# tanhuajie/Pytorch-RT1-for-Distributed-Training

Hardware: AMD Instinct MI355X
Metric: train samples/sec (whole node), RT-1 Language-Table, 1/2/4/8 MI355X (higher is better)
Workload: dtype bf16; 1 GPU; model=RT-1 (FiLM-EfficientNet-B3 + TokenLearner-8 + 8-layer transformer, 35.3M params), global_batch=128, batch_per_gpu=128, seq_len=6, parallelism=dp1, backend=hip, hipgraph=True, step=graph, graph_segments=1, tuned_library_gemms=True, full=False

## Files before the change

### pytorch_rt1_for_distributed_training_amd/csrc/bindings.cpp

```cpp
#include <algorithm>
#include <cmath>
#include <cstdlib>

#include <torch/extension.h>
#include <c10/hip/HIPStream.h>
#include <hip/hip_runtime.h>

#include "rt1_kernels.h"

namespace {

hipStream_t cur_stream() { return c10::hip::getCurrentHIPStream().stream(); }

bool sync_check() {
    static const bool on = [] {
        const char* e = std::getenv("RT1_SYNC_CHECK");
        return e != nullptr && *e != '\0' && *e != '0';
    }();
    return on;
}

void check_launch(int err, const char* what) {
    TORCH_CHECK(err == 0, what, ": HIP launch failed: ", hipGetErrorString((hipError_t)err));
    if (sync_check()) {
// ... 1207 lines not shown
    auto red = fs > 1 ? at::empty({5, N, Ce}, f32(y2)) : R[0];
    auto dW = at::empty({Cout, Ce}, f32(y2));
    check_launch(rt1_proj_bwd_finalize(G.data_ptr<float>(), R.data_ptr<float>(), gate.data_ptr<float>(), N, Cout, Ce, fs,
                                       red.data_ptr<float>(), dW.data_ptr<float>(), cur_stream()), "proj_bwd_finalize");
    return {red, dW};
}
bool proj_bwd_supported(int64_t Cout, int64_t Ce) { return rt1_proj_bwd_supported((int)Cout, (int)Ce) != 0; }

}

bool pw_gemm_supported(int64_t K, int64_t N) {
    return rt1_pw_gemm_supported((int)K, (int)N) != 0 || rt1_pw_wide_supported((int)K, (int)N) != 0;
}
bool pw_stats_supported(int64_t K, int64_t N) { return rt1_pw_gemm_supported((int)K, (int)N) != 0; }

std::vector<at::Tensor> pw_gemm(at::Tensor A, at::Tensor B, int64_t max_blocks, bool stats, OptT scale, OptT shift,
                                OptT gate, int64_t hw, bool store_operand) {
    check_bf(A, "A"); check_bf(B, "B");
    TORCH_CHECK(A.dim() == 2 && B.dim() == 2 && A.size(1) == B.size(1), "pw_gemm: A [M,K], B [N,K]");
    const int64_t M = A.size(0), K = A.size(1), N = B.size(0);
    TORCH_CHECK(M > 0 && M < (int64_t)1 << 31, "pw_gemm: bad M");
    const bool skinny = rt1_pw_gemm_supported((int)K, (int)N) != 0;
    TORCH_CHECK(skinny || (!stats && rt1_pw_wide_supported((int)K, (int)N)), "pw_gemm: no specialisation for K=", K,
                " N=", N, stats ? " with BN statistics" : "");
    TORCH_CHECK(reinterpret_cast<uintptr_t>(A.data_ptr()) % 16 == 0 && reinterpret_cast<uintptr_t>(B.data_ptr()) % 16 == 0,
                "pw_gemm: operands must be 16-byte aligned");
    const bool pro = scale.has_value() && scale->defined();
    if (pro) {
        TORCH_CHECK(skinny, "pw_gemm: the operand prologue needs a skinny specialisation (K=", K, " N=", N, ")");
        check_f(*scale, "scale", K);
        TORCH_CHECK(shift.has_value() && shift->defined() && gate.has_value() && gate->defined(),
                    "pw_gemm: prologue needs scale, shift and gate");
        check_f(*shift, "shift", K);
        TORCH_CHECK(hw > 0 && M % hw == 0, "pw_gemm: hw must divide M");
        check_f(*gate, "gate", (M / hw) * K);
    }
    TORCH_CHECK(!store_operand || pro, "pw_gemm: store_operand needs the prologue");
    auto C = at::empty({M, N}, A.options());
    at::Tensor aout;
    if (store_operand) aout = at::empty({M, K}, A.options());
    if (!skinny) {
        check_launch(rt1_pw_wide(bp(A), bp(B), (int)M, (int)K, (int)N, bp(C), (int)max_blocks, cur_stream()), "pw_wide");
        return {C};
    }
    at::Tensor ps, pq;
    if (stats) {
        const int g = rt1_pw_gemm_grid((int)M, (int)K, (int)N, (int)max_blocks);
        ps = at::empty({g, N}, f32(A));
        pq = at::empty({g, N}, f32(A));
    }
    check_launch(rt1_pw_gemm(bp(A), bp(B), (int)M, (int)K, (int)N, bp(C), stats ? ps.data_ptr<float>() : nullptr,
                             stats ? pq.data_ptr<float>() : nullptr, (int)max_blocks, fpo(scale), fpo(shift),
                             fpo(gate), (int)hw, store_operand ? bp(aout) : nullptr, cur_stream()), "pw_gemm");
    std::vector<at::Tensor> res{C};
    if (stats) { res.push_back(ps); res.push_back(pq); }
    if (store_operand) res.push_back(aout);
    return res;
}


bool pw_gemm_bnbwd_supported(int64_t K, int64_t N) { return rt1_pw_gemm_bnbwd_supported((int)K, (int)N) != 0; }
std::vector<at::Tensor> pw_gemm_bnbwd(at::Tensor dout, at::Tensor y, at::Tensor W, at::Tensor fmul, OptT keep,
                                      int64_t hw, OptT gamma, at::Tensor mean, at::Tensor rstd, at::Tensor mdz,
                                      at::Tensor mdzx, int64_t max_blocks) {
    check_bf(dout, "dout"); check_bf(y, "y"); check_bf(W, "W");
    TORCH_CHECK(dout.dim() == 2 && dout.sizes() == y.sizes() && W.dim() == 2 && W.size(1) == dout.size(1),
                "pw_gemm_bnbwd: dout, y [M, K], W [N, K]");
    const int64_t M = dout.size(0), K = dout.size(1), N = W.size(0);
    TORCH_CHECK(rt1_pw_gemm_bnbwd_supported((int)K, (int)N), "pw_gemm_bnbwd: no specialisation for K=", K, " N=", N);
    TORCH_CHECK(hw > 0 && M % hw == 0, "pw_gemm_bnbwd: hw must divide M");
    TORCH_CHECK(reinterpret_cast<uintptr_t>(dout.data_ptr()) % 16 == 0 && reinterpret_cast<uintptr_t>(y.data_ptr()) % 16 == 0 &&
                reinterpret_cast<uintptr_t>(W.data_ptr()) % 16 == 0, "pw_gemm_bnbwd: operands must be 16-byte aligned");
    check_f(fmul, "fmul", (M / hw) * K);
    check_opt_f(keep, "keep", M / hw); check_opt_f(gamma, "gamma", K);
    check_f(mean, "mean", K); check_f(rstd, "rstd", K); check_f(mdz, "mdz", K); check_f(mdzx, "mdzx", K);
    auto C = at::empty({M, N}, dout.options());
    auto dy = at::empty({M, K}, dout.options());
    check_launch(rt1_pw_gemm_bnbwd(bp(dout), bp(W), (int)M, (int)K, (int)N, bp(C), (int)max_blocks, bp(y),
                                   fmul.data_ptr<float>(), fpo(keep), (int)hw, fpo(gamma), mean.data_ptr<float>(),
                                   rstd.data_ptr<float>(), mdz.data_ptr<float>(), mdzx.data_ptr<float>(), bp(dy),
                                   cur_stream()), "pw_gemm_bnbwd");
    return {C, dy};
}

bool pw_bwd_supported(int64_t CE, int64_t CIN) { return rt1_pw_bwd_supported((int)CE, (int)CIN) != 0; }

std::vector<at::Tensor> pw_bwd(at::Tensor dA, at::Tensor y, at::Tensor x, at::Tensor We, at::Tensor consts, OptT dout,
                               OptT fmul, int64_t HW, int64_t max_blocks) {
    check_bf(dA, "dA"); check_bf(y, "y"); check_bf(x, "x"); check_bf(We, "We");
    TORCH_CHECK(dA.dim() == 2 && y.sizes() == dA.sizes() && x.dim() == 2 && x.size(0) == dA.size(0),
                "pw_bwd: dA/y [M, CE], x [M, CIN]");
    const int64_t M = dA.size(0), CE = dA.size(1), CIN = x.size(1);
    TORCH_CHECK(M > 0 && M < (int64_t)1 << 31, "pw_bwd: bad M");
    TORCH_CHECK(rt1_pw_bwd_supported((int)CE, (int)CIN), "pw_bwd: no specialisation for CE=", CE, " CIN=", CIN);
    TORCH_CHECK(We.dim() == 2 && We.size(0) == CE && We.size(1) == CIN, "pw_bwd: We must be [CE, CIN]");
    check_f(consts, "consts", 5 * CE);
    const bool skip = dout.has_value() && dout->defined();
    if (skip) {
        check_opt_bf(dout, "dout", M * CIN);
        TORCH_CHECK(fmul.has_value() && fmul->defined() && HW > 0 && M % HW == 0, "pw_bwd: residual needs fmul, HW");
        check_f(*fmul, "fmul", (M / HW) * CIN);
    }
    const int g = rt1_pw_bwd_grid((int)M, (int)max_blocks);
    auto dx = at::empty({M, CIN}, x.options());
    auto dwp = at::empty({g, CE, CIN}, f32(x));
    check_launch(rt1_pw_bwd(bp(dA), bp(y), bp(x), bp(We), consts.data_ptr<float>(), (int)M, (int)CE, (int)CIN, bp(dx),
                            skip ? bp(*dout) : nullptr, skip ? fmul->data_ptr<float>() : nullptr, (int)HW,
                            dwp.data_ptr<float>(), g, cur_stream()), "pw_bwd");
    return {dx, sum0(dwp)};
}

std::vector<at::Tensor> pw_bwd_z(at::Tensor dz, at::Tensor x, at::Tensor We, at::Tensor consts, OptT dout, OptT fmul,
                                 int64_t HW, int64_t max_blocks) {
    check_bf(dz, "dz"); check_bf(x, "x"); check_bf(We, "We");
    TORCH_CHECK(dz.dim() == 2 && x.dim() == 2 && x.size(0) == dz.size(0), "pw_bwd_z: dz [M, CE], x [M, CIN]");
    const int64_t M = dz.size(0), CE = dz.size(1), CIN = x.size(1);
    TORCH_CHECK(M > 0 && M < (int64_t)1 << 31, "pw_bwd_z: bad M");
    TORCH_CHECK(rt1_pw_bwd_supported((int)CE, (int)CIN), "pw_bwd_z: no specialisation for CE=", CE, " CIN=", CIN);
    TORCH_CHECK(We.dim() == 2 && We.size(0) == CE && We.size(1) == CIN, "pw_bwd_z: We must be [CE, CIN]");
    check_f(consts, "consts", 5 * CE);
    const bool skip = dout.has_value() && dout->defined();
    if (skip) {
        check_opt_bf(dout, "dout", M * CIN);
        TORCH_CHECK(fmul.has_value() && fmul->defined() && HW > 0 && M % HW == 0, "pw_bwd_z: residual needs fmul, HW");
        check_f(*fmul, "fmul", (M / HW) * CIN);
    }
    const int g = rt1_pw_bwd_grid((int)M, (int)max_blocks);
    auto dx = at::empty({M, CIN}, x.options());
    auto mk = at::empty({(int64_t)rt1_pw_bwd_z_mk_elems((int)CIN)}, x.options());
    auto r0 = at::empty({CIN}, f32(x));
    auto part = at::empty({g, (int64_t)rt1_pw_bwd_z_width((int)CE, (int)CIN)}, f32(x));
    check_launch(rt1_pw_bwd_z(bp(dz), bp(x), bp(We), consts.data_ptr<float>(), (int)M, (int)CE, (int)CIN, bp(mk),
                              r0.data_ptr<float>(), bp(dx), skip ? bp(*dout) : nullptr,
                              skip ? fmul->data_ptr<float>() : nullptr, (int)HW, part.data_ptr<float>(), g,
                              cur_stream()), "pw_bwd_z");
    auto S = sum0(part);
    auto dWe = at::empty({CE, CIN}, f32(x));
    check_launch(rt1_pw_bwd_z_finish(S.data_ptr<float>(), bp(We), consts.data_ptr<float>(), (int)CE, (int)CIN,
                                     dWe.data_ptr<float>(), cur_stream()), "pw_bwd_z_finish");
    return {dx, dWe};
}

std::vector<at::Tensor> pw_z_prep(at::Tensor We, at::Tensor consts) {
    check_bf(We, "We");
    TORCH_CHECK(We.dim() == 2, "pw_z_prep: We must be [CE, CIN]");
    const int64_t CE = We.size(0), CIN = We.size(1);
    check_f(consts, "consts", 5 * CE);
    auto wt = at::empty({CIN, CE}, We.options());
    auto mk = at::empty({CIN, CIN}, We.options());
    auto r0 = at::empty({CIN}, We.options().dtype(at::kFloat));
    check_launch(rt1_pw_z_prep(bp(We), consts.data_ptr<float>(), (int)CE, (int)CIN, bp(wt), bp(mk),
                               r0.data_ptr<float>(), cur_stream()), "pw_z_prep");
    return {wt, mk, r0};
}

at::Tensor pw_tall_tail(at::Tensor A, at::Tensor W, at::Tensor A2, at::Tensor W2, at::Tensor bias, OptT res,
                        OptT rmul, int64_t rhw) {
    check_bf(A, "A"); check_bf(W, "W"); check_bf(A2, "A2"); check_bf(W2, "W2");
    TORCH_CHECK(A.dim() == 2 && W.dim() == 2 && A.size(1) == W.size(1), "pw_tall_tail: A [M, K], W [N, K]");
    const int64_t M = A.size(0), K = A.size(1), N = W.size(0), K2 = A2.size(1);
    TORCH_CHECK(A2.dim() == 2 && A2.size(0) == M, "pw_tall_tail: A2 must be [M, K2]");
    TORCH_CHECK(W2.numel() == N * K2, "pw_tall_tail: W2 must be [N, K2]"); check_f(bias, "bias", N);
    TORCH_CHECK(rt1_pw_tall_preferred((int)K, (int)N) && K2 % 8 == 0, "pw_tall_tail: unsupported K=", K, " N=", N,
                " K2=", K2);
    const bool has_res = res.has_value() && res->defined();
    if (has_res) {
        check_opt_bf(res, "res", M * N);
        TORCH_CHECK(rmul.has_value() && rmul->defined() && rhw > 0 && M % rhw == 0, "pw_tall_tail: residual needs rmul");
        check_f(*rmul, "rmul", (M / rhw) * N);
    }
    auto C = at::empty({M, N}, A.options());
    check_launch(rt1_pw_tall_tail(bp(A), bp(W), (int)M, (int)K, (int)N, bp(A2), bp(W2), (int)K2,
                                  bias.data_ptr<float>(), has_res ? bp(*res) : nullptr,
                                  has_res ? rmul->data_ptr<float>() : nullptr, (int)rhw, bp(C), cur_stream()),
                 "pw_tall_tail");
    return C;
}

at::Tensor pw_z_finish(at::Tensor S, at::Tensor G, at::Tensor sx, at::Tensor We, at::Tensor consts) {
    check_bf(We, "We");
    const int64_t CE = We.size(0), CIN = We.size(1);
    const int64_t splits = S.dim() == 3 ? S.size(0) : 1;
    check_f(S, "S", splits * CE * CIN); check_f(G, "G", CIN * CIN); check_f(sx, "sx", CIN);
    check_f(consts, "consts", 5 * CE);
    auto dWe = at::empty({CE, CIN}, f32(S));
    check_launch(rt1_pw_z_finish(S.data_ptr<float>(), (int)splits, G.data_ptr<float>(), sx.data_ptr<float>(), bp(We),
                                 consts.data_ptr<float>(), (int)CE, (int)CIN, dWe.data_ptr<float>(), cur_stream()),
                 "pw_z_finish");
    return dWe;
}

void check_rows512(const at::Tensor& t, const char* name, at::ScalarType dt) {
    check_dev(t, name, dt);
    TORCH_CHECK(t.dim() == 2 && t.size(1) == 512, name, " must be [T, 512]");
}

std::vector<at::Tensor> tf_ln_fwd(at::Tensor x, at::Tensor g, at::Tensor b, double eps) {
    check_rows512(x, "x", at::kFloat);
    check_f(g, "g", 512); check_f(b, "b", 512);
    const int T = (int)x.size(0);
    auto y = at::empty({T, 512}, x.options().dtype(at::kBFloat16));
    auto mu = at::empty({T}, x.options()), rs = at::empty({T}, x.options());
    check_launch(rt1_ln_fwd(x.data_ptr<float>(), g.data_ptr<float>(), b.data_ptr<float>(), T, (float)eps, bp(y),
                            mu.data_ptr<float>(), rs.data_ptr<float>(), cur_stream()), "ln_fwd");
    return {y, mu, rs};
}

std::vector<at::Tensor> tf_ln_bwd(at::Tensor dy, at::Tensor x, at::Tensor mu, at::Tensor rs, at::Tensor g, OptT dres,
                                  bool want_bf) {
    check_rows512(dy, "dy", at::kBFloat16); check_rows512(x, "x", at::kFloat);
    const int T = (int)x.size(0);
    TORCH_CHECK(dy.size(0) == T, "dy/x rows");
    check_f(mu, "mu", T); check_f(rs, "rs", T); check_f(g, "g", 512);
    if (dres.has_value() && dres->defined()) { check_rows512(*dres, "dres", at::kFloat); TORCH_CHECK(dres->size(0) == T, "dres rows"); }
    const int grid = rt1_tf_grid(T);
    auto dx = at::empty({T, 512}, x.options());
    auto part = at::empty({want_bf ? 3 : 2, grid, 512}, x.options());
    at::Tensor dxb;
    if (want_bf) dxb = at::empty({T, 512}, x.options().dtype(at::kBFloat16));
    check_launch(rt1_ln_bwd(bp(dy), x.data_ptr<float>(), mu.data_ptr<float>(), rs.data_ptr<float>(), g.data_ptr<float>(),
                            fpo(dres), T, dx.data_ptr<float>(), part[0].data_ptr<float>(), part[1].data_ptr<float>(),
                            want_bf ? bp(dxb) : nullptr, want_bf ? part[2].data_ptr<float>() : nullptr, grid,
                            cur_stream()), "ln_bwd");
    auto s = colsum3(part, want_bf ? 3 : 2, grid, 512);
    if (want_bf) return {dx, s[0], s[1], dxb, s[2]};
    return {dx, s[0], s[1]};
}

std::vector<at::Tensor> tf_resid(at::Tensor x, at::Tensor a, at::Tensor bias, double p, int64_t seed, OptT seed_dev,
                                 OptT lg, OptT lb, double eps) {
    check_rows512(x, "x", at::kFloat); check_rows512(a, "a", at::kBFloat16);
    TORCH_CHECK(a.size(0) == x.size(0), "x/a rows");
    check_f(bias, "bias", 512);
    const int T = (int)x.size(0);
    const bool ln = lg.has_value() && lg->defined();
    if (ln) { check_f(*lg, "lg", 512); check_f(*lb, "lb", 512); }
    auto out = at::empty_like(x);
    at::Tensor xn, mu, rs;
    if (ln) {
        xn = at::empty({T, 512}, x.options().dtype(at::kBFloat16));
        mu = at::empty({T}, x.options());
        rs = at::empty({T}, x.options());
    }
    check_launch(rt1_resid(x.data_ptr<float>(), bp(a), bias.data_ptr<float>(), T, (float)p, (uint32_t)seed,
                           seed_ptr(seed_dev), out.data_ptr<float>(), fpo(lg), fpo(lb), (float)eps,
                           ln ? bp(xn) : nullptr, ln ? mu.data_ptr<float>() : nullptr,
                           ln ? rs.data_ptr<float>() : nullptr, cur_stream()), "resid");
    if (ln) return {out, xn, mu, rs};
    return {out};
}

std::vector<at::Tensor> tf_drop_bwd(at::Tensor dout, double p, int64_t seed, OptT seed_dev) {
    check_rows512(dout, "dout", at::kFloat);
    const int T = (int)dout.size(0);
    const int grid = rt1_tf_grid(T);
    auto dh = at::empty({T, 512}, dout.options().dtype(at::kBFloat16));
    auto part = at::empty({grid, 512}, dout.options());
    check_launch(rt1_drop_bwd(dout.data_ptr<float>(), T, (float)p, (uint32_t)seed, seed_ptr(seed_dev), bp(dh),
                              part.data_ptr<float>(), grid,
                              cur_stream()), "drop_bwd");
    return {dh, sum0(part)};
}


namespace rt1comm {
void register_comm(py::module_& m);
}
namespace rt1head {
void register_head(py::module_& m);
}

PYBIND11_MODULE(_rt1_hip, m) {
    m.doc() = "RT-1 HIP/CDNA4 kernels (gfx950)";
    m.def("flat_adam", &flat_adam, "fused Adam/AdamW over flat fp32 buffers");
    m.def("flat_adam_dev", &flat_adam_dev, "fused Adam/AdamW, step/lr read from a device tensor (graph-replayable)");
    m.def("flat_adam_clip_dev", &flat_adam_clip_dev, "flat_adam_dev obeying clip_state (clip coefficient, skipped step)");
    m.def("flat_adam_ema_dev", &flat_adam_ema_dev, "flat_adam_dev / flat_adam_clip_dev that also updates the EMA of the weights");
    m.def("flat_adam_groups_dev", &flat_adam_groups_dev,
          "the device-state Adam forms (plain, clip, EMA, both) with lr / weight_decay per parameter group");
    m.def("gradnorm_partials", &gradnorm_partials, "fp64 partial sums grad_sumsq writes for n floats");
    m.def("grad_sumsq", &grad_sumsq, "deterministic sum of squares of a flat fp32 gradient -> fp64 partials");
    m.def("grad_clip_finalize", &grad_clip_finalize, "partials -> clip_state {norm, coef, ok, counters}");
    m.def("buffer_guard_", &buffer_guard_, "ok ? shadow = buf : buf = shadow");
    m.def("bn_stats", &bn_stats);
    m.def("bn_finalize", &bn_finalize);
    m.def("xgram", &xgram);
    m.def("gemm_tail", &gemm_tail, py::arg("A"), py::arg("B"), py::arg("A2"), py::arg("B2"), py::arg("bias") = py::none(),
          py::arg("res") = py::none(), py::arg("rmul") = py::none(), py::arg("rhw") = 1, py::arg("cfg") = -1);
    m.def("gemm256", &gemm256, py::arg("A"), py::arg("B"), py::arg("nn") = false, py::arg("bias") = py::none(),
          py::arg("scale") = py::none(), py::arg("shift") = py::none(), py::arg("gate") = py::none(),
          py::arg("hw") = 0, py::arg("stats") = false, py::arg("store_a") = false, py::arg("bn") = 256);
    m.def("film_fwd", &film_fwd, py::arg("xe"), py::arg("K"), py::arg("w"), py::arg("bias"), py::arg("cmap"),
          py::arg("total"), py::arg("cfg") = -1);
    m.def("film_wgrad", &film_wgrad, py::arg("dflat"), py::arg("cmap"), py::arg("xe"), py::arg("K"),
          py::arg("splits") = 1, py::arg("tile") = 0);
    m.def("gemm", &gemm, py::arg("A"), py::arg("B"), py::arg("nn") = false, py::arg("bias") = py::none(),
          py::arg("scale") = py::none(), py::arg("shift") = py::none(), py::arg("gate") = py::none(),
          py::arg("hw") = 0, py::arg("out_f32") = false, py::arg("stats") = false, py::arg("cfg") = -1,
          py::arg("store_a") = false);
    m.def("x_bn_stats", &x_bn_stats);
    m.def("bn_from_gram", &bn_from_gram);
    m.def("dw_x_supported", &dw_x_supported);
    m.def("dw_tile_info", &dw_tile_info);
    m.def("dw_fwd_x", &dw_fwd_x);
    m.def("dw_bwd_fused_x", &dw_bwd_fused_x, py::arg("dA"), py::arg("y2"), py::arg("gate"), py::arg("rb"),
          py::arg("sc2"), py::arg("sh2"), py::arg("mu2"), py::arg("rs2"), py::arg("g2"), py::arg("mdz2"),
          py::arg("mdzx2"), py::arg("w"), py::arg("k"), py::arg("x"), py::arg("we"), py::arg("sc1"), py::arg("sh1"),
          py::arg("mu1"), py::arg("rs1"), py::arg("max_blocks"), py::arg("zout") = true);
    m.def("bn_apply", &bn_apply);
    m.def("bn_bwd_reduce", &bn_bwd_reduce);
    m.def("bn_bwd_finalize", &bn_bwd_finalize);
    m.def("bn_bwd_finalize_new", &bn_bwd_finalize_new);
    m.def("bn_bwd_finalize_pw", &bn_bwd_finalize_pw);
    m.def("bn_bwd_apply", &bn_bwd_apply, py::arg("G"), py::arg("rs"), py::arg("rb"), py::arg("HW"), py::arg("y"),
          py::arg("scale"), py::arg("shift"), py::arg("mean"), py::arg("rstd"), py::arg("gamma"), py::arg("act"),
          py::arg("mdz"), py::arg("mdzx"), py::arg("keep") = py::none());
    m.def("dw_fwd", &dw_fwd);
    m.def("dw_bwd_data", &dw_bwd_data);
    m.def("dw_bwd_weight", &dw_bwd_weight);
    m.def("dw_bwd_fused", &dw_bwd_fused, py::arg("dA"), py::arg("y2"), py::arg("gate"), py::arg("rb"), py::arg("sc2"),
          py::arg("sh2"), py::arg("mu2"), py::arg("rs2"), py::arg("g2"), py::arg("mdz2"), py::arg("mdzx2"), py::arg("w"),
          py::arg("k"), py::arg("x1"), py::arg("sc1"), py::arg("sh1"), py::arg("act1"), py::arg("mu1"), py::arg("rs1"),
          py::arg("max_blocks"), py::arg("variant") = -1, py::arg("zout") = false, py::arg("res") = py::none(),
          py::arg("rmul") = py::none());
    m.def("gram", &gram, "{x^T x, sum_m x} fp32 of x [M, C] bf16 in one MFMA pass", py::arg("x"),
          py::arg("variant") = -1, py::arg("splits") = 0);
    m.def("wgrad", &wgrad, "1x1-conv weight gradient dy^T a on MFMA (optional BN/act/gate prologue on a)",
          py::arg("dy"), py::arg("a"), py::arg("scale") = py::none(), py::arg("shift") = py::none(),
          py::arg("gate") = py::none(), py::arg("act") = 0, py::arg("hw") = 0, py::arg("variant") = -1,
          py::arg("splits") = -1, py::arg("partials") = false, py::arg("sums") = false);
    m.def("crop_resize_u8", &crop_resize_u8, "Pillow-exact random-resized-crop of raw uint8 frames (GPU)");
    m.def("crop_resize_gather_u8", &crop_resize_gather_u8,
          "crop_resize_u8 over frames gathered by index from an HBM-resident [F, h, w, 3] table");
    m.def("multi_reduce_copy_", &multi_reduce_copy_, "dst[i] = fixed-order sum of splits[i] partials of src[i]",
          py::arg("dst"), py::arg("src"), py::arg("splits"), py::arg("sstride"));
    m.def("multi_copy_", &multi_copy_, "dst[i].copy_(src[i]) for many same-dtype tensors, 128 per launch");
    m.def("multi_reduce_add_", &multi_reduce_add_, "dst[i] += fixed-order sum of splits[i] partials of src[i]",
          py::arg("dst"), py::arg("src"), py::arg("splits"), py::arg("sstride"));
    m.def("multi_add_", &multi_add_, "dst[i] += src[i] for many fp32 tensors, 128 per launch");
    m.def("colsum", &colsum_py, "deterministic fixed-order sum over dim 0 (fp32/bf16 in, fp32 out)");
    m.def("frame_pool", &frame_pool);
    m.def("block_tail", &block_tail);
    m.def("tail_bwd_reduce", &tail_bwd_reduce);
    m.def("stem_fwd", &stem_fwd);
    m.def("stem_bwd_weight", &stem_bwd_weight, py::arg("img"), py::arg("shift"), py::arg("dy"), py::arg("max_blocks"),
          py::arg("bn_x") = py::none(), py::arg("scale") = py::none(), py::arg("shift_bn") = py::none(),
          py::arg("mean") = py::none(), py::arg("rstd") = py::none(), py::arg("gamma") = py::none(),
          py::arg("mdz") = py::none(), py::arg("mdzx") = py::none());
    m.def("attn_fwd", &attn_fwd, py::arg("qkv"), py::arg("L"), py::arg("Kimg"), py::arg("scale"), py::arg("drop_p"),
          py::arg("seed"), py::arg("seed_dev") = py::none());
    m.def("se_bn_bwd_reduce", &se_bn_bwd_reduce);
    m.def("proj_bwd", &proj_bwd, "project-conv backward sums + dWp from (dy3, y2) per frame (skinny blocks)");
    m.def("proj_bwd_supported", &proj_bwd_supported);
    m.def("attn_keepmask", &attn_keepmask, py::arg("BH"), py::arg("S"), py::arg("drop_p"), py::arg("seed"),
          py::arg("like"), py::arg("seed_dev") = py::none());
    m.def("attn_bwd", &attn_bwd, py::arg("qkv"), py::arg("out"), py::arg("dout"), py::arg("lse"), py::arg("L"),
          py::arg("Kimg"), py::arg("scale"), py::arg("drop_p"), py::arg("seed"), py::arg("seed_dev") = py::none());
    m.def("tf_ln_fwd", &tf_ln_fwd);
    m.def("tf_ln_bwd", &tf_ln_bwd, py::arg("dy"), py::arg("x"), py::arg("mu"), py::arg("rs"), py::arg("g"),
          py::arg("dres") = py::none(), py::arg("want_bf") = false);
    m.def("tf_resid", &tf_resid, py::arg("x"), py::arg("a"), py::arg("bias"), py::arg("p"), py::arg("seed"),
          py::arg("seed_dev") = py::none(), py::arg("lg") = py::none(), py::arg("lb") = py::none(), py::arg("eps") = 1e-6);
    m.def("tf_drop_bwd", &tf_drop_bwd, py::arg("dout"), py::arg("p"), py::arg("seed"), py::arg("seed_dev") = py::none());
    m.def("pw_gemm_supported", &pw_gemm_supported);
    m.def("pw_stats_supported", &pw_stats_supported);
    m.def("add_scaled_", &add_scaled_);
    m.def("pw_bwd_supported", &pw_bwd_supported);
    m.def("pw_bwd", &pw_bwd);
    m.def("pw_bwd_z", &pw_bwd_z);
    m.def("pw_z_prep", &pw_z_prep);
    m.def("pw_gemm_bnbwd_supported", &pw_gemm_bnbwd_supported);
    m.def("pw_gemm_bnbwd", &pw_gemm_bnbwd);
    m.def("pw_tall_tail", &pw_tall_tail, py::arg("A"), py::arg("W"), py::arg("A2"), py::arg("W2"), py::arg("bias"),
          py::arg("res") = py::none(), py::arg("rmul") = py::none(), py::arg("rhw") = 1);
    m.def("pw_z_finish", &pw_z_finish);
    rt1comm::register_comm(m);
    rt1head::register_head(m);
    m.def("pw_gemm", &pw_gemm, py::arg("A"), py::arg("B"), py::arg("max_blocks"), py::arg("stats") = false,
          py::arg("scale") = py::none(), py::arg("shift") = py::none(), py::arg("gate") = py::none(),
          py::arg("hw") = 0, py::arg("store_operand") = false);
}
```

### pytorch_rt1_for_distributed_training_amd/csrc/kernels/dw/dw_plan.h

```cpp
#pragma once

namespace rt1 {
namespace dw {

enum Op : int { OP_FWD = 0, OP_FWD_X, OP_BWD_DATA, OP_BWD_WEIGHT, OP_BWD_FUSED_S1, OP_BWD_FUSED_S2 };

enum TileKind : int {
    TK_FWD = 0, TK_BWD_W = 1, TK_BWD_S2 = 2, TK_BWD_F = 3, TK_BWD_U4 = 4, TK_BWD_U8 = 5, TK_BWD_V4 = 6, TK_BWD_V8 = 7,
    TK_BWD_U2 = 8
};
inline bool is_uni(int kind) { return kind == TK_BWD_U4 || kind == TK_BWD_U8 || kind == TK_BWD_U2; }

constexpr int DW_R1 = 4;
constexpr int DWU_CPT3 = 8;
constexpr int DWU_R3 = 2;
constexpr int DWU_CPT5 = 4;
constexpr int DWU_R5 = 4;
constexpr int DWV_CPT3 = 8;
constexpr int DWV_R3 = 2;
constexpr int DWV_CPT5 = 4;
constexpr int DWV_R5 = 4;

#define DW_XMODE_S1(X) X(3, 0x14) X(5, 0x26)
#define DW_XMODE_S2(X) X(3, 0x19) X(3, 0x13) X(3, 0x11) X(3, 0x26) X(5, 0x14)

struct DwPlan {
    int err;
    int N, H, W, C, Ho, Wo, k, s, pad, nv, cv, chunks;
    int kind;
    int xk;
    int R;
    int cpt;
    int ring;
    int TH, TW;
    int sb;
    int lds;
    int red_taps;
    int grid_x;
};

DwPlan dw_plan(int op, int N, int H, int W, int C, int k, int s, int pro, int epi, int variant, int cin,
               int max_blocks_x);

}
}
```

### pytorch_rt1_for_distributed_training_amd/csrc/kernels/dw/dw_stage.h

```cpp
#pragma once
#include "dw_common.h"

namespace rt1 {
namespace dw {

typedef float f2 __attribute__((ext_vector_type(2)));

__device__ __forceinline__ void unpack4x2(const uint4 u, f2 (&f)[4]) {
#if RT1_DW_TIMING & 1
    f[0] = f2{__uint_as_float(u.x), __uint_as_float(u.y)};
    f[1] = f2{__uint_as_float(u.y), __uint_as_float(u.z)};
    f[2] = f2{__uint_as_float(u.z), __uint_as_float(u.w)};
    f[3] = f2{__uint_as_float(u.w), __uint_as_float(u.x)};
    return;
#endif
    f[0] = f2{__uint_as_float(u.x << 16), __uint_as_float(u.x & 0xffff0000u)};
    f[1] = f2{__uint_as_float(u.y << 16), __uint_as_float(u.y & 0xffff0000u)};
    f[2] = f2{__uint_as_float(u.z << 16), __uint_as_float(u.z & 0xffff0000u)};
    f[3] = f2{__uint_as_float(u.w << 16), __uint_as_float(u.w & 0xffff0000u)};
}

__device__ __forceinline__ void load4x2(const float* __restrict__ p, f2 (&o)[4]) {
    const float4 a = *reinterpret_cast<const float4*>(p);
    const float4 b = *reinterpret_cast<const float4*>(p + 4);
    o[0] = f2{a.x, a.y}; o[1] = f2{a.z, a.w}; o[2] = f2{b.x, b.y}; o[3] = f2{b.z, b.w};
}

struct StripWalk {
    int ty, gx, o1, o2;
    int dty, dgx, gw, d1, d2, w1, w2;
    __device__ __forceinline__ StripWalk(int start, int step, int gw_, int r1, int c1, int r2, int c2) {
        gw = gw_;
        ty = start / gw;
        gx = start - ty * gw;
        dty = step / gw;
        dgx = step - dty * gw;
        o1 = ty * r1 + gx * c1;
        o2 = ty * r2 + gx * c2;
        d1 = dty * r1 + dgx * c1;
        d2 = dty * r2 + dgx * c2;
        w1 = r1 - gw * c1;
        w2 = r2 - gw * c2;
    }
    __device__ __forceinline__ void next() {
        ty += dty;
        gx += dgx;
        o1 += d1;
        o2 += d2;
        if (gx >= gw) {
            gx -= gw;
            ++ty;
            o1 += w1;
            o2 += w2;
        }
    }
};

struct WinRect {
    int r0, r1, c0, c1;
    __device__ __forceinline__ WinRect(int ih0, int iw0, int IH, int IW, int Hs, int Ws)
        : r0(max(0, -ih0)), r1(max(max(0, -ih0), min(IH, Hs - ih0))), c0(max(0, -iw0)),
          c1(max(max(0, -iw0), min(IW, Ws - iw0))) {}
    __device__ __forceinline__ WinRect(int IH, int IW) : r0(0), r1(IH), c0(0), c1(IW) {}
    __device__ __forceinline__ int w() const { return c1 - c0; }
    __device__ __forceinline__ int npix() const { return (r1 - r0) * (c1 - c0); }
};

template <typename T>
__device__ __forceinline__ void zero_ring(T* tile, const WinRect& q, int IH, int IW, int lanes, int vv, int pb,
                                          int PLs, const T zero) {
    const int top = q.r0 * IW, bot = (IH - q.r1) * IW, wl = q.c0, sw = q.c0 + (IW - q.c1);
    const int n = top + bot + (q.r1 - q.r0) * sw;
    for (int i = pb; i < n; i += PLs) {
        int px;
        if (i < top) {
            px = i;
        } else if (i < top + bot) {
            px = q.r1 * IW + (i - top);
        } else {
            const int j = i - top - bot, r = j / sw, c = j - r * sw;
            px = (q.r0 + r) * IW + (c < wl ? c : q.c1 + (c - wl));
        }
        tile[px * lanes + vv] = zero;
    }
}

typedef short bf16x8 __attribute__((ext_vector_type(8)));
typedef float f32x4 __attribute__((ext_vector_type(4)));

constexpr int xk_kc(int xk) { return xk >> 4; }
constexpr int xk_ng(int xk) { return xk & 15; }

template <int KC>
constexpr int xw_ld() { return KC * 32 + 8; }
template <int KC>
__device__ __forceinline__ void stage_xweights(bf16_t* __restrict__ wel, const XExp& xe, int C8, int c0, int nch) {
    constexpr int LDW = xw_ld<KC>();
    for (int i = threadIdx.x; i < C8 * KC * 4; i += BLOCK) {
        const int row = i / (KC * 4), col = (i - row * (KC * 4)) * 8;
        uint4 u = make_uint4(0, 0, 0, 0);
        if (row < nch && col < xe.cin) u = *reinterpret_cast<const uint4*>(xe.we + (int64_t)(c0 + row) * xe.cin + col);
        *reinterpret_cast<uint4*>(wel + row * LDW + col) = u;
    }
}

template <int KC, int NG, bool ACT, bool WLDS = false>
__device__ __forceinline__ void stage_xmfma(bf16_t* __restrict__ tl, int ldt, const XExp& xe, int H, int W, int n,
                                            int ih0, int iw0, int IH, int IW, int c0, int nch,
                                            const float* __restrict__ bnl, const bf16_t* __restrict__ wel = nullptr,
                                            int ps = 1, int p0 = 0, int np = -1) {
    const int lane = threadIdx.x & 63, wave = threadIdx.x >> 6;
    const int lr = lane & 15, lh = lane >> 4;
    const int npix = np >= 0 ? np : IH * IW, ngrp = (npix + 15) >> 4;
    const int cin = xe.cin;
    bf16x8 wf[WLDS ? 1 : NG][KC];
    if constexpr (!WLDS) {
#pragma unroll
        for (int g = 0; g < NG; ++g)
#pragma unroll
            for (int kc = 0; kc < KC; ++kc) {
                const int c = g * 16 + lr, col = kc * 32 + lh * 8;
                wf[g][kc] = (c < nch && col < cin)
                                ? *reinterpret_cast<const bf16x8*>(xe.we + (int64_t)(c0 + c) * cin + col)
                                : bf16x8{0, 0, 0, 0, 0, 0, 0, 0};
            }
    }
    const bf16_t* xb = xe.x + (int64_t)n * H * W * cin;
    auto load_x = [&](int grp, bf16x8 (&xf)[KC]) -> bool {
        const int p = grp * 16 + lr, pw = p0 + p;
        const int r = pw / IW, c = pw - r * IW;
        const int ih = ih0 + ps * r, iw = iw0 + ps * c;
        const bool ok = p < npix && (unsigned)ih < (unsigned)H && (unsigned)iw < (unsigned)W;
#pragma unroll
        for (int kc = 0; kc < KC; ++kc) {
            const int col = kc * 32 + lh * 8;
            xf[kc] = (ok && col < cin)
                         ? *reinterpret_cast<const bf16x8*>(xb + (uint32_t)(ih * W + iw) * (uint32_t)cin + col)
                         : bf16x8{0, 0, 0, 0, 0, 0, 0, 0};
        }
        return ok;
    };
    int grp = wave;
    bf16x8 xc[KC], xn[KC];
    bool okc = false, okn = false;
    if (grp < ngrp) okc = load_x(grp, xc);
    for (; grp < ngrp; grp += 4) {
        if (grp + 4 < ngrp) okn = load_x(grp + 4, xn);
        const int p = grp * 16 + lr;
#pragma unroll
        for (int g = 0; g < NG; ++g) {
            f32x4 acc = f32x4{0.f, 0.f, 0.f, 0.f};
#pragma unroll
            for (int kc = 0; kc < KC; ++kc) {
                const bf16x8 wv = WLDS ? *reinterpret_cast<const bf16x8*>(wel + (g * 16 + lr) * xw_ld<KC>() + kc * 32 +
                                                                          lh * 8)
                                       : wf[WLDS ? 0 : g][kc];
                acc = __builtin_amdgcn_mfma_f32_16x16x32_bf16(wv, xc[kc], acc, 0, 0, 0);
            }
            const int ch = g * 16 + lh * 4;
            if (p < npix) {
                uint2 u = make_uint2(pack2(acc[0], acc[1]), pack2(acc[2], acc[3]));
                if constexpr (ACT) {
                    const float4 sc4 = *reinterpret_cast<const float4*>(bnl + ch);
                    const float4 sh4 = *reinterpret_cast<const float4*>(bnl + ldt + ch);
                    f2 z[2] = {f2{__uint_as_float(u.x << 16), __uint_as_float(u.x & 0xffff0000u)},
                               f2{__uint_as_float(u.y << 16), __uint_as_float(u.y & 0xffff0000u)}};
                    z[0] = z[0] * f2{sc4.x, sc4.y} + f2{sh4.x, sh4.y};
                    z[1] = z[1] * f2{sc4.z, sc4.w} + f2{sh4.z, sh4.w};
                    f2 t[2];
#pragma unroll
                    for (int j = 0; j < 2; ++j) t[j] = z[j] * f2{-1.4426950408889634f, -1.4426950408889634f};
#pragma unroll
                    for (int j = 0; j < 2; ++j)
                        t[j] = f2{__builtin_amdgcn_exp2f(t[j].x), __builtin_amdgcn_exp2f(t[j].y)} + f2{1.f, 1.f};
#pragma unroll
                    for (int j = 0; j < 2; ++j) t[j] = f2{__builtin_amdgcn_rcpf(t[j].x), __builtin_amdgcn_rcpf(t[j].y)};
#pragma unroll
                    for (int j = 0; j < 2; ++j) z[j] = z[j] * t[j];
                    u = make_uint2(pack2(z[0].x, z[0].y), pack2(z[1].x, z[1].y));
                }
                if (!okc) u = make_uint2(0u, 0u);
                *reinterpret_cast<uint2*>(tl + p * ldt + ch) = u;
            }
        }
        if (grp + 4 < ngrp) {
#pragma unroll
            for (int kc = 0; kc < KC; ++kc) xc[kc] = xn[kc];
            okc = okn;
        }
    }
}

template <int EPI>
__device__ __forceinline__ void stage_epi_consts(float* ecl, const BnBwdEpi& e, int v0, int ncv, int cv) {
    if constexpr (EPI == EPI_BNBWD) {
        const int C8 = cv * 8;
        for (int i = threadIdx.x; i < C8; i += BLOCK) {
            const bool ok = i < ncv * 8;
            const int c = v0 * 8 + i;
            const float rr = ok ? e.rstd[c] : 0.f;
            ecl[i] = ok ? e.scale[c] : 0.f;
            ecl[C8 + i] = ok ? e.shift[c] : 0.f;
            ecl[2 * C8 + i] = rr;
            ecl[3 * C8 + i] = ok ? -e.mean[c] * rr : 0.f;
        }
    }
}

constexpr uint32_t OOB = 0x7ffffff0u;
__device__ __forceinline__ __amdgpu_buffer_rsrc_t wave_rsrc(const void* p, uint32_t bytes) {
    const uint64_t a = reinterpret_cast<uint64_t>(p);
    const uint32_t lo = __builtin_amdgcn_readfirstlane((uint32_t)a);
    const uint32_t hi = __builtin_amdgcn_readfirstlane((uint32_t)(a >> 32));
    void* q = reinterpret_cast<void*>(((uint64_t)hi << 32) | lo);
    return __builtin_amdgcn_make_buffer_rsrc(q, (short)0, (int)__builtin_amdgcn_readfirstlane(bytes), 0x00020000);
}
__device__ __forceinline__ uint4 buf_load16(__amdgpu_buffer_rsrc_t r, uint32_t off) {
    typedef unsigned int u32x4 __attribute__((ext_vector_type(4)));
    const u32x4 v = __builtin_amdgcn_raw_buffer_load_b128(r, (int)off, 0, 0);
    return make_uint4(v.x, v.y, v.z, v.w);
}

template <int SU, bool RING>
__device__ __forceinline__ void stage_dy(uint4* tile, const DyBnBwd& d, const DwGeo& g, int n, int ih0, int iw0,
                                         int IH, int IW, int v0, int ncv) {
    const int cv = g.cv;
    const int t = threadIdx.x;
    const int vv = t % cv, PLs = BLOCK / cv;
    int pb = t / cv;
    if (pb >= PLs) return;
    const bool cvalid = vv < ncv;
    const int c0 = (v0 + (cvalid ? vv : 0)) * 8;
    f2 A[4], B[4], K2[4], K0[4], SC[4], SH[4];
    {
        float gm[8], rr[8], mu[8], mz[8], mx[8], a[8], b[8], sc[8], sh[8];
        load8f(d.gamma + c0, gm); load8f(d.rstd + c0, rr); load8f(d.mean + c0, mu);
        load8f(d.mdz + c0, mz); load8f(d.mdzx + c0, mx);
        load8f(d.gate + (int64_t)n * g.C + c0, a); load8f(d.rb + (int64_t)n * g.C + c0, b);
        load8f(d.scale + c0, sc); load8f(d.shift + c0, sh);
#pragma unroll
        for (int j = 0; j < 4; ++j) {
            float k1x = gm[2 * j] * rr[2 * j], k1y = gm[2 * j + 1] * rr[2 * j + 1];
            A[j] = f2{a[2 * j] * k1x, a[2 * j + 1] * k1y};
            B[j] = f2{b[2 * j] * k1x, b[2 * j + 1] * k1y};
            K2[j] = f2{-k1x * rr[2 * j] * mx[2 * j], -k1y * rr[2 * j + 1] * mx[2 * j + 1]};
            K0[j] = f2{-k1x * (mz[2 * j] - mu[2 * j] * rr[2 * j] * mx[2 * j]),
                       -k1y * (mz[2 * j + 1] - mu[2 * j + 1] * rr[2 * j + 1] * mx[2 * j + 1])};
            SC[j] = f2{sc[2 * j], sc[2 * j + 1]};
            SH[j] = f2{sh[2 * j], sh[2 * j + 1]};
        }
    }
#if RT1_DW_TIMING & 32
    const uint32_t fbytes = 0u;
#else
    const uint32_t fbytes = (uint32_t)g.H * g.W * g.C * 2u;
#endif
    const __amdgpu_buffer_rsrc_t rg = wave_rsrc(d.dA + (int64_t)n * g.H * g.W * g.C, fbytes);
    const __amdgpu_buffer_rsrc_t ry = wave_rsrc(d.y + (int64_t)n * g.H * g.W * g.C, fbytes);
    const uint32_t cb = (uint32_t)c0 * 2u;
    const WinRect q = RING ? WinRect(ih0, iw0, IH, IW, g.H, g.W) : WinRect(IH, IW);
    if constexpr (RING) zero_ring(tile, q, IH, IW, cv, vv, pb, PLs, make_uint4(0, 0, 0, 0));
    const int npix = q.npix(), qw = q.w();
    if (npix == 0) return;
    int row = pb / qw, col = pb - row * qw;
    const int dr = PLs / qw, dc = PLs - dr * qw;
    for (; pb < npix; pb += PLs * SU) {
        uint4 ug[SU], uy[SU];
        bool ok[SU];
        int px[SU];
#pragma unroll
        for (int k = 0; k < SU; ++k) {
            const int ih = ih0 + q.r0 + row, iw = iw0 + q.c0 + col;
            if constexpr (RING) px[k] = (q.r0 + row) * IW + q.c0 + col;
            ok[k] = cvalid && pb + k * PLs < npix &&
                    (RING || ((unsigned)ih < (unsigned)g.H && (unsigned)iw < (unsigned)g.W));
            const uint32_t off = ok[k] ? (uint32_t)(ih * g.W + iw) * (uint32_t)g.C * 2u + cb : OOB;
            ug[k] = buf_load16(rg, off);
            uy[k] = buf_load16(ry, off);
            row += dr;
            col += dc;
            if (col >= qw) { col -= qw; ++row; }
        }
#pragma unroll
        for (int k = 0; k < SU; ++k) {
            const int p = RING ? px[k] : pb + k * PLs;
            if (pb + k * PLs >= npix) break;
            f2 gv[4], yv[4];
            unpack4x2(ug[k], gv);
            unpack4x2(uy[k], yv);
            f2 o[4];
            const f2 one = f2{1.f, 1.f};
            f2 z[4], t[4], lin[4];
#pragma unroll
            for (int j = 0; j < 4; ++j) z[j] = yv[j] * SC[j] + SH[j];
#pragma unroll
            for (int j = 0; j < 4; ++j) t[j] = z[j] * f2{-1.4426950408889634f, -1.4426950408889634f};
#pragma unroll
            for (int j = 0; j < 4; ++j) lin[j] = K2[j] * yv[j] + K0[j];
#pragma unroll
            for (int j = 0; j < 4; ++j) t[j] = f2{__builtin_amdgcn_exp2f(t[j].x), __builtin_amdgcn_exp2f(t[j].y)};
#pragma unroll
            for (int j = 0; j < 4; ++j) gv[j] = A[j] * gv[j] + B[j];
#pragma unroll
            for (int j = 0; j < 4; ++j) t[j] = t[j] + one;
#pragma unroll
            for (int j = 0; j < 4; ++j) t[j] = f2{__builtin_amdgcn_rcpf(t[j].x), __builtin_amdgcn_rcpf(t[j].y)};
#pragma unroll
            for (int j = 0; j < 4; ++j) yv[j] = one - t[j];
#pragma unroll
            for (int j = 0; j < 4; ++j) z[j] = z[j] * yv[j] + one;
#pragma unroll
            for (int j = 0; j < 4; ++j) z[j] = t[j] * z[j];
#pragma unroll
            for (int j = 0; j < 4; ++j) o[j] = z[j] * gv[j] + lin[j];
            uint4 v = make_uint4(pack2(o[0].x, o[0].y), pack2(o[1].x, o[1].y), pack2(o[2].x, o[2].y),
                                 pack2(o[3].x, o[3].y));
            if (!ok[k]) v = make_uint4(0, 0, 0, 0);
            tile[p * cv + vv] = v;
        }
    }
}

}
}
```

### pytorch_rt1_for_distributed_training_amd/csrc/kernels/dw_bwd_s1.hip

```cpp
#include "dw/dw_uni.h"

using namespace rt1;
using namespace rt1::dw;

namespace {


#ifndef DW_CENTRE_PREFETCH
#define DW_CENTRE_PREFETCH 1
#endif
typedef __attribute__((address_space(3))) void dw_lds_void;
constexpr int DWU2_SU = 4;

template <int SU, bool RING>
__device__ __forceinline__ void stage_dy_half(uint4* tile, const DyBnBwd& d, const DwGeo& g, int n, int ih0, int iw0,
                                              int IH, int IW, int v0, int ncv) {
    const int cv = g.cv, ch = 2 * cv;
    const int t = threadIdx.x;
    const int hv = t % ch, PLs = BLOCK / ch;
    int pb = t / ch;
    if (pb >= PLs) return;
    const bool cvalid = (hv >> 1) < ncv;
    const int c0 = v0 * 8 + (cvalid ? hv : 0) * 4;
    f2 A[2], B[2], K2[2], K0[2], SC[2], SH[2];
    {
        float gm[4], rr[4], mu[4], mz[4], mx[4], a[4], b[4], sc[4], sh[4];
        auto ld4 = [](const float* p, float (&o)[4]) {
            const float4 v = *reinterpret_cast<const float4*>(p);
            o[0] = v.x; o[1] = v.y; o[2] = v.z; o[3] = v.w;
        };
        ld4(d.gamma + c0, gm); ld4(d.rstd + c0, rr); ld4(d.mean + c0, mu);
        ld4(d.mdz + c0, mz); ld4(d.mdzx + c0, mx);
        ld4(d.gate + (int64_t)n * g.C + c0, a); ld4(d.rb + (int64_t)n * g.C + c0, b);
        ld4(d.scale + c0, sc); ld4(d.shift + c0, sh);
#pragma unroll
        for (int j = 0; j < 2; ++j) {
            float k1x = gm[2 * j] * rr[2 * j], k1y = gm[2 * j + 1] * rr[2 * j + 1];
            A[j] = f2{a[2 * j] * k1x, a[2 * j + 1] * k1y};
            B[j] = f2{b[2 * j] * k1x, b[2 * j + 1] * k1y};
            K2[j] = f2{-k1x * rr[2 * j] * mx[2 * j], -k1y * rr[2 * j + 1] * mx[2 * j + 1]};
            K0[j] = f2{-k1x * (mz[2 * j] - mu[2 * j] * rr[2 * j] * mx[2 * j]),
                       -k1y * (mz[2 * j + 1] - mu[2 * j + 1] * rr[2 * j + 1] * mx[2 * j + 1])};
            SC[j] = f2{sc[2 * j], sc[2 * j + 1]};
            SH[j] = f2{sh[2 * j], sh[2 * j + 1]};
        }
    }
    const uint32_t fbytes = (uint32_t)g.H * g.W * g.C * 2u;
    const __amdgpu_buffer_rsrc_t rg = wave_rsrc(d.dA + (int64_t)n * g.H * g.W * g.C, fbytes);
    const __amdgpu_buffer_rsrc_t ry = wave_rsrc(d.y + (int64_t)n * g.H * g.W * g.C, fbytes);
    const uint32_t cb = (uint32_t)c0 * 2u;
    uint2* tl = reinterpret_cast<uint2*>(tile);
    const WinRect q = RING ? WinRect(ih0, iw0, IH, IW, g.H, g.W) : WinRect(IH, IW);
    if constexpr (RING) zero_ring(tl, q, IH, IW, ch, hv, pb, PLs, make_uint2(0, 0));
    const int npix = q.npix(), qw = q.w();
    if (npix == 0) return;
    int row = pb / qw, col = pb - row * qw;
    const int dr = PLs / qw, dc = PLs - dr * qw;
    typedef unsigned int u32x2 __attribute__((ext_vector_type(2)));
    for (; pb < npix; pb += PLs * SU) {
        u32x2 ug[SU], uy[SU];
        bool ok[SU];
        int px[SU];
#pragma unroll
        for (int k = 0; k < SU; ++k) {
            const int ih = ih0 + q.r0 + row, iw = iw0 + q.c0 + col;
            if constexpr (RING) px[k] = (q.r0 + row) * IW + q.c0 + col;
            ok[k] = cvalid && pb + k * PLs < npix &&
                    (RING || ((unsigned)ih < (unsigned)g.H && (unsigned)iw < (unsigned)g.W));
            const uint32_t off = ok[k] ? (uint32_t)(ih * g.W + iw) * (uint32_t)g.C * 2u + cb : OOB;
            ug[k] = __builtin_amdgcn_raw_buffer_load_b64(rg, (int)off, 0, 0);
            uy[k] = __builtin_amdgcn_raw_buffer_load_b64(ry, (int)off, 0, 0);
            row += dr;
            col += dc;
            if (col >= qw) { col -= qw; ++row; }
        }
        f2 o[SU][2];
        {
            const f2 one = f2{1.f, 1.f};
            f2 gv[SU][2], yv[SU][2], z[SU][2], t[SU][2];
#pragma unroll
            for (int k = 0; k < SU; ++k) {
                gv[k][0] = f2{__uint_as_float(ug[k].x << 16), __uint_as_float(ug[k].x & 0xffff0000u)};
                gv[k][1] = f2{__uint_as_float(ug[k].y << 16), __uint_as_float(ug[k].y & 0xffff0000u)};
                yv[k][0] = f2{__uint_as_float(uy[k].x << 16), __uint_as_float(uy[k].x & 0xffff0000u)};
                yv[k][1] = f2{__uint_as_float(uy[k].y << 16), __uint_as_float(uy[k].y & 0xffff0000u)};
            }
#pragma unroll
            for (int k = 0; k < SU; ++k)
#pragma unroll
                for (int j = 0; j < 2; ++j) z[k][j] = yv[k][j] * SC[j] + SH[j];
#pragma unroll
            for (int k = 0; k < SU; ++k)
#pragma unroll
                for (int j = 0; j < 2; ++j) t[k][j] = z[k][j] * f2{-1.4426950408889634f, -1.4426950408889634f};
#pragma unroll
            for (int k = 0; k < SU; ++k)
#pragma unroll
                for (int j = 0; j < 2; ++j) {
                    t[k][j] = f2{__builtin_amdgcn_exp2f(t[k][j].x), __builtin_amdgcn_exp2f(t[k][j].y)};
                    o[k][j] = K2[j] * yv[k][j] + K0[j];
                }
#pragma unroll
            for (int k = 0; k < SU; ++k)
#pragma unroll
                for (int j = 0; j < 2; ++j) {
                    t[k][j] = t[k][j] + one;
                    gv[k][j] = A[j] * gv[k][j] + B[j];
                }
#pragma unroll
            for (int k = 0; k < SU; ++k)
#pragma unroll
                for (int j = 0; j < 2; ++j) t[k][j] = f2{__builtin_amdgcn_rcpf(t[k][j].x), __builtin_amdgcn_rcpf(t[k][j].y)};
#pragma unroll
            for (int k = 0; k < SU; ++k)
#pragma unroll
                for (int j = 0; j < 2; ++j) yv[k][j] = one - t[k][j];
#pragma unroll
            for (int k = 0; k < SU; ++k)
#pragma unroll
                for (int j = 0; j < 2; ++j) z[k][j] = z[k][j] * yv[k][j] + one;
#pragma unroll
            for (int k = 0; k < SU; ++k)
#pragma unroll
                for (int j = 0; j < 2; ++j) z[k][j] = t[k][j] * z[k][j];
#pragma unroll
            for (int k = 0; k < SU; ++k)
#pragma unroll
                for (int j = 0; j < 2; ++j) o[k][j] = z[k][j] * gv[k][j] + o[k][j];
        }
#pragma unroll
        for (int k = 0; k < SU; ++k) {
            const int p = RING ? px[k] : pb + k * PLs;
            if (pb + k * PLs >= npix) break;
            uint2 v = make_uint2(pack2(o[k][0].x, o[k][0].y), pack2(o[k][1].x, o[k][1].y));
            if (!ok[k]) v = make_uint2(0, 0);
            tl[p * ch + hv] = v;
        }
    }
}

template <int K, int R, int EPI, int CPT, int XK = 0, bool RG = false>
__global__ __launch_bounds__(BLOCK, CPT == 2 ? DWU2_OCC : DWU_OCC) void dw_bwd_uni_kernel(DyBnBwd d, const bf16_t* __restrict__ x1,
                                                                        const float* __restrict__ w, DwGeo g,
                                                                        int TH, int TW, BnBwdEpi e,
                                                                        bf16_t* __restrict__ dx, float* __restrict__ pdz,
                                                                        float* __restrict__ pdzx,
                                                                        float* __restrict__ dwp, int red_taps, XExp xe,
                                                                        int sb) {
    using CV = ChanVec<CPT>;
    using V = typename CV::T;
    constexpr int P = (K - 1) / 2, KK = K * K, NV = CPT / 2, HPV = 8 / CPT;
    static_assert(XK == 0 || EPI == EPI_BNBWD, "x-mode is for expand blocks (BN1 epilogue)");
    extern __shared__ __attribute__((aligned(16))) char smem[];
    const int IH = TH + K - 1, IW = TW + K - 1;
    const int cv = g.cv, C8 = cv * 8, nlc = cv * HPV;
    uint4* dt = reinterpret_cast<uint4*>(smem);
    float* wl = reinterpret_cast<float*>(dt + IH * IW * cv);
    float* ecl = wl + KK * C8;
    bf16_t* yl = reinterpret_cast<bf16_t*>(ecl + (EPI == EPI_BNBWD ? 4 * C8 : 0));
    bf16_t* wel = yl + (sb > 0 ? sb * R : TH * TW) * C8;
    float* red = reinterpret_cast<float*>(smem);

    const int v0 = blockIdx.y * cv;
    const int ncv = min(cv, g.nv - v0);
    const int t = threadIdx.x;
    if constexpr (XK != 0) stage_xweights<xk_kc(XK)>(wel, xe, C8, v0 * 8, ncv * 8);
    const int lane_c = t % nlc, pl = t / nlc, PL = BLOCK / nlc;
    const int cofs = lane_c * CPT;
    const bool active = lane_c / HPV < ncv && pl < PL;
    const int groups_w = TW / R;
    const StripWalk walk0(pl, PL, groups_w, IW * nlc, R * nlc, g.W * g.C, R * g.C);

    for (int i = t; i < KK * C8; i += BLOCK) {
        const int tap = i / C8, cc = i % C8;
        wl[i] = (cc < ncv * 8) ? w[(int64_t)(v0 * 8 + cc) * KK + (KK - 1 - tap)] : 0.f;
    }
    stage_epi_consts<EPI>(ecl, e, v0, ncv, cv);
    const int tiles_h = (g.H + TH - 1) / TH, tiles_w = (g.W + TW - 1) / TW;
    const int64_t ntiles = (int64_t)g.N * tiles_h * tiles_w;
    f2 wacc[KK][NV], s_acc[NV], q_acc[NV];
#pragma unroll
    for (int j = 0; j < NV; ++j) {
        s_acc[j] = q_acc[j] = f2{0.f, 0.f};
#pragma unroll
        for (int a = 0; a < KK; ++a) wacc[a][j] = f2{0.f, 0.f};
    }

    constexpr bool CS = XK == 0 && centre_stage_on(CPT, R);
    for (int64_t tile_id = blockIdx.x; tile_id < ntiles; tile_id += gridDim.x) {
        const int n = (int)(tile_id / (tiles_h * tiles_w));
        const int rem = (int)(tile_id - (int64_t)n * tiles_h * tiles_w);
        const int oh0 = (rem / tiles_w) * TH, ow0 = (rem % tiles_w) * TW;
        __syncthreads();
        if constexpr (CS) {
            const int nvec = TH * TW * cv, lane = t & 63;
            const bf16_t* fb = x1 + (int64_t)n * g.H * g.W * g.C;
            for (int i0 = (t >> 6) * 64; i0 < nvec; i0 += BLOCK) {
                const int i = i0 + lane;
                if (i < nvec) {
                    const int px = i / cv, v = i - px * cv;
                    const int py = px / TW, pxx = px - py * TW;
                    const bool ok = v < ncv && oh0 + py < g.H && ow0 + pxx < g.W;
                    const bf16_t* src = ok ? fb + ((int64_t)(oh0 + py) * g.W + ow0 + pxx) * g.C + (v0 + v) * 8 : fb;
                    __builtin_amdgcn_global_load_lds(src, (dw_lds_void*)(yl + (size_t)i0 * 8), 16, 0, 0);
                }
            }
        }
#if !(RT1_DW_TIMING & 2)
        if constexpr (CPT == 2) stage_dy_half<DWU2_SU, RG>(dt, d, g, n, oh0 - P, ow0 - P, IH, IW, v0, ncv);
        else stage_dy<DWU_SU, RG>(dt, d, g, n, oh0 - P, ow0 - P, IH, IW, v0, ncv);
#endif
        if constexpr (CS) asm volatile("s_waitcnt vmcnt(0)" ::: "memory");
        const int nstrips = TH * groups_w, sbw = (XK != 0 && sb > 0) ? sb : nstrips;
        for (int s0 = 0; s0 < nstrips; s0 += sbw) {
        const int s1 = XK != 0 ? min(nstrips, s0 + sbw) : nstrips;
        if constexpr (XK != 0) {
            if (s0 > 0) __syncthreads();
            stage_xmfma<xk_kc(XK), xk_ng(XK), false, true>(yl, C8, xe, g.H, g.W, n, oh0, ow0, TH, TW, v0 * 8, ncv * 8,
                                                           nullptr, wel, 1, s0 * R, (s1 - s0) * R);
        }
        __syncthreads();
        if (!active) {
            if constexpr (XK != 0) continue;
            else break;
        }
        const int64_t tbase = (((int64_t)n * g.H + oh0) * g.W + ow0) * g.C + v0 * 8 + cofs;
        auto centre_load = [&](const StripWalk& w, V (&dst)[R]) {
            const bool rowok = w.ty < TH && oh0 + w.ty < g.H;
#pragma unroll
            for (int r = 0; r < R; ++r)
                dst[r] = (rowok && ow0 + w.gx * R + r < g.W)
                             ? *reinterpret_cast<const V*>(x1 + tbase + w.o2 + (int64_t)r * g.C)
                             : CV::zero();
        };
        constexpr bool CPREF = XK == 0 && !CS && DW_CENTRE_PREFETCH && CPT == 2 && R == 4;
        V ynext[R];
        if constexpr (CPREF) centre_load(walk0, ynext);
        int si = s0 + pl;
        for (StripWalk it = (XK != 0 && s0) ? StripWalk(s0 + pl, PL, groups_w, IW * nlc, R * nlc, g.W * g.C, R * g.C)
                                            : walk0;
             (XK == 0 || si < s1) && it.ty < TH; it.next(), si += (XK != 0 ? PL : 0)) {
            const int tx = it.gx * R;
            if (oh0 + it.ty >= g.H) break;
            const int64_t obase = tbase + it.o2;
            const int co = opaque(cofs);
            V yr[R];
            if constexpr (CPREF) {
#pragma unroll
                for (int r = 0; r < R; ++r) yr[r] = ynext[r];
                StripWalk nx = it;
                nx.next();
                centre_load(nx, ynext);
            } else {
#pragma unroll
            for (int r = 0; r < R; ++r) {
#if RT1_DW_TIMING & 16
                yr[r] = CV::zero();
#else
                if constexpr (XK != 0)
                    yr[r] = *reinterpret_cast<const V*>(yl + ((si - s0) * R + r) * C8 + co);
                else if constexpr (CS)
                    yr[r] = (ow0 + tx + r < g.W) ? *reinterpret_cast<const V*>(yl + (it.ty * TW + tx + r) * C8 + co)
                                                 : CV::zero();
                else
                    yr[r] = (ow0 + tx + r < g.W) ? *reinterpret_cast<const V*>(x1 + obase + (int64_t)r * g.C)
                                                 : CV::zero();
#endif
            }
            }
            f2 a[R][NV], gp[R][NV];
#if RT1_DW_TIMING & 16
            if constexpr (false) {
#else
            if constexpr (EPI == EPI_BNBWD) {
#endif
                f2 sc[NV], sh[NV];
                CV::loadf(ecl + co, sc);
                CV::loadf(ecl + C8 + co, sh);
                f2 y[R][NV];
                bool ok[R];
#pragma unroll
                for (int r = 0; r < R; ++r) {
                    CV::unpack(yr[r], y[r]);
                    ok[r] = ow0 + tx + r < g.W;
                }
                centre_silu<R, NV>(y, sc, sh, ok, a, gp);
            } else {
#pragma unroll
                for (int r = 0; r < R; ++r) CV::unpack(yr[r], a[r]);
            }
            f2 acc[R][NV];
#pragma unroll
            for (int r = 0; r < R; ++r)
#pragma unroll
                for (int j = 0; j < NV; ++j) acc[r][j] = f2{0.f, 0.f};
            const V* trow = reinterpret_cast<const V*>(dt) + it.o1 + lane_c;
#if RT1_DW_TIMING & 4
#pragma unroll
            for (int kr = 0; kr < 0; ++kr) {
#else
#pragma unroll
            for (int kr = 0; kr < K; ++kr) {
#endif
                f2 wrow[K][NV];
#pragma unroll
                for (int kw = 0; kw < K; ++kw) CV::loadf(wl + (kr * K + kw) * C8 + co, wrow[kw]);
                constexpr int NIN = R - 1 + K;
#pragma unroll
                for (int qq = 0; qq < NIN; ++qq) {
                    f2 in[NV];
                    CV::unpack(trow[(kr * IW + qq) * nlc], in);
#pragma unroll
                    for (int r = 0; r < R; ++r) {
                        const int kw = qq - r;
                        if (kw >= 0 && kw < K) {
#pragma unroll
                            for (int j = 0; j < NV; ++j) {
                                acc[r][j] = in[j] * wrow[kw][j] + acc[r][j];
                                wacc[kr * K + kw][j] = in[j] * a[r][j] + wacc[kr * K + kw][j];
                            }
                        }
                    }
                }
#pragma unroll
                for (int r = 0; r < R; ++r)
#pragma unroll
                    for (int j = 0; j < NV; ++j) pin(acc[r][j]);
#pragma unroll
                for (int kw = 0; kw < K; ++kw)
#pragma unroll
                    for (int j = 0; j < NV; ++j) pin(wacc[kr * K + kw][j]);
            }
            f2 rr[NV], mr[NV];
            if constexpr (EPI == EPI_BNBWD) {
                CV::loadf(ecl + 2 * C8 + co, rr);
                CV::loadf(ecl + 3 * C8 + co, mr);
            }
#if RT1_DW_TIMING & 8
#pragma unroll
            for (int r = 0; r < R; ++r)
                if (acc[r][0].x == 1234.5f) dx[obase + (int64_t)r * g.C] = (bf16_t)1;
            if constexpr (false)
#endif
#pragma unroll
            for (int r = 0; r < R; ++r) {
                if (ow0 + tx + r >= g.W) continue;
                if constexpr (EPI == EPI_BNBWD) {
                    if (e.zout) {
#pragma unroll
                        for (int j = 0; j < NV; ++j) acc[r][j] = acc[r][j] * gp[r][j];
                    }
                }
                if constexpr (EPI == EPI_NONE) {
                    if (e.res) {
                        f2 rv[NV], fm[NV];
                        CV::unpack(*reinterpret_cast<const V*>(e.res + obase + (int64_t)r * g.C), rv);
                        CV::loadf(e.rmul + (int64_t)n * g.C + v0 * 8 + co, fm);
#pragma unroll
                        for (int j = 0; j < NV; ++j) acc[r][j] = rv[j] * fm[j] + acc[r][j];
                    }
                }
                const V o = CV::pack(acc[r]);
                *reinterpret_cast<V*>(dx + obase + (int64_t)r * g.C) = o;
                if constexpr (EPI == EPI_BNBWD) {
                    f2 of[NV], y[NV];
                    CV::unpack(o, of);
                    CV::unpack(yr[r], y);
#pragma unroll
                    for (int j = 0; j < NV; ++j) {
                        f2 dz = of[j];
                        if (!e.zout) dz = dz * gp[r][j];
                        s_acc[j] = s_acc[j] + dz;
                        q_acc[j] = dz * (y[j] * rr[j] + mr[j]) + q_acc[j];
                    }
                }
            }
        }
        if constexpr (XK == 0) break;
        }
    }
    const int nc = ncv * 8;
    if constexpr (EPI != EPI_NONE) {
        __syncthreads();
        if (active) {
#pragma unroll
            for (int j = 0; j < NV; ++j) {
                red[pl * C8 + cofs + 2 * j] = s_acc[j].x;
                red[pl * C8 + cofs + 2 * j + 1] = s_acc[j].y;
                red[(PL + pl) * C8 + cofs + 2 * j] = q_acc[j].x;
                red[(PL + pl) * C8 + cofs + 2 * j + 1] = q_acc[j].y;
            }
        }
        __syncthreads();
        for (int cc = t; cc < nc; cc += BLOCK) {
            float sa = 0.f, sb = 0.f;
            for (int p = 0; p < PL; ++p) {
                sa += red[p * C8 + cc];
                sb += red[(PL + p) * C8 + cc];
            }
            pdz[(int64_t)blockIdx.x * g.C + v0 * 8 + cc] = sa;
            pdzx[(int64_t)blockIdx.x * g.C + v0 * 8 + cc] = sb;
        }
    }
    for (int t0 = 0; t0 < KK; t0 += red_taps) {
        const int tn = min(red_taps, KK - t0);
        __syncthreads();
        if (active) {
#pragma unroll
            for (int tap = 0; tap < KK; ++tap) {
                if (tap < t0 || tap >= t0 + tn) continue;
                float* rp = red + ((tap - t0) * PL + pl) * C8 + cofs;
#pragma unroll
                for (int j = 0; j < NV; ++j) {
                    rp[2 * j] = wacc[tap][j].x;
                    rp[2 * j + 1] = wacc[tap][j].y;
                }
            }
        }
        __syncthreads();
        for (int i = t; i < tn * nc; i += BLOCK) {
            const int tt = i / nc, cc = i - tt * nc;
            float s = 0.f;
            for (int p = 0; p < PL; ++p) s += red[(tt * PL + p) * C8 + cc];
            dwp[(int64_t)blockIdx.x * g.C * KK + (int64_t)(v0 * 8 + cc) * KK + (KK - 1 - (t0 + tt))] = s;
        }
    }
}

}

extern "C" {

int rt1_dw_bwd_fused(const bf16_t* dA, const bf16_t* y2, const float* gate, const float* rb, const float* scale2,
                     const float* shift2, const float* mean2, const float* rstd2, const float* gamma2,
                     const float* mdz2, const float* mdzx2, const float* w, const float* wflip, const bf16_t* x1,
                     const float* scale1, const float* shift1, int act1, const float* mean1, const float* rstd1, int N,
                     int H, int W, int C, int k, int grid_x, bf16_t* dx, float* pdz, float* pdzx, float* dwp,
                     hipStream_t st, int variant, int zout, const bf16_t* xin, const bf16_t* we, int cin,
                     const bf16_t* res, const float* rmul) {
    const bool pro = scale1 != nullptr, epi = mean1 != nullptr;
    if (xin && (cin <= 0 || !we)) return (int)hipErrorInvalidValue;
    const DwPlan p = dw_plan(OP_BWD_FUSED_S1, N, H, W, C, k, 1, pro, epi, variant, xin ? cin : 0, grid_x);
    if (p.err) return p.err;
    const bool uni = is_uni(p.kind);
    if (res && (epi || !rmul || !uni)) return (int)hipErrorInvalidValue;
    if (zout && !(epi && uni)) return (int)hipErrorInvalidValue;
    const DwGeo g = geo_of(p);
    DyBnBwd d{dA, y2, gate, rb, scale2, shift2, mean2, rstd2, gamma2, mdz2, mdzx2};
    BnBwdEpi e{epi ? x1 : nullptr, scale1, shift1, mean1, rstd1, zout ? 1 : 0, res, rmul};
    dim3 grid(grid_x, p.chunks);
    if (uni) {
        if (epi && act1 != ACT_SILU) return (int)hipErrorInvalidValue;
        const XExp xe{xin, we, cin};
#define LU1(KK, RR, EE, CC, XX, RGV)                                                                                \
    hipLaunchKernelGGL((dw_bwd_uni_kernel<KK, RR, EE, CC, XX, RGV>), grid, dim3(BLOCK), p.lds, st, d, x1, w, g,      \
                       p.TH, p.TW, e, dx, pdz, pdzx, dwp, p.red_taps, xe, p.sb)
#define LU(KK, RR, EE, CC, XX)                                                                                      \
    if (p.k == KK && p.R == RR && epi == (EE == EPI_BNBWD) && p.cpt == CC && p.xk == XX) {                          \
        if (p.ring) LU1(KK, RR, EE, CC, XX, true); else LU1(KK, RR, EE, CC, XX, false);                             \
        return (int)hipGetLastError();                                                                              \
    }
#define XU(KK, XX) LU(KK, (KK == 3 ? DWU_R3 : DWU_R5), EPI_BNBWD, (KK == 3 ? DWU_CPT3 : DWU_CPT5), XX)
        DW_XMODE_S1(XU)
        LU(3, DWU_R3, EPI_BNBWD, DWU_CPT3, 0) LU(3, DWU_R3, EPI_NONE, DWU_CPT3, 0)
        LU(5, 5, EPI_BNBWD, 2, 0) LU(5, 5, EPI_NONE, 2, 0)
        LU(5, 4, EPI_BNBWD, 2, 0) LU(5, 4, EPI_NONE, 2, 0)
        LU(5, 5, EPI_BNBWD, DWU_CPT5, 0) LU(5, 5, EPI_NONE, DWU_CPT5, 0)
        LU(5, DWU_R5, EPI_BNBWD, DWU_CPT5, 0) LU(5, DWU_R5, EPI_NONE, DWU_CPT5, 0)
#undef XU
#undef LU
#undef LU1
        return (int)hipErrorInvalidValue;
    }
    if (y2 == nullptr) return (int)hipErrorInvalidValue;
    return launch_bwd_twopass(p, d, x1, scale1, shift1, act1, wflip, grid_x, dx, pdz, pdzx, e, epi, dwp, st);
}

}
```

### pytorch_rt1_for_distributed_training_amd/csrc/kernels/dw_bwd_s2.hip

```cpp
#include "dw/dw_uni.h"

using namespace rt1;
using namespace rt1::dw;

namespace {

template <int K, int R, int EPI, int CPT, int PR, int PC, bool XM>
__device__ __forceinline__ void uni_s2_class(const uint4* __restrict__ dt, const float* __restrict__ wl,
                                             const float* __restrict__ ecl, const bf16_t* __restrict__ x1,
                                             bf16_t* __restrict__ dx, const DwGeo& g, int C8, int nlc, int lane_c,
                                             int cofs, int pl, int PL, int TH, int TW, int DW, int ih0, int iw0,
                                             int oh_lo, int ow_lo, int64_t tbase, f2 (&wacc)[K * K][CPT / 2],
                                             f2 (&s_acc)[CPT / 2], f2 (&q_acc)[CPT / 2], int zout,
                                             const bf16_t* __restrict__ yl) {
    using CV = ChanVec<CPT>;
    using V = typename CV::T;
    constexpr int P = (K - 1) / 2, NV = CPT / 2;
    constexpr int KH0 = (PR + P) & 1, KW0 = (PC + P) & 1;
    constexpr int NKH = (K - KH0 + 1) / 2, NKW = (K - KW0 + 1) / 2;
    constexpr int KWMAX = KW0 + 2 * (NKW - 1);
    constexpr int NIN = R + NKW - 1;
    const int groups_w = TW / (2 * R);
    StripWalk it(pl, PL, groups_w, DW * nlc, R * nlc, 2 * g.W * g.C, 2 * R * g.C);
    const int64_t cbase = tbase + ((int64_t)PR * g.W + PC) * g.C;
    for (; 2 * it.ty + PR < TH; it.next()) {
        const int ih = ih0 + PR + 2 * it.ty;
        if (ih >= g.H) break;
        const int iwb = iw0 + PC + 2 * R * it.gx;
        const int64_t obase = cbase + it.o2;
        const int co = opaque(cofs);
        V yr[R];
#pragma unroll
        for (int r = 0; r < R; ++r) {
            if constexpr (XM)
                yr[r] = *reinterpret_cast<const V*>(yl + (it.ty * (TW / 2) + R * it.gx + r) * C8 + co);
            else
                yr[r] = (iwb + 2 * r < g.W) ? *reinterpret_cast<const V*>(x1 + obase + (int64_t)2 * r * g.C)
                                            : CV::zero();
        }
        f2 a[R][NV], gp[R][NV];
        if constexpr (EPI == EPI_BNBWD) {
            f2 sc[NV], sh[NV];
            CV::loadf(ecl + co, sc);
            CV::loadf(ecl + C8 + co, sh);
            f2 y[R][NV];
            bool ok[R];
#pragma unroll
            for (int r = 0; r < R; ++r) {
                CV::unpack(yr[r], y[r]);
                ok[r] = iwb + 2 * r < g.W;
            }
            centre_silu<R, NV>(y, sc, sh, ok, a, gp);
        } else {
#pragma unroll
            for (int r = 0; r < R; ++r) CV::unpack(yr[r], a[r]);
        }
        f2 acc[R][NV];
#pragma unroll
        for (int r = 0; r < R; ++r)
#pragma unroll
            for (int j = 0; j < NV; ++j) acc[r][j] = f2{0.f, 0.f};
        const int row0 = ((ih + P - KH0) >> 1) - oh_lo, col0 = ((iwb + P - KWMAX) >> 1) - ow_lo;
        const V* tw = reinterpret_cast<const V*>(dt) + (row0 * DW + col0) * nlc + lane_c;
#pragma unroll
        for (int ih_ = 0; ih_ < NKH; ++ih_) {
            const int kh = KH0 + 2 * ih_;
            f2 wrow[NKW][NV];
#pragma unroll
            for (int jw = 0; jw < NKW; ++jw) CV::loadf(wl + (kh * K + KWMAX - 2 * jw) * C8 + co, wrow[jw]);
            const V* trow = tw - ih_ * DW * nlc;
#pragma unroll
            for (int q = 0; q < NIN; ++q) {
                f2 in[NV];
                CV::unpack(trow[q * nlc], in);
#pragma unroll
                for (int r = 0; r < R; ++r) {
                    const int jw = q - r;
                    if (jw >= 0 && jw < NKW) {
#pragma unroll
                        for (int j = 0; j < NV; ++j) {
                            acc[r][j] = in[j] * wrow[jw][j] + acc[r][j];
                            wacc[kh * K + KWMAX - 2 * jw][j] = in[j] * a[r][j] + wacc[kh * K + KWMAX - 2 * jw][j];
                        }
                    }
                }
            }
#pragma unroll
            for (int r = 0; r < R; ++r)
#pragma unroll
                for (int j = 0; j < NV; ++j) pin(acc[r][j]);
#pragma unroll
            for (int jw = 0; jw < NKW; ++jw)
#pragma unroll
                for (int j = 0; j < NV; ++j) pin(wacc[kh * K + KWMAX - 2 * jw][j]);
        }
        f2 rr[NV], mr[NV];
        if constexpr (EPI == EPI_BNBWD) {
            CV::loadf(ecl + 2 * C8 + co, rr);
            CV::loadf(ecl + 3 * C8 + co, mr);
        }
#pragma unroll
        for (int r = 0; r < R; ++r) {
            if (iwb + 2 * r >= g.W) continue;
            if constexpr (EPI == EPI_BNBWD) {
                if (zout) {
#pragma unroll
                    for (int j = 0; j < NV; ++j) acc[r][j] = acc[r][j] * gp[r][j];
                }
            }
            const V o = CV::pack(acc[r]);
            *reinterpret_cast<V*>(dx + obase + (int64_t)2 * r * g.C) = o;
            if constexpr (EPI == EPI_BNBWD) {
                f2 of[NV], y[NV];
                CV::unpack(o, of);
                CV::unpack(yr[r], y);
#pragma unroll
                for (int j = 0; j < NV; ++j) {
                    f2 dz = of[j];
                        if (!zout) dz = dz * gp[r][j];
                    s_acc[j] = s_acc[j] + dz;
                    q_acc[j] = dz * (y[j] * rr[j] + mr[j]) + q_acc[j];
                }
            }
        }
    }
}

template <int K, int R, int EPI, int CPT, int XK = 0, bool RG = false>
__global__ __launch_bounds__(BLOCK, DWU_OCC) void dw_bwd_uni_s2_kernel(DyBnBwd d, const bf16_t* __restrict__ x1,
                                                                           const float* __restrict__ w, DwGeo g,
                                                                           int TH, int TW, BnBwdEpi e,
                                                                           bf16_t* __restrict__ dx,
                                                                           float* __restrict__ pdz,
                                                                           float* __restrict__ pdzx,
                                                                           float* __restrict__ dwp, int red_taps,
                                                                           XExp xe) {
    constexpr int P = (K - 1) / 2, KK = K * K, NV = CPT / 2, HPV = 8 / CPT;
    static_assert(XK == 0 || EPI == EPI_BNBWD, "x-mode is for expand blocks (BN1 epilogue)");
    extern __shared__ __attribute__((aligned(16))) char smem[];
    const int DH = (TH + K) / 2 + 1, DW = (TW + K) / 2 + 1;
    const int cv = g.cv, C8 = cv * 8, nlc = cv * HPV;
    uint4* dt = reinterpret_cast<uint4*>(smem);
    float* wl = reinterpret_cast<float*>(dt + DH * DW * cv);
    float* ecl = wl + KK * C8;
    bf16_t* yl = reinterpret_cast<bf16_t*>(ecl + (EPI == EPI_BNBWD ? 4 * C8 : 0));
    bf16_t* wel = yl + (TH / 2) * (TW / 2) * C8;
    float* red = reinterpret_cast<float*>(smem);

    const int v0 = blockIdx.y * cv;
    const int ncv = min(cv, g.nv - v0);
    const int t = threadIdx.x;
    if constexpr (XK != 0) stage_xweights<xk_kc(XK)>(wel, xe, C8, v0 * 8, ncv * 8);
    const int lane_c = t % nlc, pl = t / nlc, PL = BLOCK / nlc;
    const int cofs = lane_c * CPT;
    const bool active = lane_c / HPV < ncv && pl < PL;
    DwGeo go = g;
    go.H = g.Ho;
    go.W = g.Wo;

    for (int i = t; i < KK * C8; i += BLOCK) {
        const int tap = i / C8, cc = i % C8;
        wl[i] = (cc < ncv * 8) ? w[(int64_t)(v0 * 8 + cc) * KK + tap] : 0.f;
    }
    stage_epi_consts<EPI>(ecl, e, v0, ncv, cv);
    const int tiles_h = (g.H + TH - 1) / TH, tiles_w = (g.W + TW - 1) / TW;
    const int64_t ntiles = (int64_t)g.N * tiles_h * tiles_w;
    f2 wacc[KK][NV], s_acc[NV], q_acc[NV];
#pragma unroll
    for (int j = 0; j < NV; ++j) {
        s_acc[j] = q_acc[j] = f2{0.f, 0.f};
#pragma unroll
        for (int a = 0; a < KK; ++a) wacc[a][j] = f2{0.f, 0.f};
    }
    for (int64_t tile_id = blockIdx.x; tile_id < ntiles; tile_id += gridDim.x) {
        const int n = (int)(tile_id / (tiles_h * tiles_w));
        const int rem = (int)(tile_id - (int64_t)n * tiles_h * tiles_w);
        const int ih0 = (rem / tiles_w) * TH, iw0 = (rem % tiles_w) * TW;
        const int oh_lo = (ih0 + P - (K - 1)) >> 1, ow_lo = (iw0 + P - (K - 1)) >> 1;
        __syncthreads();
        stage_dy<DWU_SU, RG>(dt, d, go, n, oh_lo, ow_lo, DH, DW, v0, ncv);
        const int64_t tbase = (((int64_t)n * g.H + ih0) * g.W + iw0) * g.C + v0 * 8 + cofs;
        if constexpr (XK != 0) {
#define CLS(PR_, PC_)                                                                                              \
    if (PR_ | PC_) __syncthreads();                                                                                \
    stage_xmfma<xk_kc(XK), xk_ng(XK), false, true>(yl, C8, xe, g.H, g.W, n, ih0 + PR_, iw0 + PC_, TH / 2, TW / 2,   \
                                                   v0 * 8, ncv * 8, nullptr, wel, 2);                              \
    __syncthreads();                                                                                               \
    if (active)                                                                                                    \
        uni_s2_class<K, R, EPI, CPT, PR_, PC_, true>(dt, wl, ecl, x1, dx, g, C8, nlc, lane_c, cofs, pl, PL, TH, TW, DW, \
                                                     ih0, iw0, oh_lo, ow_lo, tbase, wacc, s_acc, q_acc, e.zout, yl)
            CLS(0, 0);
            CLS(0, 1);
            CLS(1, 0);
            CLS(1, 1);
#undef CLS
            continue;
        }
        __syncthreads();
        if (!active) continue;
#define CLS(PR_, PC_)                                                                                              \
    uni_s2_class<K, R, EPI, CPT, PR_, PC_, false>(dt, wl, ecl, x1, dx, g, C8, nlc, lane_c, cofs, pl, PL, TH, TW, DW, \
                                                  ih0, iw0, oh_lo, ow_lo, tbase, wacc, s_acc, q_acc, e.zout, yl)
        CLS(0, 0);
        CLS(0, 1);
        CLS(1, 0);
        CLS(1, 1);
#undef CLS
    }
    const int nc = ncv * 8;
    if constexpr (EPI != EPI_NONE) {
        __syncthreads();
        if (active) {
#pragma unroll
            for (int j = 0; j < NV; ++j) {
                red[pl * C8 + cofs + 2 * j] = s_acc[j].x;
                red[pl * C8 + cofs + 2 * j + 1] = s_acc[j].y;
                red[(PL + pl) * C8 + cofs + 2 * j] = q_acc[j].x;
                red[(PL + pl) * C8 + cofs + 2 * j + 1] = q_acc[j].y;
            }
        }
        __syncthreads();
        for (int cc = t; cc < nc; cc += BLOCK) {
            float sa = 0.f, sb = 0.f;
            for (int p = 0; p < PL; ++p) {
                sa += red[p * C8 + cc];
                sb += red[(PL + p) * C8 + cc];
            }
            pdz[(int64_t)blockIdx.x * g.C + v0 * 8 + cc] = sa;
            pdzx[(int64_t)blockIdx.x * g.C + v0 * 8 + cc] = sb;
        }
    }
    for (int t0 = 0; t0 < KK; t0 += red_taps) {
        const int tn = min(red_taps, KK - t0);
        __syncthreads();
        if (active) {
#pragma unroll
            for (int tap = 0; tap < KK; ++tap) {
                if (tap < t0 || tap >= t0 + tn) continue;
                float* rp = red + ((tap - t0) * PL + pl) * C8 + cofs;
#pragma unroll
                for (int j = 0; j < NV; ++j) {
                    rp[2 * j] = wacc[tap][j].x;
                    rp[2 * j + 1] = wacc[tap][j].y;
                }
            }
        }
        __syncthreads();
        for (int i = t; i < tn * nc; i += BLOCK) {
            const int tt = i / nc, cc = i - tt * nc;
            float s = 0.f;
            for (int p = 0; p < PL; ++p) s += red[(tt * PL + p) * C8 + cc];
            dwp[(int64_t)blockIdx.x * g.C * KK + (int64_t)(v0 * 8 + cc) * KK + t0 + tt] = s;
        }
    }
}

}

extern "C" {

int rt1_dw_bwd_fused_s2(const bf16_t* dA, const bf16_t* y2, const float* gate, const float* rb, const float* scale2,
                        const float* shift2, const float* mean2, const float* rstd2, const float* gamma2,
                        const float* mdz2, const float* mdzx2, const float* w, const bf16_t* x1, const float* scale1,
                        const float* shift1, const float* mean1, const float* rstd1, int N, int H, int W, int C, int k,
                        int grid_x, bf16_t* dx, float* pdz, float* pdzx, float* dwp, hipStream_t st, int zout,
                        const bf16_t* xin, const bf16_t* we, int cin) {
    const bool epi = mean1 != nullptr;
    if (epi != (scale1 != nullptr) || (zout && !epi)) return (int)hipErrorInvalidValue;
    if (xin && (cin <= 0 || !we)) return (int)hipErrorInvalidValue;
    const DwPlan p = dw_plan(OP_BWD_FUSED_S2, N, H, W, C, k, 2, epi, epi, 1, xin ? cin : 0, grid_x);
    if (p.err) return p.err;
    const DwGeo g = geo_of(p);
    DyBnBwd d{dA, y2, gate, rb, scale2, shift2, mean2, rstd2, gamma2, mdz2, mdzx2};
    BnBwdEpi e{epi ? x1 : nullptr, scale1, shift1, mean1, rstd1, zout ? 1 : 0};
    dim3 grid(grid_x, p.chunks);
    const XExp xe{xin, we, cin};
#define LV1(KK, RR, EE, CC, XX, RGV)                                                                                \
    hipLaunchKernelGGL((dw_bwd_uni_s2_kernel<KK, RR, EE, CC, XX, RGV>), grid, dim3(BLOCK), p.lds, st, d, x1, w, g,   \
                       p.TH, p.TW, e, dx, pdz, pdzx, dwp, p.red_taps, xe)
#define LV(KK, RR, EE, CC, XX)                                                                                      \
    if (p.k == KK && p.R == RR && epi == (EE == EPI_BNBWD) && p.cpt == CC && p.xk == XX) {                          \
        if (p.ring) LV1(KK, RR, EE, CC, XX, true); else LV1(KK, RR, EE, CC, XX, false);                             \
        return (int)hipGetLastError();                                                                              \
    }
#define XV(KK, XX) LV(KK, (KK == 3 ? DWV_R3 : DWV_R5), EPI_BNBWD, (KK == 3 ? DWV_CPT3 : DWV_CPT5), XX)
    DW_XMODE_S2(XV)
    LV(3, DWV_R3, EPI_BNBWD, DWV_CPT3, 0) LV(3, DWV_R3, EPI_NONE, DWV_CPT3, 0)
    LV(5, DWV_R5, EPI_BNBWD, DWV_CPT5, 0) LV(5, DWV_R5, EPI_NONE, DWV_CPT5, 0)
#undef XV
#undef LV
#undef LV1
    return (int)hipErrorInvalidValue;
}

}
```

### pytorch_rt1_for_distributed_training_amd/csrc/kernels/dw_fwd.hip

```cpp
#include "dw/dw_stage.h"

using namespace rt1;
using namespace rt1::dw;

namespace {

constexpr int DW_SU = 4;
enum StagePro : int { PRO_COPY = 0, PRO_AFFINE = 1, PRO_SILU = 2 };
template <int SU, int PRO, bool RING>
__device__ __forceinline__ void stage_tile_t(uint4* tile, const bf16_t* __restrict__ x, const DwGeo& g, int n, int ih0,
                                             int iw0, int IH, int IW, int Hs, int Ws, int v0, int ncv,
                                             const float* __restrict__ scale, const float* __restrict__ shift) {
    const int cv = g.cv;
    const int t = threadIdx.x;
    const int vv = t % cv, PLs = BLOCK / cv;
    int pb = t / cv;
    if (pb >= PLs) return;
    const bool cvalid = vv < ncv;
    const int c0 = (v0 + (cvalid ? vv : 0)) * 8;
    f2 SC[4], SH[4];
    if constexpr (PRO != PRO_COPY) {
        load4x2(scale + c0, SC);
        load4x2(shift + c0, SH);
    }
    const bf16_t* xb = x + (int64_t)n * Hs * Ws * g.C + c0;
    const WinRect q = RING ? WinRect(ih0, iw0, IH, IW, Hs, Ws) : WinRect(IH, IW);
    if constexpr (RING) zero_ring(tile, q, IH, IW, cv, vv, pb, PLs, make_uint4(0, 0, 0, 0));
    const int npix = q.npix(), qw = q.w();
    if (npix == 0) return;
    int row = pb / qw, col = pb - row * qw;
    const int dr = PLs / qw, dc = PLs - dr * qw;
    for (; pb < npix; pb += PLs * SU) {
        uint4 u[SU];
        int px[SU];
        unsigned valid = 0;
#pragma unroll
        for (int k = 0; k < SU; ++k) {
            const int ih = ih0 + q.r0 + row, iw = iw0 + q.c0 + col;
            if constexpr (RING) px[k] = (q.r0 + row) * IW + q.c0 + col;
            u[k] = make_uint4(0, 0, 0, 0);
            if (cvalid && pb + k * PLs < npix && (RING || ((unsigned)ih < (unsigned)Hs && (unsigned)iw < (unsigned)Ws))) {
                u[k] = *reinterpret_cast<const uint4*>(xb + (uint32_t)(ih * Ws + iw) * (uint32_t)g.C);
                valid |= 1u << k;
            }
            row += dr;
            col += dc;
            if (col >= qw) { col -= qw; ++row; }
        }
#pragma unroll
        for (int k = 0; k < SU; ++k) {
            const int p = RING ? px[k] : pb + k * PLs;
            if (pb + k * PLs >= npix) break;
            uint4 v = u[k];
            if (PRO != PRO_COPY && (valid >> k & 1u)) {
                f2 z[4];
                unpack4x2(v, z);
#pragma unroll
                for (int j = 0; j < 4; ++j) z[j] = z[j] * SC[j] + SH[j];
                if constexpr (PRO == PRO_SILU) {
                    f2 t[4];
#pragma unroll
                    for (int j = 0; j < 4; ++j) t[j] = z[j] * f2{-1.4426950408889634f, -1.4426950408889634f};
#pragma unroll
                    for (int j = 0; j < 4; ++j)
                        t[j] = f2{__builtin_amdgcn_exp2f(t[j].x), __builtin_amdgcn_exp2f(t[j].y)} + f2{1.f, 1.f};
#pragma unroll
                    for (int j = 0; j < 4; ++j) t[j] = f2{__builtin_amdgcn_rcpf(t[j].x), __builtin_amdgcn_rcpf(t[j].y)};
#pragma unroll
                    for (int j = 0; j < 4; ++j) z[j] = z[j] * t[j];
                }
                v.x = pack2(z[0].x, z[0].y); v.y = pack2(z[1].x, z[1].y); v.z = pack2(z[2].x, z[2].y);
                v.w = pack2(z[3].x, z[3].y);
            }
            tile[p * cv + vv] = v;
        }
    }
}

template <int SU = DW_SU, bool RING = false>
__device__ __forceinline__ void stage_tile(uint4* tile, const bf16_t* __restrict__ x, const DwGeo& g, int n, int ih0,
                                           int iw0, int IH, int IW, int Hs, int Ws, int v0, int ncv,
                                           const float* __restrict__ scale, const float* __restrict__ shift, int act) {
    if (!scale)
        stage_tile_t<SU, PRO_COPY, RING>(tile, x, g, n, ih0, iw0, IH, IW, Hs, Ws, v0, ncv, scale, shift);
    else if (act == ACT_SILU)
        stage_tile_t<SU, PRO_SILU, RING>(tile, x, g, n, ih0, iw0, IH, IW, Hs, Ws, v0, ncv, scale, shift);
    else
        stage_tile_t<SU, PRO_AFFINE, RING>(tile, x, g, n, ih0, iw0, IH, IW, Hs, Ws, v0, ncv, scale, shift);
}

__device__ __forceinline__ void write_partials(float* red, const float (&s)[8], const float (&q)[8], int PL, int pl,
                                               int cv, int lane_cv, int ncv, int v0, int C, float* __restrict__ ps,
                                               float* __restrict__ pq) {
    __syncthreads();
    const int C8 = cv * 8;
    for (int i = threadIdx.x; i < PL * C8 * 2; i += BLOCK) red[i] = 0.f;
    __syncthreads();
    if (pl < PL) {
#pragma unroll
        for (int j = 0; j < 8; ++j) {
            red[pl * C8 + lane_cv * 8 + j] = s[j];
            red[PL * C8 + pl * C8 + lane_cv * 8 + j] = q[j];
        }
    }
    __syncthreads();
    for (int cc = threadIdx.x; cc < ncv * 8; cc += BLOCK) {
        float a = 0.f, b = 0.f;
        for (int p = 0; p < PL; ++p) {
            a += red[p * C8 + cc];
            b += red[PL * C8 + p * C8 + cc];
        }
        ps[(int64_t)blockIdx.x * C + v0 * 8 + cc] = a;
        pq[(int64_t)blockIdx.x * C + v0 * 8 + cc] = b;
    }
}

template <int EPI>
__device__ __forceinline__ void epilogue(float (&o)[8], bf16_t* __restrict__ out, int64_t off, const uint4 ypre,
                                         const float* ecl, int C8, float (&s)[8], float (&q)[8]) {
#pragma unroll
    for (int j = 0; j < 8; ++j) o[j] = bf2f(f2bf(o[j]));
    store8(out + off, o);
    if constexpr (EPI == EPI_STATS) {
#pragma unroll
        for (int j = 0; j < 8; ++j) {
            s[j] += o[j];
            q[j] = fmaf(o[j], o[j], q[j]);
        }
    } else if constexpr (EPI == EPI_BNBWD) {
        float yv[8], sc[8], sh[8], rr[8], mr[8];
        unpack8(ypre, yv);
        load8f(ecl, sc);
        load8f(ecl + C8, sh);
        load8f(ecl + 2 * C8, rr);
        load8f(ecl + 3 * C8, mr);
#pragma unroll
        for (int j = 0; j < 8; ++j) {
            const float dz = o[j] * silu_grad(fmaf(yv[j], sc[j], sh[j]));
            s[j] += dz;
            q[j] = fmaf(dz, fmaf(yv[j], rr[j], mr[j]), q[j]);
        }
    }
}

template <int K, int S, int R, int EPI, int XK = 0, bool RG = false>
__global__ __launch_bounds__(BLOCK, 3) void dw_fwd_kernel(const bf16_t* __restrict__ x, const float* __restrict__ w,
                                                       const float* __restrict__ scale,
                                                       const float* __restrict__ shift, int act, DwGeo g, int TH,
                                                       int TW, bf16_t* __restrict__ out, float* __restrict__ psum,
                                                       float* __restrict__ psq, BnBwdEpi e, XExp xe) {
    extern __shared__ __attribute__((aligned(16))) char smem[];
    const int IH = (TH - 1) * S + K, IW = (TW - 1) * S + K;
    const int cv = g.cv;
    uint4* tile = reinterpret_cast<uint4*>(smem);
    float* wl = reinterpret_cast<float*>(smem + (size_t)IH * IW * cv * 16);
    float* ecl = wl + K * K * cv * 8;
    float* red = reinterpret_cast<float*>(smem);

    const int v0 = blockIdx.y * cv;
    const int ncv = min(cv, g.nv - v0);
    const int t = threadIdx.x;
    const int lane_cv = t % cv, pl = t / cv, PL = BLOCK / cv;
    const int groups_w = TW / R;
    const StripWalk walk0(pl, PL, groups_w, S * IW * cv, R * S * cv, g.Wo * g.C, R * g.C);

    for (int i = t; i < K * K * cv * 8; i += BLOCK) {
        const int tap = i / (cv * 8), cc = i % (cv * 8);
        wl[i] = (cc < ncv * 8) ? w[(int64_t)(v0 * 8 + cc) * K * K + tap] : 0.f;
    }
    const int tiles_h = (g.Ho + TH - 1) / TH, tiles_w = (g.Wo + TW - 1) / TW;
    const int64_t ntiles = (int64_t)g.N * tiles_h * tiles_w;
    float s_acc[8], q_acc[8];
    f2 s2[4], q2[4];
#pragma unroll
    for (int j = 0; j < 4; ++j) s2[j] = q2[j] = f2{0.f, 0.f};
    stage_epi_consts<EPI>(ecl, e, v0, ncv, cv);
    if constexpr (XK != 0) {
        for (int i = t; i < cv * 8; i += BLOCK) {
            const bool ok = i < ncv * 8;
            ecl[i] = ok ? scale[v0 * 8 + i] : 0.f;
            ecl[cv * 8 + i] = ok ? shift[v0 * 8 + i] : 0.f;
        }
    }
#pragma unroll
    for (int j = 0; j < 8; ++j) s_acc[j] = q_acc[j] = 0.f;

    for (int64_t tile_id = blockIdx.x; tile_id < ntiles; tile_id += gridDim.x) {
        const int n = (int)(tile_id / (tiles_h * tiles_w));
        const int rem = (int)(tile_id - (int64_t)n * tiles_h * tiles_w);
        const int oh0 = (rem / tiles_w) * TH, ow0 = (rem % tiles_w) * TW;
        __syncthreads();
        if constexpr (XK != 0)
            stage_xmfma<xk_kc(XK), xk_ng(XK), true>(reinterpret_cast<bf16_t*>(tile), cv * 8, xe, g.H, g.W, n,
                                                    oh0 * S - g.pad, ow0 * S - g.pad, IH, IW, v0 * 8, ncv * 8, ecl);
        else
#if !(RT1_DW_TIMING & 2)
            stage_tile<DW_SU, RG>(tile, x, g, n, oh0 * S - g.pad, ow0 * S - g.pad, IH, IW, g.H, g.W, v0, ncv, scale,
                                      shift, act);
#else
            ;
#endif
        __syncthreads();
        if (lane_cv >= ncv || pl >= PL) continue;
        const int c0 = (v0 + lane_cv) * 8;
        const int64_t tbase = (((int64_t)n * g.Ho + oh0) * g.Wo + ow0) * g.C + c0;
        for (StripWalk it = walk0; it.ty < TH; it.next()) {
            const int tx = it.gx * R;
            if (oh0 + it.ty >= g.Ho) break;
            const int64_t obase = tbase + it.o2;
            constexpr bool PREF = EPI == EPI_BNBWD && !(K == 5 && S == 1);
            uint4 ypre[R];
#pragma unroll
            for (int r = 0; r < R; ++r) {
                ypre[r] = make_uint4(0, 0, 0, 0);
                if (PREF && ow0 + tx + r < g.Wo)
                    ypre[r] = *reinterpret_cast<const uint4*>(e.y + obase + (int64_t)r * g.C);
            }
            f2 acc2[R][4];
#pragma unroll
            for (int r = 0; r < R; ++r)
#pragma unroll
                for (int j = 0; j < 4; ++j) acc2[r][j] = f2{0.f, 0.f};
            const uint4* trow = tile + it.o1 + lane_cv;
            const float* wrow_p = wl + lane_cv * 8;
#if RT1_DW_TIMING & 4
#pragma unroll 1
            for (int kh = 0; kh < 0; ++kh, trow += IW * cv, wrow_p += K * cv * 8) {
#else
#pragma unroll 1
            for (int kh = 0; kh < K; ++kh, trow += IW * cv, wrow_p += K * cv * 8) {
#endif
                f2 wrow[K][4];
#pragma unroll
                for (int kw = 0; kw < K; ++kw) load4x2(wrow_p + kw * cv * 8, wrow[kw]);
                constexpr int NIN = (R - 1) * S + K;
#pragma unroll
                for (int qq = 0; qq < NIN; ++qq) {
                    f2 in[4];
                    unpack4x2(trow[qq * cv], in);
#pragma unroll
                    for (int r = 0; r < R; ++r) {
                        const int kw = qq - r * S;
                        if (kw >= 0 && kw < K) {
#pragma unroll
                            for (int j = 0; j < 4; ++j) acc2[r][j] = in[j] * wrow[kw][j] + acc2[r][j];
                        }
                    }
                }
            }
            float acc[R][8];
#pragma unroll
            for (int r = 0; r < R; ++r)
#pragma unroll
                for (int j = 0; j < 4; ++j) { acc[r][2 * j] = acc2[r][j].x; acc[r][2 * j + 1] = acc2[r][j].y; }
            if constexpr (EPI == EPI_BNBWD && !PREF) {
#pragma unroll
                for (int r = 0; r < R; ++r)
                    if (ow0 + tx + r < g.Wo) ypre[r] = *reinterpret_cast<const uint4*>(e.y + obase + (int64_t)r * g.C);
            }
#if RT1_DW_TIMING & 8
#pragma unroll
            for (int r = 0; r < R; ++r)
                if (acc[r][0] == 1234.5f) out[obase + (int64_t)r * g.C] = (bf16_t)1;
            if constexpr (false)
#endif
#pragma unroll
            for (int r = 0; r < R; ++r) {
                const int ow = ow0 + tx + r;
                if (ow >= g.Wo) continue;
                if constexpr (EPI == EPI_BNBWD) {
                    epilogue<EPI>(acc[r], out, obase + (int64_t)r * g.C, ypre[r], ecl + lane_cv * 8, cv * 8, s_acc,
                                  q_acc);
                } else {
                    const uint4 u = make_uint4(pack2(acc2[r][0].x, acc2[r][0].y), pack2(acc2[r][1].x, acc2[r][1].y),
                                               pack2(acc2[r][2].x, acc2[r][2].y), pack2(acc2[r][3].x, acc2[r][3].y));
                    *reinterpret_cast<uint4*>(out + obase + (int64_t)r * g.C) = u;
                    if constexpr (EPI == EPI_STATS) {
                        f2 v[4];
                        unpack4x2(u, v);
#pragma unroll
                        for (int j = 0; j < 4; ++j) {
                            s2[j] = s2[j] + v[j];
                            q2[j].x = fmaf(v[j].x, v[j].x, q2[j].x);
                            q2[j].y = fmaf(v[j].y, v[j].y, q2[j].y);
                        }
                    }
                }
            }
        }
    }
    if constexpr (EPI == EPI_STATS) {
#pragma unroll
        for (int j = 0; j < 4; ++j) {
            s_acc[2 * j] = s2[j].x; s_acc[2 * j + 1] = s2[j].y;
            q_acc[2 * j] = q2[j].x; q_acc[2 * j + 1] = q2[j].y;
        }
    }
    if constexpr (EPI != EPI_NONE) write_partials(red, s_acc, q_acc, PL, pl, cv, lane_cv, ncv, v0, g.C, psum, psq);
}

template <int K, int EPI>
__global__ __launch_bounds__(BLOCK, EPI == EPI_NONE ? 4 : 3) void dw_bwd_data_s2_kernel(const bf16_t* __restrict__ dy,
                                                               const float* __restrict__ w, DwGeo g, int TH, int TW,
                                                               bf16_t* __restrict__ dx, float* __restrict__ pdz,
                                                               float* __restrict__ pdzx, BnBwdEpi e) {
    extern __shared__ __attribute__((aligned(16))) char smem[];
    constexpr int R = 4;
    const int DH = (TH + K) / 2 + 1, DW = (TW + K) / 2 + 1;
    const int cv = g.cv;
    uint4* tile = reinterpret_cast<uint4*>(smem);
    float* wl = reinterpret_cast<float*>(smem + (size_t)DH * DW * cv * 16);
    float* ecl = wl + K * K * cv * 8;
    float* red = reinterpret_cast<float*>(smem);

    const int v0 = blockIdx.y * cv;
    const int ncv = min(cv, g.nv - v0);
    const int t = threadIdx.x;
    const int lane_cv = t % cv, pl = t / cv, PL = BLOCK / cv;
    const int ngroups = TH * (TW / 8) * 2;

    for (int i = t; i < K * K * cv * 8; i += BLOCK) {
        const int tap = i / (cv * 8), cc = i % (cv * 8);
        wl[i] = (cc < ncv * 8) ? w[(int64_t)(v0 * 8 + cc) * K * K + tap] : 0.f;
    }
    const int tiles_h = (g.H + TH - 1) / TH, tiles_w = (g.W + TW - 1) / TW;
    const int64_t ntiles = (int64_t)g.N * tiles_h * tiles_w;
    float s_acc[8], q_acc[8];
    stage_epi_consts<EPI>(ecl, e, v0, ncv, cv);
#pragma unroll
    for (int j = 0; j < 8; ++j) s_acc[j] = q_acc[j] = 0.f;

    for (int64_t tile_id = blockIdx.x; tile_id < ntiles; tile_id += gridDim.x) {
        const int n = (int)(tile_id / (tiles_h * tiles_w));
        const int rem = (int)(tile_id - (int64_t)n * tiles_h * tiles_w);
        const int ih0 = (rem / tiles_w) * TH, iw0 = (rem % tiles_w) * TW;
        const int oh_lo = (ih0 + g.pad - (K - 1)) >> 1;
        const int ow_lo = (iw0 + g.pad - (K - 1)) >> 1;
        __syncthreads();
        stage_tile(tile, dy, g, n, oh_lo, ow_lo, DH, DW, g.Ho, g.Wo, v0, ncv, nullptr, nullptr, 0);
        __syncthreads();
        if (lane_cv >= ncv || pl >= PL) continue;
        for (int grp = pl; grp < ngroups; grp += PL) {
            const int ty = grp / ((TW / 8) * 2);
            const int rem2 = grp % ((TW / 8) * 2);
            const int par = rem2 & 1, xb = (rem2 >> 1) * 8;
            const int ih = ih0 + ty;
            if (ih >= g.H) continue;
            const int iwb = iw0 + xb + par;
            const int c0 = (v0 + lane_cv) * 8;
            const int64_t obase = (((int64_t)n * g.H + ih) * g.W + iwb) * g.C + c0;
            uint4 ypre[R];
#pragma unroll
            for (int r = 0; r < R; ++r) {
                ypre[r] = make_uint4(0, 0, 0, 0);
                if (EPI == EPI_BNBWD && iwb + 2 * r < g.W)
                    ypre[r] = *reinterpret_cast<const uint4*>(e.y + obase + (int64_t)2 * r * g.C);
            }
            f2 acc2[R][4];
#pragma unroll
            for (int r = 0; r < R; ++r)
#pragma unroll
                for (int j = 0; j < 4; ++j) acc2[r][j] = f2{0.f, 0.f};
#pragma unroll
            for (int kh = 0; kh < K; ++kh) {
                const int nh = ih + g.pad - kh;
                if (nh & 1) continue;
                const int oh = nh >> 1;
                const uint4* trow = tile + (oh - oh_lo) * DW * cv + lane_cv;
#pragma unroll
                for (int kw = 0; kw < K; ++kw) {
                    const int nw = iwb + g.pad - kw;
                    if (nw & 1) continue;
                    const int oc = (nw >> 1) - ow_lo;
                    f2 wv[4];
                    load4x2(wl + (kh * K + kw) * cv * 8 + lane_cv * 8, wv);
#pragma unroll
                    for (int r = 0; r < R; ++r) {
                        f2 in[4];
                        unpack4x2(trow[(oc + r) * cv], in);
#pragma unroll
                        for (int j = 0; j < 4; ++j) acc2[r][j] = in[j] * wv[j] + acc2[r][j];
                    }
                }
            }
            float acc[R][8];
#pragma unroll
            for (int r = 0; r < R; ++r)
#pragma unroll
                for (int j = 0; j < 4; ++j) { acc[r][2 * j] = acc2[r][j].x; acc[r][2 * j + 1] = acc2[r][j].y; }
#pragma unroll
            for (int r = 0; r < R; ++r) {
                const int iw = iwb + 2 * r;
                if (iw < g.W)
                    epilogue<EPI>(acc[r], dx, obase + (int64_t)2 * r * g.C, ypre[r], ecl + lane_cv * 8, cv * 8, s_acc,
                                  q_acc);
            }
        }
    }
    if constexpr (EPI != EPI_NONE) write_partials(red, s_acc, q_acc, PL, pl, cv, lane_cv, ncv, v0, g.C, pdz, pdzx);
}

template <int K, int S, int R>
__global__ __launch_bounds__(BLOCK, 3) void dw_bwd_weight_kernel(const bf16_t* __restrict__ dy,
                                                              const bf16_t* __restrict__ x,
                                                              const float* __restrict__ scale,
                                                              const float* __restrict__ shift, int act, DwGeo g,
                                                              int TH, int TW, float* __restrict__ dwp) {
    extern __shared__ __attribute__((aligned(16))) char smem[];
    const int IH = (TH - 1) * S + K, IW = (TW - 1) * S + K;
    const int cv = g.cv;
    uint4* xt = reinterpret_cast<uint4*>(smem);
    uint4* dt = xt + IH * IW * cv;
    float* red = reinterpret_cast<float*>(smem);

    const int v0 = blockIdx.y * cv;
    const int ncv = min(cv, g.nv - v0);
    const int t = threadIdx.x;
    const int per = cv * K;
    const int lane_cv = t % cv, kh = (t / cv) % K, pl = t / per, PL = BLOCK / per;
    const int groups_w = TW / R;
    const StripWalk walk0(pl, PL, groups_w, S * IW * cv, R * S * cv, TW * cv, R * cv);
    const int xoff = kh * IW * cv + lane_cv;

    const int tiles_h = (g.Ho + TH - 1) / TH, tiles_w = (g.Wo + TW - 1) / TW;
    const int64_t ntiles = (int64_t)g.N * tiles_h * tiles_w;
    f2 acc2[K][4];
#pragma unroll
    for (int a = 0; a < K; ++a)
#pragma unroll
        for (int j = 0; j < 4; ++j) acc2[a][j] = f2{0.f, 0.f};

    for (int64_t tile_id = blockIdx.x; tile_id < ntiles; tile_id += gridDim.x) {
        const int n = (int)(tile_id / (tiles_h * tiles_w));
        const int rem = (int)(tile_id - (int64_t)n * tiles_h * tiles_w);
        const int oh0 = (rem / tiles_w) * TH, ow0 = (rem % tiles_w) * TW;
        __syncthreads();
        stage_tile(xt, x, g, n, oh0 * S - g.pad, ow0 * S - g.pad, IH, IW, g.H, g.W, v0, ncv, scale, shift, act);
        stage_tile<2>(dt, dy, g, n, oh0, ow0, TH, TW, g.Ho, g.Wo, v0, ncv, nullptr, nullptr, 0);
        __syncthreads();
        if (pl >= PL || lane_cv >= ncv) continue;
        for (StripWalk it = walk0; it.ty < TH; it.next()) {
            f2 d[R][4];
            const uint4* drow = dt + it.o2 + lane_cv;
#pragma unroll
            for (int r = 0; r < R; ++r) unpack4x2(drow[r * cv], d[r]);
            const uint4* xrow = xt + it.o1 + xoff;
            constexpr int NIN = (R - 1) * S + K;
#pragma unroll
            for (int qq = 0; qq < NIN; ++qq) {
                f2 in[4];
                unpack4x2(xrow[qq * cv], in);
#pragma unroll
                for (int r = 0; r < R; ++r) {
                    const int kw = qq - r * S;
                    if (kw >= 0 && kw < K) {
#pragma unroll
                        for (int j = 0; j < 4; ++j) acc2[kw][j] = d[r][j] * in[j] + acc2[kw][j];
                    }
                }
            }
        }
    }
    __syncthreads();
    const int C8 = cv * 8, KK = K * K;
    for (int i = t; i < PL * C8 * KK; i += BLOCK) red[i] = 0.f;
    __syncthreads();
    if (pl < PL && lane_cv < ncv) {
#pragma unroll
        for (int kw = 0; kw < K; ++kw)
#pragma unroll
            for (int j = 0; j < 8; ++j)
                red[(pl * C8 + lane_cv * 8 + j) * KK + kh * K + kw] = (j & 1) ? acc2[kw][j >> 1].y : acc2[kw][j >> 1].x;
    }
    __syncthreads();
    for (int i = t; i < ncv * 8 * KK; i += BLOCK) {
        float a = 0.f;
        for (int p = 0; p < PL; ++p) a += red[p * C8 * KK + i];
        dwp[(int64_t)blockIdx.x * g.C * KK + (int64_t)v0 * 8 * KK + i] = a;
    }
}

constexpr int DWF_SU = 4;

template <int K, int R, int EPI>
__global__ __launch_bounds__(BLOCK, DWF_OCC) void dw_bwd_fused_kernel(DyBnBwd d, const bf16_t* __restrict__ x1,
                                                             const float* __restrict__ scale1,
                                                             const float* __restrict__ shift1, int act1,
                                                             const float* __restrict__ wflip, DwGeo g, int TH, int TW,
                                                             bf16_t* __restrict__ dx, float* __restrict__ pdz,
                                                             float* __restrict__ pdzx, BnBwdEpi e,
                                                             float* __restrict__ dwp) {
    extern __shared__ __attribute__((aligned(16))) char smem[];
    constexpr int P = (K - 1) / 2, KK = K * K;
    const int IH = TH + K - 1, IW = TW + K - 1;
    const int cv = g.cv;
    uint4* dt = reinterpret_cast<uint4*>(smem);
    uint4* at = dt + IH * IW * cv;
    float* wl = reinterpret_cast<float*>(at + IH * IW * cv);
    float* ecl = wl + KK * cv * 8;
    float* red = reinterpret_cast<float*>(smem);

    const int v0 = blockIdx.y * cv;
    const int ncv = min(cv, g.nv - v0);
    const int t = threadIdx.x;
    const int lane_cv = t % cv, pl = t / cv, PL = BLOCK / cv;
    const int kh = (t / cv) % K, plw = t / (cv * K), PLW = BLOCK / (cv * K);
    const int groups_w = TW / R;
    const StripWalk dwalk0(pl, PL, groups_w, IW * cv, R * cv, g.W * g.C, R * g.C);
    const StripWalk wwalk0(plw, PLW, groups_w, IW * cv, R * cv, IW * cv, R * cv);
    const int aoff = kh * IW * cv + lane_cv, doff = (P * IW + P) * cv + lane_cv;

    for (int i = t; i < KK * cv * 8; i += BLOCK) {
        const int tap = i / (cv * 8), cc = i % (cv * 8);
        wl[i] = (cc < ncv * 8) ? wflip[(int64_t)(v0 * 8 + cc) * KK + tap] : 0.f;
    }
    const int tiles_h = (g.H + TH - 1) / TH, tiles_w = (g.W + TW - 1) / TW;
    const int64_t ntiles = (int64_t)g.N * tiles_h * tiles_w;
    float s_acc[8], q_acc[8];
    stage_epi_consts<EPI>(ecl, e, v0, ncv, cv);
#pragma unroll
    for (int j = 0; j < 8; ++j) s_acc[j] = q_acc[j] = 0.f;
    f2 wacc[K][4];
#pragma unroll
    for (int a = 0; a < K; ++a)
#pragma unroll
        for (int j = 0; j < 4; ++j) wacc[a][j] = f2{0.f, 0.f};

    for (int64_t tile_id = blockIdx.x; tile_id < ntiles; tile_id += gridDim.x) {
        const int n = (int)(tile_id / (tiles_h * tiles_w));
        const int rem = (int)(tile_id - (int64_t)n * tiles_h * tiles_w);
        const int oh0 = (rem / tiles_w) * TH, ow0 = (rem % tiles_w) * TW;
        __syncthreads();
        stage_dy<DWF_SU, false>(dt, d, g, n, oh0 - P, ow0 - P, IH, IW, v0, ncv);
        stage_tile(at, x1, g, n, oh0 - P, ow0 - P, IH, IW, g.H, g.W, v0, ncv, scale1, shift1, act1);
        __syncthreads();
        if (lane_cv >= ncv) continue;
        const int64_t tbase = (((int64_t)n * g.H + oh0) * g.W + ow0) * g.C + (v0 + lane_cv) * 8;
        for (StripWalk it = dwalk0; it.ty < TH; it.next()) {
            const int tx = it.gx * R;
            if (oh0 + it.ty >= g.H) break;
            const int64_t obase = tbase + it.o2;
            f2 acc2[R][4];
#pragma unroll
            for (int r = 0; r < R; ++r)
#pragma unroll
                for (int j = 0; j < 4; ++j) acc2[r][j] = f2{0.f, 0.f};
            const uint4* trow = dt + it.o1 + lane_cv;
            const float* wrow_p = wl + lane_cv * 8;
#pragma unroll 1
            for (int kr = 0; kr < K; ++kr, trow += IW * cv, wrow_p += K * cv * 8) {
                f2 wrow[K][4];
#pragma unroll
                for (int kw = 0; kw < K; ++kw) load4x2(wrow_p + kw * cv * 8, wrow[kw]);
                constexpr int NIN = R - 1 + K;
#pragma unroll
                for (int qq = 0; qq < NIN; ++qq) {
                    f2 in[4];
                    unpack4x2(trow[qq * cv], in);
#pragma unroll
                    for (int r = 0; r < R; ++r) {
                        const int kw = qq - r;
                        if (kw >= 0 && kw < K) {
#pragma unroll
                            for (int j = 0; j < 4; ++j) acc2[r][j] = in[j] * wrow[kw][j] + acc2[r][j];
                        }
                    }
                }
            }
            float acc[R][8];
#pragma unroll
            for (int r = 0; r < R; ++r)
#pragma unroll
                for (int j = 0; j < 4; ++j) { acc[r][2 * j] = acc2[r][j].x; acc[r][2 * j + 1] = acc2[r][j].y; }
            uint4 ypre[R];
#pragma unroll
            for (int r = 0; r < R; ++r) {
                ypre[r] = make_uint4(0, 0, 0, 0);
                if (EPI == EPI_BNBWD && ow0 + tx + r < g.W)
                    ypre[r] = *reinterpret_cast<const uint4*>(e.y + obase + (int64_t)r * g.C);
            }
#pragma unroll
            for (int r = 0; r < R; ++r)
                if (ow0 + tx + r < g.W)
                    epilogue<EPI>(acc[r], dx, obase + (int64_t)r * g.C, ypre[r], ecl + lane_cv * 8, cv * 8, s_acc, q_acc);
        }
        if (plw >= PLW) continue;
        for (StripWalk it = wwalk0; it.ty < TH; it.next()) {
            f2 dv[R][4];
            const uint4* drow = dt + it.o2 + doff;
#pragma unroll
            for (int r = 0; r < R; ++r) unpack4x2(drow[r * cv], dv[r]);
            const uint4* xrow = at + it.o1 + aoff;
            constexpr int NIN = R - 1 + K;
#pragma unroll
            for (int qq = 0; qq < NIN; ++qq) {
                f2 in[4];
                unpack4x2(xrow[qq * cv], in);
#pragma unroll
                for (int r = 0; r < R; ++r) {
                    const int kw = qq - r;
                    if (kw >= 0 && kw < K) {
#pragma unroll
                        for (int j = 0; j < 4; ++j) wacc[kw][j] = dv[r][j] * in[j] + wacc[kw][j];
                    }
                }
            }
        }
    }
    if constexpr (EPI != EPI_NONE) write_partials(red, s_acc, q_acc, PL, pl, cv, lane_cv, ncv, v0, g.C, pdz, pdzx);
    __syncthreads();
    const int C8 = cv * 8;
    for (int i = t; i < PLW * C8 * KK; i += BLOCK) red[i] = 0.f;
    __syncthreads();
    if (plw < PLW && lane_cv < ncv) {
#pragma unroll
        for (int kw = 0; kw < K; ++kw)
#pragma unroll
            for (int j = 0; j < 8; ++j)
                red[(plw * C8 + lane_cv * 8 + j) * KK + kh * K + kw] = (j & 1) ? wacc[kw][j >> 1].y : wacc[kw][j >> 1].x;
    }
    __syncthreads();
    for (int i = t; i < ncv * 8 * KK; i += BLOCK) {
        float a = 0.f;
        for (int p = 0; p < PLW; ++p) a += red[p * C8 * KK + i];
        dwp[(int64_t)blockIdx.x * g.C * KK + (int64_t)v0 * 8 * KK + i] = a;
    }
}

template <int EPI>
int launch_fwd(const DwPlan& p, const bf16_t* x, const float* w, const float* scale, const float* shift, int act,
               int grid_x, bf16_t* out, float* ps, float* pq, BnBwdEpi e, hipStream_t st) {
    if (p.err) return p.err;
    const DwGeo g = geo_of(p);
    dim3 grid(grid_x, p.chunks);
#define L(KK, SS, RR)                                                                                               \
    if (p.k == KK && p.s == SS && p.R == RR) {                                                                      \
        if (p.ring)                                                                                                 \
            hipLaunchKernelGGL((dw_fwd_kernel<KK, SS, RR, EPI, 0, true>), grid, dim3(BLOCK), p.lds, st, x, w,       \
                               scale, shift, act, g, p.TH, p.TW, out, ps, pq, e, XExp{nullptr, nullptr, 0});        \
        else                                                                                                        \
            hipLaunchKernelGGL((dw_fwd_kernel<KK, SS, RR, EPI>), grid, dim3(BLOCK), p.lds, st, x, w, scale, shift,  \
                               act, g, p.TH, p.TW, out, ps, pq, e, XExp{nullptr, nullptr, 0});                      \
        return (int)hipGetLastError();                                                                              \
    }
    L(3, 1, 5) L(3, 1, DW_R1) L(3, 2, 2) L(5, 1, 5) L(5, 1, DW_R1) L(5, 2, 2)
#undef L
    return (int)hipErrorInvalidValue;
}

}

int rt1::dw::launch_bwd_twopass(const DwPlan& p, const DyBnBwd& d, const bf16_t* x1, const float* scale1,
                                const float* shift1, int act1, const float* wflip, int grid_x, bf16_t* dx, float* pdz,
                                float* pdzx, const BnBwdEpi& e, bool epi, float* dwp, hipStream_t st) {
    const DwGeo g = geo_of(p);
    const int k = p.k;
    dim3 grid(grid_x, p.chunks);
#define L(KK, EE)                                                                                                   \
    hipLaunchKernelGGL((dw_bwd_fused_kernel<KK, DW_R1, EE>), grid, dim3(BLOCK), p.lds, st, d, x1, scale1, shift1,   \
                       act1, wflip, g, p.TH, p.TW, dx, pdz, pdzx, e, dwp)
    if (k == 3) { if (epi) L(3, EPI_BNBWD); else L(3, EPI_NONE); }
    else if (k == 5) { if (epi) L(5, EPI_BNBWD); else L(5, EPI_NONE); }
    else return (int)hipErrorInvalidValue;
#undef L
    return (int)hipGetLastError();
}

extern "C" {

int rt1_dw_fwd(const bf16_t* x, const float* w, const float* scale, const float* shift, int act, int N, int H, int W,
               int C, int k, int s, int grid_x, bf16_t* out, float* psum, float* psq, hipStream_t st) {
    const DwPlan p = dw_plan(OP_FWD, N, H, W, C, k, s, scale != nullptr, 0, 0, 0, grid_x);
    BnBwdEpi e{nullptr, nullptr, nullptr, nullptr, nullptr, 0};
    return psum ? launch_fwd<EPI_STATS>(p, x, w, scale, shift, act, grid_x, out, psum, psq, e, st)
                : launch_fwd<EPI_NONE>(p, x, w, scale, shift, act, grid_x, out, psum, psq, e, st);
}

int rt1_dw_bwd_data(const bf16_t* dy, const float* w, const float* wflip, int N, int H, int W, int C, int k, int s,
                    int grid_x, bf16_t* dx, const bf16_t* y_in, const float* scale, const float* shift,
                    const float* mean, const float* rstd, float* pdz, float* pdzx, hipStream_t st) {
    const int epi = y_in != nullptr;
    const DwPlan p = dw_plan(OP_BWD_DATA, N, H, W, C, k, s, 0, epi, 0, 0, grid_x);
    BnBwdEpi e{y_in, scale, shift, mean, rstd, 0};
    if (p.kind == TK_FWD)
        return epi ? launch_fwd<EPI_BNBWD>(p, dy, wflip, nullptr, nullptr, 0, grid_x, dx, pdz, pdzx, e, st)
                   : launch_fwd<EPI_NONE>(p, dy, wflip, nullptr, nullptr, 0, grid_x, dx, pdz, pdzx, e, st);
    if (p.err) return p.err;
    const DwGeo g = geo_of(p);
    dim3 grid(grid_x, p.chunks);
#define L(KK, EE)                                                                                                   \
    hipLaunchKernelGGL((dw_bwd_data_s2_kernel<KK, EE>), grid, dim3(BLOCK), p.lds, st, dy, w, g, p.TH, p.TW, dx, pdz, \
                       pdzx, e)
    if (k == 3) { if (epi) L(3, EPI_BNBWD); else L(3, EPI_NONE); }
    else if (k == 5) { if (epi) L(5, EPI_BNBWD); else L(5, EPI_NONE); }
    else return (int)hipErrorInvalidValue;
#undef L
    return (int)hipGetLastError();
}

int rt1_dw_fwd_x(const bf16_t* x, int cin, const bf16_t* we, const float* w, const float* scale1, const float* shift1,
                 int N, int H, int W, int C, int k, int s, int grid_x, bf16_t* out, float* psum, float* psq,
                 hipStream_t st) {
    const DwPlan p = dw_plan(OP_FWD_X, N, H, W, C, k, s, 1, 0, 0, cin, grid_x);
    if (p.err || !scale1 || !shift1 || !psum || !psq) return (int)hipErrorInvalidValue;
    const DwGeo g = geo_of(p);
    const BnBwdEpi e{nullptr, nullptr, nullptr, nullptr, nullptr, 0};
    const XExp xe{x, we, cin};
    dim3 grid(grid_x, p.chunks);
#define L(KK, SS, RR, XX)                                                                                           \
    if (p.k == KK && p.s == SS && p.xk == XX && p.R == RR) {                                                        \
        hipLaunchKernelGGL((dw_fwd_kernel<KK, SS, RR, EPI_STATS, XX>), grid, dim3(BLOCK), p.lds, st, nullptr, w,    \
                           scale1, shift1, (int)ACT_SILU, g, p.TH, p.TW, out, psum, psq, e, xe);                    \
        return (int)hipGetLastError();                                                                              \
    }
#define X1(KK, XX) L(KK, 1, DW_R1, XX)
#define X2(KK, XX) L(KK, 2, 2, XX)
    DW_XMODE_S1(X1) DW_XMODE_S2(X2)
#undef X2
#undef X1
#undef L
    return (int)hipErrorInvalidValue;
}

int rt1_dw_bwd_weight(const bf16_t* dy, const bf16_t* x, const float* scale, const float* shift, int act, int N, int H,
                      int W, int C, int k, int s, int grid_x, float* dwp, hipStream_t st) {
    const DwPlan p = dw_plan(OP_BWD_WEIGHT, N, H, W, C, k, s, scale != nullptr, 0, 0, 0, grid_x);
    if (p.err) return p.err;
    const DwGeo g = geo_of(p);
    dim3 grid(grid_x, p.chunks);
#define L(KK, SS, RR)                                                                                               \
    hipLaunchKernelGGL((dw_bwd_weight_kernel<KK, SS, RR>), grid, dim3(BLOCK), p.lds, st, dy, x, scale, shift, act, \
                       g, p.TH, p.TW, dwp)
    if (k == 3 && s == 1) L(3, 1, DW_R1);
    else if (k == 3 && s == 2) L(3, 2, 2);
    else if (k == 5 && s == 1) L(5, 1, DW_R1);
    else if (k == 5 && s == 2) L(5, 2, 2);
    else return (int)hipErrorInvalidValue;
#undef L
    return (int)hipGetLastError();
}

}
```

### pytorch_rt1_for_distributed_training_amd/csrc/kernels/dw_plan.hip

```cpp
#include <algorithm>
#include <array>
#include <unordered_map>

#include "dw/dw_common.h"

using namespace rt1;
using namespace rt1::dw;

namespace {

constexpr int DW_RING_PIX = 2000;
constexpr int DW_FULLROW_MAX = 18;

DwGeo make_geo(int N, int H, int W, int C, int k, int s) {
    DwGeo g;
    g.N = N; g.H = H; g.W = W; g.C = C; g.k = k; g.s = s; g.pad = (k - 1) / 2;
    g.Ho = (H + 2 * g.pad - k) / s + 1;
    g.Wo = (W + 2 * g.pad - k) / s + 1;
    g.nv = C / 8;
    g.cv = g.nv;
    if (g.nv > 8) {
        g.cv = 8;
        const int slots8 = (g.nv + 7) / 8 * 8;
        if (slots8 * 100 > g.nv * 115) {
            int slots = slots8;
            for (int cv = 7; cv >= 4; --cv) {
                const int sl = (g.nv + cv - 1) / cv * cv;
                if (sl < slots) { slots = sl; g.cv = cv; }
            }
        }
    }
    if (g.nv <= DW_FULLROW_MAX) g.cv = g.nv;
    if (g.nv == 36) g.cv = 12;
    g.chunks = (g.nv + g.cv - 1) / g.cv;
    return g;
}

inline int cdiv(int a, int b) { return (a + b - 1) / b; }

int xk_of(int cin, int C, int k, int s) {
    const DwGeo g = make_geo(1, 8, 8, C, k, s);
    const int C8 = g.cv * 8, kc = (cin + 31) / 32, ng = C8 / 16;
    if (cin <= 0 || cin % 8 || kc > 2 || C8 % 16 || ng > 15) return 0;
    return kc * 16 + ng;
}

bool x_supported(int k, int s, int xk) {
#define X(KK, XX) if (k == KK && xk == XX) return true;
    if (s == 1) { DW_XMODE_S1(X) } else { DW_XMODE_S2(X) }
#undef X
    return false;
}

constexpr int DW_R5_MASK = 1;
constexpr int DWU2_MAX_PIX = 400;
inline int uni_kind(int K, int xk, int H, int W) {
    if (K == 5 && xk == 0 && H * W <= DWU2_MAX_PIX) return TK_BWD_U2;
    return (K == 3 ? DWU_CPT3 : DWU_CPT5) == 4 ? TK_BWD_U4 : TK_BWD_U8;
}
inline bool is_uni2(int kind) { return kind == TK_BWD_V4 || kind == TK_BWD_V8; }
inline bool r5_fits(int W, int xk, int bit) { return xk == 0 && W > 0 && W % 5 == 0 && W % 4 != 0 && (DW_R5_MASK & bit); }
inline int uni_r(int K, int W, int xk, int cpt) {
    if (K == 5 && cpt == 2 && xk == 0 && W > 0 && W % 5 == 0 && W % 4 != 0) return 5;
    return K == 3 ? DWU_R3 : (r5_fits(W, xk, 2) ? 5 : DWU_R5);
}
inline int uni2_kind(int K) { return (K == 3 ? DWV_CPT3 : DWV_CPT5) == 4 ? TK_BWD_V4 : TK_BWD_V8; }
inline int uni2_r(int K) { return K == 3 ? DWV_R3 : DWV_R5; }
inline int kind_cpt(int kind) {
    return kind == TK_BWD_U2 ? 2 : (kind == TK_BWD_U4 || kind == TK_BWD_V4) ? 4 : 8;
}
inline bool use_uni(int variant, bool pro, bool epi) {
    if (pro != epi) return false;
    return variant != 0;
}
inline int fwd_r(int S, int Wo, int xk) { return S == 1 && r5_fits(Wo, xk, 1) ? 5 : DW_R1; }
struct TileChoice { int TH, TW, sb = 0; };

constexpr size_t LDS_BUDGET = DW_LDS_KB * 1024;

size_t tile_lds(int kind, int K, int S, int cv, bool epi, int R, int TH, int TW, int xk, int sb) {
    const size_t ec = epi ? (size_t)cv * 8 * 4 * 4 : 0;
    const size_t ypix = is_uni2(kind) ? (size_t)(TH / 2) * (TW / 2) : (sb > 0 ? (size_t)sb * R : (size_t)TH * TW);
    const size_t xt = xk ? ypix * cv * 16 + (size_t)cv * 8 * ((xk >> 4) * 32 + 8) * 2 : 0;
    if (kind == TK_FWD) {
        const int IH = (TH - 1) * S + K, IW = (TW - 1) * S + K;
        const size_t a = (size_t)IH * IW * cv * 16 + (size_t)K * K * cv * 8 * 4 + ec + (xk ? (size_t)cv * 8 * 2 * 4 : 0);
        const size_t red = (size_t)(BLOCK / cv) * cv * 8 * 2 * 4;
        return a > red ? a : red;
    }
    if (kind == TK_BWD_W) {
        const int IH = (TH - 1) * S + K, IW = (TW - 1) * S + K;
        const size_t a = (size_t)IH * IW * cv * 16 + (size_t)TH * TW * cv * 16;
        const size_t red = (size_t)(BLOCK / (cv * K)) * cv * 8 * K * K * 4;
        return a > red ? a : red;
    }
    if (is_uni2(kind)) {
        const int DH = (TH + K) / 2 + 1, DW = (TW + K) / 2 + 1, cpt = kind_cpt(kind);
        const size_t a = (size_t)DH * DW * cv * 16 + (size_t)K * K * cv * 8 * 4 + ec + xt;
        const size_t red = (size_t)(BLOCK / (cv * 8 / cpt)) * cv * 8 * 2 * 4;
        return a > red ? a : red;
    }
    if (is_uni(kind)) {
        const int IH = TH + K - 1, IW = TW + K - 1, cpt = kind_cpt(kind);
        const size_t cs = (!xk && centre_stage_on(cpt, R)) ? (size_t)TH * TW * cv * 16 : 0;
        const size_t a = (size_t)IH * IW * cv * 16 + (size_t)K * K * cv * 8 * 4 + ec + xt + cs;
        const size_t red = (size_t)(BLOCK / (cv * 8 / cpt)) * cv * 8 * 2 * 4;
        return a > red ? a : red;
    }
    if (kind == TK_BWD_F) {
        const int IH = TH + K - 1, IW = TW + K - 1;
        const size_t a = 2 * (size_t)IH * IW * cv * 16 + (size_t)K * K * cv * 8 * 4 + ec;
        const size_t r1 = (size_t)(BLOCK / cv) * cv * 8 * 2 * 4, r2 = (size_t)(BLOCK / (cv * K)) * cv * 8 * K * K * 4;
        const size_t red = r1 > r2 ? r1 : r2;
        return a > red ? a : red;
    }
    const int DH = (TH + K) / 2 + 1, DW = (TW + K) / 2 + 1;
    const size_t a = (size_t)DH * DW * cv * 16 + (size_t)K * K * cv * 8 * 4 + ec;
    const size_t red = (size_t)(BLOCK / cv) * cv * 8 * 2 * 4;
    return a > red ? a : red;
}

TileChoice search_tile(int kind, int R, int Ho, int Wo, int K, int S, int cv, bool pro, bool epi, int xk) {
    const bool uni = is_uni(kind);
    const bool uni2 = is_uni2(kind);
    const int NIN = (R - 1) * S + K;
    const int wstep = kind == TK_BWD_S2 ? 8 : uni2 ? 2 * R : R, hstep = (kind == TK_BWD_S2 || uni2) ? 2 : 1;
    int slots, strip;
    if (kind == TK_FWD) {
        slots = BLOCK / cv;
        strip = K * (8 * NIN + 4 * R * K + 12) + R * (epi ? 60 : 24);
    } else if (kind == TK_BWD_W) {
        slots = BLOCK / (cv * K);
        strip = 8 * R + 8 * NIN + 4 * R * K + 12;
    } else if (uni2) {
        const int cpt = kind_cpt(kind), kh = (K + 1) / 2;
        slots = BLOCK / (cv * 8 / cpt);
        strip = kh * ((R + kh - 1) * (cpt + 2) + R * kh * cpt) + R * (epi ? 14 * cpt : 2 * cpt);
    } else if (uni) {
        const int cpt = kind_cpt(kind);
        slots = BLOCK / (cv * 8 / cpt);
        strip = K * (NIN * (cpt + 2) + R * K * cpt) + R * (epi ? 14 * cpt : 2 * cpt);
    } else if (kind == TK_BWD_F) {
        slots = BLOCK / cv;
        strip = K * (8 * NIN + 4 * R * K + 12) + R * (epi ? 60 : 24) + K * (8 * R + 8 * NIN + 4 * R * K + 12);
    } else {
        slots = BLOCK / cv;
        const int taps = ((K + 1) / 2) * ((K + 1) / 2);
        strip = taps * (4 * 8 + 4 * 4 + 4) + R * (epi ? 60 : 24);
    }
    const int stage = (uni || uni2) ? 110 : kind == TK_BWD_F ? (pro ? 90 : 30) + 110 : (pro ? 90 : 30);
    const size_t budget = kind == TK_BWD_U2 ? (size_t)DWU2_LDS_KB * 1024
                        : (uni || uni2) ? (size_t)DWU_LDS_KB * 1024
                              : kind == TK_BWD_F ? (size_t)DWF_LDS_KB * 1024 : LDS_BUDGET;
    const int wmax = (Wo + wstep - 1) / wstep * wstep;
    const int hmax = (Ho + hstep - 1) / hstep * hstep;
    TileChoice best{hstep, wstep};
    double best_cost = 1e300;
    const int nrmax = (xk && uni) ? 6 : 0;
    for (int TW = wstep; TW <= wmax && TW <= 40; TW += wstep) {
        for (int TH = hstep; TH <= hmax && TH <= 40; TH += hstep) {
          bool fits_any = false;
          for (int nr = nrmax; nr >= 0; --nr) {
            const int all = TH * (TW / R);
            const int sbv = nr > 0 ? nr * slots : 0;
            if (nr > 0 && sbv >= all) continue;
            if (tile_lds(kind, K, S, cv, epi, R, TH, TW, xk, sbv) > budget) continue;
            fits_any = true;
            const int nb = sbv > 0 ? cdiv(all, sbv) : 1;
            const int tiles = cdiv(Ho, TH) * cdiv(Wo, TW);
            int strips, staged;
            if (uni2) {
                strips = TH * (TW / R) / 2;
                staged = ((TH + K) / 2 + 1) * ((TW + K) / 2 + 1) * cv;
            } else if (uni) {
                strips = TH * (TW / R);
                staged = (TH + K - 1) * (TW + K - 1) * cv;
            } else if (kind == TK_FWD || kind == TK_BWD_F) {
                strips = TH * (TW / R);
                staged = ((TH - 1) * S + K) * ((TW - 1) * S + K) * cv;
            } else if (kind == TK_BWD_W) {
                strips = TH * (TW / R);
                staged = ((TH - 1) * S + K) * ((TW - 1) * S + K) * cv + TH * TW * cv;
            } else {
                strips = TH * (TW / 8) * 2;
                staged = ((TH + K) / 2 + 1) * ((TW + K) / 2 + 1) * cv;
            }
            const int xstage = (xk && (uni || uni2)) ? cdiv(TH * TW * cv, BLOCK) * 40 + (uni2 ? 4 : nb) * 100 : 0;
            const double cost = (double)tiles * ((double)cdiv(strips, slots) * strip +
                                                 (double)cdiv(staged, BLOCK) * stage + xstage + 150.0);
            if (cost < best_cost * 0.999) {
                best_cost = cost;
                best = TileChoice{TH, TW, sbv};
            }
          }
          if (!fits_any) break;
        }
    }
    return best;
}

int clamp_grid(int64_t tiles, int max_blocks_x) {
    int64_t gx = tiles < max_blocks_x ? tiles : max_blocks_x;
    return (int)(gx < 1 ? 1 : gx);
}

constexpr int DW_WG_TARGET = 3072;
constexpr int DW_CAP_MIN_CHUNKS = 8;
int chunk_cap(int max_blocks_x, int chunks) {
    if (DW_WG_TARGET <= 0 || chunks < DW_CAP_MIN_CHUNKS) return max_blocks_x;
    const int cap = (DW_WG_TARGET + chunks - 1) / chunks;
    return cap < max_blocks_x ? cap : max_blocks_x;
}

DwPlan plan_frame(int op, int H, int W, int C, int k, int s, bool pro, bool epi, bool unified, int cin, int& tiles) {
    if (op == OP_BWD_FUSED_S1) s = 1;
    if (op == OP_BWD_FUSED_S2) s = 2;
    const DwGeo g = make_geo(1, H, W, C, k, s);
    DwPlan p{};
    p.N = 1; p.H = H; p.W = W; p.C = C; p.Ho = g.Ho; p.Wo = g.Wo; p.k = k; p.s = s; p.pad = g.pad;
    p.nv = g.nv; p.cv = g.cv; p.chunks = g.chunks;
    p.cpt = 8;
    bool ok = (k == 3 || k == 5) && (s == 1 || s == 2);
    int mh = g.Ho, mw = g.Wo, S = s;
    switch (op) {
    case OP_FWD_X:
        p.xk = xk_of(cin, C, k, s);
        ok = ok && x_supported(k, s, p.xk);
        [[fallthrough]];
    case OP_FWD:
        p.kind = TK_FWD;
        p.R = s == 1 ? fwd_r(s, g.Wo, p.xk) : 2;
        p.ring = op == OP_FWD && H * W <= DW_RING_PIX;
        break;
    case OP_BWD_DATA:
        mh = H; mw = W; pro = false;
        if (s == 1) {
            p.kind = TK_FWD;
            p.R = fwd_r(1, W, 0);
            p.ring = g.Ho * g.Wo <= DW_RING_PIX;
        } else {
            p.kind = TK_BWD_S2;
            p.R = 4;
            S = 2;
        }
        break;
    case OP_BWD_WEIGHT:
        p.kind = TK_BWD_W;
        p.R = s == 1 ? DW_R1 : 2;
        epi = false;
        break;
    case OP_BWD_FUSED_S1: {
        mh = H; mw = W;
        const bool uni = use_uni(unified ? 1 : 0, pro, epi);
        p.xk = (cin > 0 && uni) ? xk_of(cin, C, k, 1) : 0;
        p.kind = uni ? uni_kind(k, p.xk, H, W) : TK_BWD_F;
        p.cpt = kind_cpt(p.kind);
        p.R = uni ? uni_r(k, W, p.xk, p.cpt) : DW_R1;
        p.ring = uni && H * W <= DW_RING_PIX;
        if (cin > 0) ok = ok && uni && epi && x_supported(k, 1, p.xk);
        break;
    }
    case OP_BWD_FUSED_S2:
        mh = H; mw = W; pro = epi;
        p.xk = cin > 0 ? xk_of(cin, C, k, 2) : 0;
        p.kind = uni2_kind(k);
        p.cpt = kind_cpt(p.kind);
        p.R = uni2_r(k);
        p.ring = g.Ho * g.Wo <= DW_RING_PIX;
        if (cin > 0) ok = ok && epi && x_supported(k, 2, p.xk);
        break;
    default:
        ok = false;
        p.kind = TK_FWD;
        p.R = DW_R1;
    }
    const TileChoice tc = search_tile(p.kind, p.R, mh, mw, k, S, g.cv, pro, epi, p.xk);
    p.TH = tc.TH; p.TW = tc.TW; p.sb = tc.sb;
    if (op == OP_BWD_FUSED_S2 && ((tc.TH & 1) || (tc.TW % (2 * p.R)))) ok = false;
    p.lds = (int)tile_lds(p.kind, k, S, g.cv, epi, p.R, tc.TH, tc.TW, p.xk, tc.sb);
    if (is_uni(p.kind) || is_uni2(p.kind)) {
        const size_t per_tap = (size_t)(BLOCK / (g.cv * 8 / p.cpt)) * g.cv * 8 * 4;
        p.red_taps = (int)std::min<size_t>((size_t)k * k, (size_t)p.lds / per_tap);
    }
    tiles = cdiv(mh, tc.TH) * cdiv(mw, tc.TW);
    p.err = ok ? 0 : (int)hipErrorInvalidValue;
    return p;
}

}

namespace rt1 {
namespace dw {

DwPlan dw_plan(int op, int N, int H, int W, int C, int k, int s, int pro, int epi, int variant, int cin,
               int max_blocks_x) {
    typedef std::array<int, 10> Key;
    struct Hash {
        size_t operator()(const Key& a) const {
            size_t h = 1469598103934665603ull;
            for (int v : a) h = (h ^ (size_t)(unsigned)v) * 1099511628211ull;
            return h;
        }
    };
    struct Entry { DwPlan p; int tiles; };
    thread_local std::unordered_map<Key, Entry, Hash> memo;
    const Key key{op, H, W, C, k, s, pro != 0, epi != 0, variant != 0, cin};
    auto it = memo.find(key);
    if (it == memo.end()) {
        Entry e;
        e.p = plan_frame(op, H, W, C, k, s, pro != 0, epi != 0, variant != 0, cin, e.tiles);
        it = memo.emplace(key, e).first;
    }
    DwPlan p = it->second.p;
    p.N = N;
    p.grid_x = clamp_grid((int64_t)N * it->second.tiles, chunk_cap(max_blocks_x, p.chunks));
    return p;
}

}
}

extern "C" {

int rt1_dw_grid(int N, int H, int W, int C, int k, int s, int max_blocks_x, int pro, int epi) {
    return dw_plan(OP_FWD, N, H, W, C, k, s, pro, epi, 0, 0, max_blocks_x).grid_x;
}

int rt1_dw_wgrad_grid(int N, int H, int W, int C, int k, int s, int max_blocks_x, int pro) {
    return dw_plan(OP_BWD_WEIGHT, N, H, W, C, k, s, pro, 0, 0, 0, max_blocks_x).grid_x;
}

int rt1_dw_bwd_grid(int N, int H, int W, int C, int k, int s, int max_blocks_x, int epi) {
    return dw_plan(OP_BWD_DATA, N, H, W, C, k, s, 0, epi, 0, 0, max_blocks_x).grid_x;
}

int rt1_dw_bwd_fused_grid(int N, int H, int W, int C, int k, int max_blocks_x, int pro, int epi, int variant,
                          int cin) {
    return dw_plan(OP_BWD_FUSED_S1, N, H, W, C, k, 1, pro, epi, variant, cin, max_blocks_x).grid_x;
}

int rt1_dw_bwd_fused_s2_grid(int N, int H, int W, int C, int k, int max_blocks_x, int epi, int cin) {
    return dw_plan(OP_BWD_FUSED_S2, N, H, W, C, k, 2, epi, epi, 1, cin, max_blocks_x).grid_x;
}

int rt1_dw_grid_x(int N, int H, int W, int C, int k, int s, int cin, int max_blocks_x) {
    return dw_plan(OP_FWD_X, N, H, W, C, k, s, 1, 0, 0, cin, max_blocks_x).grid_x;
}

int rt1_dw_bwd_uses_uni(int variant, int pro, int epi) { return use_uni(variant, pro != 0, epi != 0) ? 1 : 0; }

int rt1_dw_x_supported(int cin, int C, int k, int s) { return dw_plan(OP_FWD_X, 1, 8, 8, C, k, s, 1, 0, 0, cin, 1).err == 0; }

int rt1_dw_tile_info(int which, int H, int W, int C, int k, int s, int cin, int* out) {
    const DwPlan p = which == 0 ? dw_plan(cin > 0 ? OP_FWD_X : OP_FWD, 1, H, W, C, k, s, 1, 0, 0, cin, 1)
                                : dw_plan(s == 2 ? OP_BWD_FUSED_S2 : OP_BWD_FUSED_S1, 1, H, W, C, k, s, 1, 1, 1, cin, 1);
    if (cin > 0 && !p.xk) return (int)hipErrorInvalidValue;
    out[0] = p.TH;
    out[1] = p.TW;
    out[2] = p.lds;
    out[3] = p.sb;
    return 0;
}

}
```

### pytorch_rt1_for_distributed_training_amd/csrc/rt1_kernels.h

```cpp
#pragma once
#include <hip/hip_runtime.h>
#include <stdint.h>

extern "C" {

int rt1_flat_adam(float* p, const float* g, float* m, float* v, int64_t n, float lr, float beta1, float beta2,
                  float eps, float weight_decay, float step_size, float inv_sqrt_bc2, float grad_scale,
                  hipStream_t stream);
int rt1_flat_adam_dev(float* p, const float* g, float* m, float* v, int64_t n, const float* state, float beta1,
                      float beta2, float eps, float weight_decay, float grad_scale, hipStream_t stream);
int rt1_flat_adam_clip_dev(float* p, const float* g, float* m, float* v, int64_t n, const float* state,
                           const float* clip_state, float beta1, float beta2, float eps, float weight_decay,
                           float grad_scale, hipStream_t stream);
int rt1_flat_adam_ema_dev(float* p, const float* g, float* m, float* v, float* ema, int64_t n, const float* state,
                          const float* clip_state, float* ema_state, float beta1, float beta2, float eps,
                          float weight_decay, float grad_scale, float one_minus_decay, int warmup,
                          hipStream_t stream);
int rt1_flat_adam_groups_dev(float* p, const float* g, float* m, float* v, float* ema, int64_t n, const float* state,
                             const float* group_state, const uint8_t* chunk_group, int G, const float* clip_state,
                             float* ema_state, float beta1, float beta2, float eps, float grad_scale,
                             float one_minus_decay, int warmup, hipStream_t stream);

int rt1_gradnorm_partials(int64_t n);
int rt1_grad_sumsq(const float* g, int64_t n, double* partials, hipStream_t stream);
int rt1_grad_clip_finalize(const double* partials, int P, float max_norm, float grad_scale, int skip_nonfinite,
                           float* clip_state, hipStream_t stream);
int rt1_buffer_guard(float* buf, float* shadow, int64_t n, const float* clip_state, hipStream_t stream);

}

extern "C" {
typedef uint16_t rt1_bf16;

int rt1_bn_stats(const rt1_bf16* x, int64_t M, int C, int P, float* psum, float* psq, hipStream_t st);
int rt1_bn_finalize(const float* psum, const float* psq, int P, int C, double count, const float* gamma,
                    const float* beta, float eps, float momentum, float* running_mean, float* running_var,
                    float* scale, float* shift, float* save_mean, float* save_rstd, hipStream_t st);
int rt1_bn_apply(const rt1_bf16* y, int64_t M, int C, const float* scale, const float* shift, int act, const float* rs,
                 int64_t HW, rt1_bf16* out, hipStream_t st);
int rt1_bn_bwd_reduce(const rt1_bf16* G, const float* rs, const float* rb, int64_t HW, const rt1_bf16* y, int64_t M,
                      int C, const float* scale, const float* shift, const float* mean, const float* rstd, int act,
                      int P, float* pdz, float* pdzx, hipStream_t st);
int rt1_bn_bwd_finalize_consts(const float* pdz, const float* pdzx, int P, int C, double count, float* dgamma,
                               float* dbeta, float* mdz, float* mdzx, const float* scale, const float* shift,
                               const float* gamma, const float* mean, const float* rstd, float* consts,
                               hipStream_t st);
int rt1_bn_bwd_finalize(const float* pdz, const float* pdzx, int P, int C, double count, float* dgamma, float* dbeta,
                        float* mdz, float* mdzx, hipStream_t st, int accumulate);
int rt1_bn_bwd_apply(const rt1_bf16* G, const float* rs, const float* rb, int64_t HW, const rt1_bf16* y, int64_t M,
                     int C, const float* scale, const float* shift, const float* mean, const float* rstd,
                     const float* gamma, int act, const float* mdz, const float* mdzx, rt1_bf16* dy, hipStream_t st,
                     const float* keep = nullptr);

int rt1_dw_grid(int N, int H, int W, int C, int k, int s, int max_blocks_x, int pro, int epi);
int rt1_dw_wgrad_grid(int N, int H, int W, int C, int k, int s, int max_blocks_x, int pro);
int rt1_dw_bwd_grid(int N, int H, int W, int C, int k, int s, int max_blocks_x, int epi);
int rt1_dw_fwd(const rt1_bf16* x, const float* w, const float* scale, const float* shift, int act, int N, int H, int W,
               int C, int k, int s, int grid_x, rt1_bf16* out, float* psum, float* psq, hipStream_t st);
int rt1_dw_bwd_data(const rt1_bf16* dy, const float* w, const float* wflip, int N, int H, int W, int C, int k, int s,
                    int grid_x,
                    rt1_bf16* dx, const rt1_bf16* y_in, const float* scale, const float* shift, const float* mean,
                    const float* rstd, float* pdz, float* pdzx, hipStream_t st);
int rt1_dw_bwd_weight(const rt1_bf16* dy, const rt1_bf16* x, const float* scale, const float* shift, int act, int N,
                      int H, int W, int C, int k, int s, int grid_x, float* dwp, hipStream_t st);
int rt1_dw_bwd_uses_uni(int variant, int pro, int epi);
int rt1_dw_bwd_fused_s2_grid(int N, int H, int W, int C, int k, int max_blocks_x, int epi, int cin);
int rt1_dw_bwd_fused_s2(const rt1_bf16* dA, const rt1_bf16* y2, const float* gate, const float* rb,
                        const float* scale2, const float* shift2, const float* mean2, const float* rstd2,
                        const float* gamma2, const float* mdz2, const float* mdzx2, const float* w,
                        const rt1_bf16* x1, const float* scale1, const float* shift1, const float* mean1,
                        const float* rstd1, int N, int H, int W, int C, int k, int grid_x, rt1_bf16* dx, float* pdz,
                        float* pdzx, float* dwp, hipStream_t st, int zout, const rt1_bf16* xin,
                        const rt1_bf16* we, int cin);
int rt1_dw_bwd_fused_grid(int N, int H, int W, int C, int k, int max_blocks_x, int pro, int epi, int variant,
                          int cin);
int rt1_dw_bwd_fused(const rt1_bf16* dA, const rt1_bf16* y2, const float* gate, const float* rb, const float* scale2,
                     const float* shift2, const float* mean2, const float* rstd2, const float* gamma2,
                     const float* mdz2, const float* mdzx2, const float* w, const float* wflip, const rt1_bf16* x1,
                     const float* scale1,
                     const float* shift1, int act1, const float* mean1, const float* rstd1, int N, int H, int W, int C,
                     int k, int grid_x, rt1_bf16* dx, float* pdz, float* pdzx, float* dwp, hipStream_t st,
                     int variant, int zout, const rt1_bf16* xin, const rt1_bf16* we, int cin,
                     const rt1_bf16* res = nullptr, const float* rmul = nullptr);
int rt1_dw_x_supported(int cin, int C, int k, int s);
int rt1_dw_grid_x(int N, int H, int W, int C, int k, int s, int cin, int max_blocks_x);
int rt1_dw_tile_info(int which, int H, int W, int C, int k, int s, int cin, int* out);
int rt1_dw_fwd_x(const rt1_bf16* x, int cin, const rt1_bf16* we, const float* w, const float* scale1,
                 const float* shift1, int N, int H, int W, int C, int k, int s, int grid_x, rt1_bf16* out, float* psum,
                 float* psq, hipStream_t st);
int rt1_gemm_tiles_m(int M, int N, int K, int cfg);
int rt1_gemm_cmap(const rt1_bf16* A, int lda, const rt1_bf16* B, float* C, int M, int N, int K, const float* bias,
                  const int* cmap, int cfg, hipStream_t st);
int rt1_gemm(const rt1_bf16* A, const rt1_bf16* B, void* C, int M, int N, int K, int nn, const float* bias,
             const float* scale, const float* shift, const float* gate, int hw, int out_f32, float* ps, float* pq,
             int cfg, rt1_bf16* aout, hipStream_t st);
int rt1_gemm_tail(const rt1_bf16* A, const rt1_bf16* B, int M, int N, int K, const rt1_bf16* A2, const rt1_bf16* B2,
                  int K2, const float* bias, const rt1_bf16* res, const float* rmul, int rhw, rt1_bf16* C, int cfg,
                  hipStream_t st);
int rt1_g256_tiles_m(int M);
int rt1_g256(const rt1_bf16* A, const rt1_bf16* B, rt1_bf16* C, int M, int N, int K, int nn, const float* bias,
             const float* scale, const float* shift, const float* gate, int hw, rt1_bf16* aout, float* ps, float* pq,
             int bn, hipStream_t st);
int rt1_xgram_grid(int64_t M, int cin);
int rt1_xgram(const rt1_bf16* x, int64_t M, int cin, int grid, float* work, double* out, hipStream_t st);
int rt1_bn_from_gram(const double* G, const double* sx, const rt1_bf16* we, int cin, int C, double count,
                     const float* gamma, const float* beta, float eps, float momentum, float* running_mean,
                     float* running_var, float* scale, float* shift, float* save_mean, float* save_rstd,
                     hipStream_t st);
int rt1_bn_from_wg(const float* WG, const float* sx, const rt1_bf16* we, int cin, int C, double count,
                         const float* gamma, const float* beta, float eps, float momentum, float* running_mean,
                         float* running_var, float* scale, float* shift, float* save_mean, float* save_rstd,
                         hipStream_t st);

int rt1_frame_splits(int N, int HW, int C);
int rt1_frame_pool(const rt1_bf16* y, const rt1_bf16* G, int N, int HW, int C, const float* scale, const float* shift,
                   int act, int splits, float* pool, hipStream_t st);
int rt1_se_bn_bwd_reduce(const rt1_bf16* G, const rt1_bf16* y, int N, int HW, int C, const float* scale,
                         const float* shift, const float* mean, const float* rstd, int splits, float* out,
                         hipStream_t st);
int rt1_block_tail(const rt1_bf16* y3, int64_t M, int HW, int C, const float* scale, const float* shift,
                   const float* keep, const rt1_bf16* skip, const float* fmul, const float* fadd, rt1_bf16* out,
                   hipStream_t st);
int rt1_tail_bwd_reduce(const rt1_bf16* dout, const rt1_bf16* y3, int N, int HW, int C, const float* scale,
                        const float* shift, const float* mean, const float* rstd, const float* keep,
                        const rt1_bf16* skip, const float* fmul, int splits, float* dmul, float* dadd, float* pdz,
                        float* pdzx, hipStream_t st);

int rt1_stem_grid(int N, int H, int W, int max_blocks);
int rt1_stem_fwd(const void* img, int img_is_u8, const int* shift, const float* w, int N, int H, int W, int Cout,
                 int grid, rt1_bf16* out, float* psum, float* psq, hipStream_t st);
int rt1_stem_bwd_weight(const void* img, int img_is_u8, const int* shift, const rt1_bf16* dy, int N, int H, int W,
                        int Cout, int grid, float* dwp, hipStream_t st, const rt1_bf16* bn_x = nullptr,
                        const float* bn_scale = nullptr, const float* bn_shift = nullptr,
                        const float* bn_mean = nullptr, const float* bn_rstd = nullptr,
                        const float* bn_gamma = nullptr, const float* bn_mdz = nullptr,
                        const float* bn_mdzx = nullptr);

int rt1_attn_fwd(const rt1_bf16* qkv, rt1_bf16* out, float* lse, int B, int S, int H, int L, int Kimg, float scale,
                 float drop_p, uint32_t seed, const uint32_t* seed_dev, hipStream_t st);
int rt1_attn_keepmask(uint8_t* keep, int BH, int S, float drop_p, uint32_t seed, const uint32_t* seed_dev,
                      hipStream_t st);
int rt1_attn_bwd(const rt1_bf16* qkv, const rt1_bf16* out, const rt1_bf16* dout, const float* lse, rt1_bf16* dqkv,
                 int B, int S, int H, int L, int Kimg, float scale, float drop_p, uint32_t seed,
                 const uint32_t* seed_dev, hipStream_t st);

int rt1_attn_bwd_long(const rt1_bf16* qkv, const rt1_bf16* out, const rt1_bf16* dout, const float* lse,
                      rt1_bf16* dqkv, int B, int S, int H, int L, int Kimg, float scale, float drop_p, uint32_t seed,
                      const uint32_t* seed_dev, hipStream_t st);

int rt1_action_tokenize(const void* const* comps, const int* kind, const int* dim, int n, const float* low,
                        const float* high, int rows, int V, int64_t* out64, int* out32, hipStream_t st);
int rt1_head_ce_supported(int V, int E);
int rt1_head_ce_fwd(const float* hidden, const int* pos, const rt1_bf16* W, const float* bias, const int* target,
                    int R, int P, int S, int V, float* ce, int* pred, rt1_bf16* G, rt1_bf16* hb, hipStream_t st);
int rt1_head_ce_scale(const rt1_bf16* G, const float* dce, int R, int V, rt1_bf16* dz, hipStream_t st);

int rt1_tl_supported(int P, int C, int h1, int t);
int rt1_tl_fwd(const rt1_bf16* x, const float* gamma, const float* beta, float eps, const rt1_bf16* W1, const float* b1,
               const float* W2, const float* b2, int N, int P, rt1_bf16* out, float* mu, float* rs, rt1_bf16* z1,
               float* s, hipStream_t st);
int rt1_tl_bwd(const rt1_bf16* x, const rt1_bf16* dO, const float* s, const rt1_bf16* z1, const float* mu,
               const float* rs, const float* gamma, const float* beta, const rt1_bf16* W1T, const float* W2, int N,
               int P, rt1_bf16* dx, rt1_bf16* dz1, rt1_bf16* xn, float* pw2, float* pg, hipStream_t st);


int rt1_add_scaled(rt1_bf16* x, const rt1_bf16* y, const float* sc, int64_t M, int HW, int C, hipStream_t st);

int rt1_pw_gemm_supported(int K, int N);
int rt1_pw_gemm_grid(int M, int K, int N, int max_blocks);
int rt1_pw_gemm(const rt1_bf16* A, const rt1_bf16* B, int M, int K, int N, rt1_bf16* C, float* ps, float* pq,
                int max_blocks, const float* scale, const float* shift, const float* gate, int hw, rt1_bf16* aout,
                hipStream_t st);
int rt1_pw_gemm_bnbwd_supported(int K, int N);
int rt1_pw_gemm_bnbwd(const rt1_bf16* dout, const rt1_bf16* B, int M, int K, int N, rt1_bf16* C, int max_blocks,
                      const rt1_bf16* y, const float* fmul, const float* keep, int hw, const float* gamma,
                      const float* mean, const float* rstd, const float* mdz, const float* mdzx, rt1_bf16* dy_out,
                      hipStream_t st);

int rt1_tf_grid(int T);
int rt1_ln_fwd(const float* x, const float* g, const float* b, int T, float eps, rt1_bf16* y, float* mu, float* rs,
               hipStream_t st);
int rt1_ln_bwd(const rt1_bf16* dy, const float* x, const float* mu, const float* rs, const float* g, const float* dres,
               int T, float* dx, float* dgp, float* dbp, rt1_bf16* dxb, float* dsp, int grid, hipStream_t st);
int rt1_resid(const float* x, const rt1_bf16* a, const float* bias, int T, float p, uint32_t seed,
              const uint32_t* seed_dev, float* out, const float* lg, const float* lb, float eps, rt1_bf16* xn, float* mu,
              float* rs, hipStream_t st);
int rt1_drop_bwd(const float* dout, int T, float p, uint32_t seed, const uint32_t* seed_dev, rt1_bf16* dh, float* dbp,
                 int grid, hipStream_t st);

int rt1_se_part_size(int N, int C, int S);
int rt1_se_fwd(const float* pool_sum, float inv_hw, int N, int C, int S, const float* w1, const float* b1,
               const float* w2, const float* b2, float* part, float* h, float* gate, hipStream_t st);
int rt1_se_bwd_frame(const float* dsum, const float* gate, const float* h, float inv_hw, int N, int C, int S,
                     const float* w1, const float* w2, float* part, float* dh, float* rb, hipStream_t st);
size_t rt1_se_wsum_ws_bytes(int N, int C, int S);
int rt1_se_bwd_wsum(const float* red, const float* gate, const float* h, const float* dh, const float* pool,
                    const float* rb, int N, int C, int S, float inv_hw, double count, void* ws, float* dw2,
                    float* dw1, float* db2, float* db1, float* sdz, float* sdzx, float* mdz, float* mdzx,
                    hipStream_t st);
int rt1_se_bwd_dz(const float* dsum, const float* gate, int N, int C, float* dz, float* db, hipStream_t st);
int rt1_se_bwd_dh(const float* dzf2, const float* h, int N, int S, float* dh, float* db, hipStream_t st);
int rt1_se_bwd_bnsum(const float* red, const float* gate, const float* rbraw, float inv_hw, int N, int C, double count,
                     float* rb, float* sdz, float* sdzx, float* mdz, float* mdzx, hipStream_t st);

int rt1_pw_tall_supported(int K, int N);
int rt1_pw_tall_preferred(int K, int N);
int rt1_pw_tall(const rt1_bf16* A, const rt1_bf16* W, int M, int K, int N, rt1_bf16* C, const float* scale,
                const float* shift, const float* gate, int hw, rt1_bf16* aout, hipStream_t st);
int rt1_embed_fwd(const rt1_bf16* A, const rt1_bf16* W, const float* bias, const float* pos, int M, int K, int N, int S,
                  float* out, hipStream_t st);

int rt1_pw_wide_supported(int K, int N);
int rt1_pw_wide(const rt1_bf16* A, const rt1_bf16* B, int M, int K, int N, rt1_bf16* C, int max_blocks, hipStream_t st);

int rt1_colsum_chunks(int64_t R, int C, int B);
int rt1_multi_copy(const float* const* src, float* const* dst, const int64_t* n, int count, hipStream_t st);
int rt1_multi_reduce_copy(const float* const* src, float* const* dst, const int64_t* n, const int64_t* sstride,
                          const int* splits, int count, hipStream_t st);
int rt1_multi_add(const float* const* src, float* const* dst, const int64_t* n, int count, hipStream_t st);
int rt1_multi_reduce_add(const float* const* src, float* const* dst, const int64_t* n, const int64_t* sstride,
                         const int* splits, int count, hipStream_t st);
int rt1_colsum(const void* in, int in_is_bf16, int64_t R, int C, int B, float* out, float* tmp, int chunks,
               hipStream_t st);

int rt1_crop_resize_u8(const uint8_t* raw, const int* boxes, int N, int h, int w, int H, int W, uint8_t* out,
                       hipStream_t st);
int rt1_crop_resize_gather_u8(const uint8_t* raw, int64_t F, const int64_t* rows, const int* boxes, int N, int h,
                              int w, int H, int W, uint8_t* out, hipStream_t st);

int rt1_wgrad_splits(int64_t M, int Co, int Ci, int variant);
int rt1_wgrad_run(const rt1_bf16* dy, const rt1_bf16* a, int64_t M, int Co, int Ci, const float* scale,
                  const float* shift, const float* gate, int act, int hw, int splits, float* out, int variant,
                  int sums, hipStream_t st);
int rt1_wgrad_dymap(const float* dyf, const int* map, const rt1_bf16* a, int64_t M, int Co, int Ci, int splits,
                    float* out, float* dbout, int tile, hipStream_t st);

int rt1_proj_bwd_supported(int Cout, int Ce);
int rt1_proj_bwd_fsplit(int N, int HW, int Ce);
int rt1_proj_bwd_frame(const rt1_bf16* dy, const rt1_bf16* y, int N, int HW, int Cout, int Ce, const float* scale,
                       const float* shift, const float* mean, const float* rstd, const rt1_bf16* Wp, int fsplit,
                       float* G, float* R, hipStream_t st);
int rt1_proj_bwd_finalize(const float* G, const float* R, const float* gate, int N, int Cout, int Ce, int fsplit,
                          float* red, float* dW, hipStream_t st);

int rt1_pw_bwd_supported(int CE, int CIN);
int rt1_pw_bwd_grid(int M, int max_blocks);
int rt1_pw_bwd(const rt1_bf16* dA, const rt1_bf16* y, const rt1_bf16* x, const rt1_bf16* We, const float* consts,
               int M, int CE, int CIN, rt1_bf16* dx, const rt1_bf16* dout, const float* fmul, int HW, float* dwp,
               int grid, hipStream_t st);
int rt1_pw_bwd_z_width(int CE, int CIN);
int rt1_pw_bwd_z_mk_elems(int CIN);
int rt1_pw_bwd_z(const rt1_bf16* dz, const rt1_bf16* x, const rt1_bf16* We, const float* consts, int M, int CE,
                 int CIN, rt1_bf16* mk, float* r0, rt1_bf16* dx, const rt1_bf16* dout, const float* fmul, int HW,
                 float* part, int grid, hipStream_t st);
int rt1_pw_tall_tail(const rt1_bf16* A, const rt1_bf16* W, int M, int K, int N, const rt1_bf16* A2, const rt1_bf16* W2,
                     int K2, const float* bias, const rt1_bf16* res, const float* rmul, int rhw, rt1_bf16* C,
                     hipStream_t st);
int rt1_pw_z_prep(const rt1_bf16* We, const float* consts, int CE, int CIN, rt1_bf16* wt, rt1_bf16* mk, float* r0,
                  hipStream_t st);
int rt1_pw_z_finish(const float* S, int splits, const float* G, const float* sx, const rt1_bf16* We,
                    const float* consts, int CE, int CIN, float* dWe, hipStream_t st);
int rt1_pw_bwd_z_finish(const float* S, const rt1_bf16* We, const float* consts, int CE, int CIN, float* dWe,
                        hipStream_t st);

}
```

### pytorch_rt1_for_distributed_training_amd/ops/_ext.py

```python
from __future__ import annotations

import importlib
import importlib.util
import os
import sys

_MOD = None
_ERR = None
HERE = os.path.dirname(os.path.abspath(__file__))
PKG = os.path.dirname(HERE)


def load():
    global _MOD, _ERR
    if _MOD is not None:
        return _MOD
    try:
        import torch
        alt = os.environ.get("RT1_HIP_SO")
        if alt:
            name = "pytorch_rt1_for_distributed_training_amd._rt1_hip"
            spec = importlib.util.spec_from_file_location(name, alt)
            _MOD = importlib.util.module_from_spec(spec)
            spec.loader.exec_module(_MOD)
            sys.modules[name] = _MOD
            return _MOD
        _MOD = importlib.import_module("pytorch_rt1_for_distributed_training_amd._rt1_hip")
    except ImportError as e:
        _ERR = e
        raise ImportError(
            "HIP extension _rt1_hip is not built. Run `python build.py` (hipcc --offload-arch=gfx950) "
            f"in the repo root. Original error: {e}") from e
    return _MOD


def available() -> bool:
    try:
        load()
        return True
    except ImportError:
        return False
```

### pytorch_rt1_for_distributed_training_amd/ops/switches.py

```python
from __future__ import annotations

import os
from typing import Dict

DEFAULTS: Dict[str, str] = {
    "pw_tall": "1",
    "g256": "1",
    "wgrad_mfma": "1",
    "wgrad_deep": "1",
    "dw_fused": "1",
    "dw_s2_fused": "1",
    "dw_variant": "1",
    "dw_res": "1",
    "pw_pro": "1",
    "proj_bwd": "1",
    "se_fused": "1",
    "stem_in_block0": "1",
    "stem_bn_bwd": "1",
    "pw_bwd_z": "1",
    "pw_z_wide": "1",
    "z_gemm": "1",
    "xmode": "1",
    "gram_bn": "1",
    "gemm_proj": "1",
    "gemm_proj_dgrad": "1",
    "tall_res": "1",
    "gram_sx": "1",
    "tf_wgrad": "1",
    "tf_gemm": "1",
    "tf_fuse_ln": "1",
    "multi_copy": "1",
}


def _parse(spec: str) -> Dict[str, str]:
    out: Dict[str, str] = {}
    for item in filter(None, (s.strip() for s in spec.split(","))):
        name, sep, value = item.partition("=")
        name = name.strip()
        if not sep or name not in DEFAULTS:
            raise ValueError(f"RT1_AB: unknown or malformed switch {item!r}; known: {', '.join(sorted(DEFAULTS))}")
        out[name] = value.strip()
    return out


_OVERRIDES = _parse(os.environ.get("RT1_AB", ""))


def get(name: str) -> str:
    if name not in DEFAULTS:
        raise KeyError(name)
    return _OVERRIDES.get(name, DEFAULTS[name])


def on(name: str) -> bool:
    return get(name) != "0"


def overrides() -> Dict[str, str]:
    return dict(_OVERRIDES)
```

Measured before the change: 1438 samples/s.

## Walk depthwise tiles column-wise and carry overlapping halo rows in LDS

Depthwise conv forward and backward kernels now walk tiles down contiguous columns per workgroup instead of grid-strided order. When the previous tile sits directly above, the overlapping halo rows are copied within LDS rather than reloaded from global memory, so only the new rows are staged. A planner heuristic enables this only when the overlap is a large enough share of the tile. The cost is an extra LDS copy plus a barrier per tile, and a different work distribution that could hurt load balance or L2 locality.

```diff
diff --git a/pytorch_rt1_for_distributed_training_amd/csrc/bindings.cpp b/pytorch_rt1_for_distributed_training_amd/csrc/bindings.cpp
--- a/pytorch_rt1_for_distributed_training_amd/csrc/bindings.cpp
+++ b/pytorch_rt1_for_distributed_training_amd/csrc/bindings.cpp
@@ -1533,6 +1533,7 @@
     m.def("bn_from_gram", &bn_from_gram);
     m.def("dw_x_supported", &dw_x_supported);
     m.def("dw_tile_info", &dw_tile_info);
+    m.def("dw_set_carry", [](bool on) { return rt1_dw_set_carry(on ? 1 : 0) != 0; });
     m.def("dw_fwd_x", &dw_fwd_x);
     m.def("dw_bwd_fused_x", &dw_bwd_fused_x, py::arg("dA"), py::arg("y2"), py::arg("gate"), py::arg("rb"),
           py::arg("sc2"), py::arg("sh2"), py::arg("mu2"), py::arg("rs2"), py::arg("g2"), py::arg("mdz2"),
diff --git a/pytorch_rt1_for_distributed_training_amd/csrc/kernels/dw/dw_plan.h b/pytorch_rt1_for_distributed_training_amd/csrc/kernels/dw/dw_plan.h
--- a/pytorch_rt1_for_distributed_training_amd/csrc/kernels/dw/dw_plan.h
+++ b/pytorch_rt1_for_distributed_training_amd/csrc/kernels/dw/dw_plan.h
@@ -37,10 +37,80 @@
     int lds;
     int red_taps;
     int grid_x;
+    int carry;
 };
 
 DwPlan dw_plan(int op, int N, int H, int W, int C, int k, int s, int pro, int epi, int variant, int cin,
                int max_blocks_x);
 
+
+int dw_carry();
+
+constexpr int WALK_COLUMNS = 1, WALK_CARRY = 2;
+inline int walk_mode(const DwPlan& p) { return p.carry ? (WALK_COLUMNS | (dw_carry() ? WALK_CARRY : 0)) : 0; }
+
+#if defined(__HIPCC__) || defined(__CUDACC__)
+#define DW_HD __host__ __device__ __forceinline__
+#else
+#define DW_HD inline
+#endif
+struct TileWalk {
+    struct Pos {
+        int n, tc, tr;
+        int above;
+    };
+    long long first;
+    int count;
+    int tiles_h, tiles_w;
+    int step;
+    DW_HD TileWalk(int wg, int grid, int N, int tiles_h_, int tiles_w_, bool columns = true)
+        : tiles_h(tiles_h_), tiles_w(tiles_w_), step(columns ? 0 : grid) {
+        const long long total = (long long)N * tiles_h_ * tiles_w_;
+        if (columns) {
+            const long long base = total / grid, rem = total - base * grid;
+            first = wg * base + (wg < rem ? wg : rem);
+            count = (int)(base + (wg < rem ? 1 : 0));
+        } else {
+            first = wg;
+            count = wg < total ? (int)((total - wg + grid - 1) / grid) : 0;
+        }
+    }
+    DW_HD Pos at(int i) const {
+        Pos p;
+        if (step == 0) {
+            const long long idx = first + i;
+            const long long col = idx / tiles_h;
+            p.tr = (int)(idx - col * tiles_h);
+            p.n = (int)(col / tiles_w);
+            p.tc = (int)(col - (long long)p.n * tiles_w);
+            p.above = i > 0 && p.tr > 0;
+        } else {
+            const long long idx = first + (long long)i * step;
+            const int per = tiles_h * tiles_w;
+            p.n = (int)(idx / per);
+            const int rem = (int)(idx - (long long)p.n * per);
+            p.tr = rem / tiles_w;
+            p.tc = rem - p.tr * tiles_w;
+            p.above = 0;
+        }
+        return p;
+    }
+    DW_HD void advance(Pos& p, int i) const {
+        if (step != 0) {
+            p = at(i + 1);
+            return;
+        }
+        p.above = 1;
+        if (++p.tr == tiles_h) {
+            p.tr = 0;
+            p.above = 0;
+            if (++p.tc == tiles_w) {
+                p.tc = 0;
+                ++p.n;
+            }
+        }
+    }
+};
+
 }
 }
diff --git a/pytorch_rt1_for_distributed_training_amd/csrc/kernels/dw/dw_stage.h b/pytorch_rt1_for_distributed_training_amd/csrc/kernels/dw/dw_stage.h
--- a/pytorch_rt1_for_distributed_training_amd/csrc/kernels/dw/dw_stage.h
+++ b/pytorch_rt1_for_distributed_training_amd/csrc/kernels/dw/dw_stage.h
@@ -83,6 +83,15 @@
         }
         tile[px * lanes + vv] = zero;
     }
+}
+
+__device__ __forceinline__ int carry_rows(uint4* tile, bool on, int o, int IH, int IW, int cv) {
+    if (!on || o <= 0 || 2 * o > IH) return 0;
+    const int nvec = o * IW * cv;
+    const uint4* src = tile + (IH - o) * IW * cv;
+    for (int i = threadIdx.x; i < nvec; i += BLOCK) tile[i] = src[i];
+    __syncthreads();
+    return o;
 }
 
 typedef short bf16x8 __attribute__((ext_vector_type(8)));
@@ -223,8 +232,11 @@
 
 template <int SU, bool RING>
 __device__ __forceinline__ void stage_dy(uint4* tile, const DyBnBwd& d, const DwGeo& g, int n, int ih0, int iw0,
-                                         int IH, int IW, int v0, int ncv) {
+                                         int IH, int IW, int v0, int ncv, int r_begin = 0) {
     const int cv = g.cv;
+    tile += r_begin * IW * cv;
+    ih0 += r_begin;
+    IH -= r_begin;
     const int t = threadIdx.x;
     const int vv = t % cv, PLs = BLOCK / cv;
     int pb = t / cv;
diff --git a/pytorch_rt1_for_distributed_training_amd/csrc/kernels/dw_bwd_s1.hip b/pytorch_rt1_for_distributed_training_amd/csrc/kernels/dw_bwd_s1.hip
--- a/pytorch_rt1_for_distributed_training_amd/csrc/kernels/dw_bwd_s1.hip
+++ b/pytorch_rt1_for_distributed_training_amd/csrc/kernels/dw_bwd_s1.hip
@@ -14,8 +14,11 @@
 
 template <int SU, bool RING>
 __device__ __forceinline__ void stage_dy_half(uint4* tile, const DyBnBwd& d, const DwGeo& g, int n, int ih0, int iw0,
-                                              int IH, int IW, int v0, int ncv) {
+                                              int IH, int IW, int v0, int ncv, int r_begin = 0) {
     const int cv = g.cv, ch = 2 * cv;
+    tile += r_begin * IW * cv;
+    ih0 += r_begin;
+    IH -= r_begin;
     const int t = threadIdx.x;
     const int hv = t % ch, PLs = BLOCK / ch;
     int pb = t / ch;
@@ -146,7 +149,7 @@
                                                                         bf16_t* __restrict__ dx, float* __restrict__ pdz,
                                                                         float* __restrict__ pdzx,
                                                                         float* __restrict__ dwp, int red_taps, XExp xe,
-                                                                        int sb) {
+                                                                        int sb, int walk) {
     using CV = ChanVec<CPT>;
     using V = typename CV::T;
     constexpr int P = (K - 1) / 2, KK = K * K, NV = CPT / 2, HPV = 8 / CPT;
@@ -177,7 +180,6 @@
     }
     stage_epi_consts<EPI>(ecl, e, v0, ncv, cv);
     const int tiles_h = (g.H + TH - 1) / TH, tiles_w = (g.W + TW - 1) / TW;
-    const int64_t ntiles = (int64_t)g.N * tiles_h * tiles_w;
     f2 wacc[KK][NV], s_acc[NV], q_acc[NV];
 #pragma unroll
     for (int j = 0; j < NV; ++j) {
@@ -187,11 +189,12 @@
     }
 
     constexpr bool CS = XK == 0 && centre_stage_on(CPT, R);
-    for (int64_t tile_id = blockIdx.x; tile_id < ntiles; tile_id += gridDim.x) {
-        const int n = (int)(tile_id / (tiles_h * tiles_w));
-        const int rem = (int)(tile_id - (int64_t)n * tiles_h * tiles_w);
-        const int oh0 = (rem / tiles_w) * TH, ow0 = (rem % tiles_w) * TW;
-        __syncthreads();
+    const TileWalk tiles(blockIdx.x, gridDim.x, g.N, tiles_h, tiles_w, walk & WALK_COLUMNS);
+    TileWalk::Pos tp = tiles.at(0);
+    for (int ti = 0; ti < tiles.count; tiles.advance(tp, ti), ++ti) {
+        const int n = tp.n, oh0 = tp.tr * TH, ow0 = tp.tc * TW;
+        __syncthreads();
+        const int rb = carry_rows(dt, (walk & WALK_CARRY) && tp.above, K - 1, IH, IW, cv);
         if constexpr (CS) {
             const int nvec = TH * TW * cv, lane = t & 63;
             const bf16_t* fb = x1 + (int64_t)n * g.H * g.W * g.C;
@@ -207,8 +210,8 @@
             }
         }
 #if !(RT1_DW_TIMING & 2)
-        if constexpr (CPT == 2) stage_dy_half<DWU2_SU, RG>(dt, d, g, n, oh0 - P, ow0 - P, IH, IW, v0, ncv);
-        else stage_dy<DWU_SU, RG>(dt, d, g, n, oh0 - P, ow0 - P, IH, IW, v0, ncv);
+        if constexpr (CPT == 2) stage_dy_half<DWU2_SU, RG>(dt, d, g, n, oh0 - P, ow0 - P, IH, IW, v0, ncv, rb);
+        else stage_dy<DWU_SU, RG>(dt, d, g, n, oh0 - P, ow0 - P, IH, IW, v0, ncv, rb);
 #endif
         if constexpr (CS) asm volatile("s_waitcnt vmcnt(0)" ::: "memory");
         const int nstrips = TH * groups_w, sbw = (XK != 0 && sb > 0) ? sb : nstrips;
@@ -454,7 +457,7 @@
         const XExp xe{xin, we, cin};
 #define LU1(KK, RR, EE, CC, XX, RGV)                                                                                \
     hipLaunchKernelGGL((dw_bwd_uni_kernel<KK, RR, EE, CC, XX, RGV>), grid, dim3(BLOCK), p.lds, st, d, x1, w, g,      \
-                       p.TH, p.TW, e, dx, pdz, pdzx, dwp, p.red_taps, xe, p.sb)
+                       p.TH, p.TW, e, dx, pdz, pdzx, dwp, p.red_taps, xe, p.sb, walk_mode(p))
 #define LU(KK, RR, EE, CC, XX)                                                                                      \
     if (p.k == KK && p.R == RR && epi == (EE == EPI_BNBWD) && p.cpt == CC && p.xk == XX) {                          \
         if (p.ring) LU1(KK, RR, EE, CC, XX, true); else LU1(KK, RR, EE, CC, XX, false);                             \
diff --git a/pytorch_rt1_for_distributed_training_amd/csrc/kernels/dw_bwd_s2.hip b/pytorch_rt1_for_distributed_training_amd/csrc/kernels/dw_bwd_s2.hip
--- a/pytorch_rt1_for_distributed_training_amd/csrc/kernels/dw_bwd_s2.hip
+++ b/pytorch_rt1_for_distributed_training_amd/csrc/kernels/dw_bwd_s2.hip
@@ -134,7 +134,7 @@
                                                                            float* __restrict__ pdz,
                                                                            float* __restrict__ pdzx,
                                                                            float* __restrict__ dwp, int red_taps,
-                                                                           XExp xe) {
+                                                                           XExp xe, int walk) {
     constexpr int P = (K - 1) / 2, KK = K * K, NV = CPT / 2, HPV = 8 / CPT;
     static_assert(XK == 0 || EPI == EPI_BNBWD, "x-mode is for expand blocks (BN1 epilogue)");
     extern __shared__ __attribute__((aligned(16))) char smem[];
@@ -164,7 +164,6 @@
     }
     stage_epi_consts<EPI>(ecl, e, v0, ncv, cv);
     const int tiles_h = (g.H + TH - 1) / TH, tiles_w = (g.W + TW - 1) / TW;
-    const int64_t ntiles = (int64_t)g.N * tiles_h * tiles_w;
     f2 wacc[KK][NV], s_acc[NV], q_acc[NV];
 #pragma unroll
     for (int j = 0; j < NV; ++j) {
@@ -172,13 +171,14 @@
 #pragma unroll
         for (int a = 0; a < KK; ++a) wacc[a][j] = f2{0.f, 0.f};
     }
-    for (int64_t tile_id = blockIdx.x; tile_id < ntiles; tile_id += gridDim.x) {
-        const int n = (int)(tile_id / (tiles_h * tiles_w));
-        const int rem = (int)(tile_id - (int64_t)n * tiles_h * tiles_w);
-        const int ih0 = (rem / tiles_w) * TH, iw0 = (rem % tiles_w) * TW;
+    const TileWalk tiles(blockIdx.x, gridDim.x, g.N, tiles_h, tiles_w, walk & WALK_COLUMNS);
+    TileWalk::Pos tp = tiles.at(0);
+    for (int ti = 0; ti < tiles.count; tiles.advance(tp, ti), ++ti) {
+        const int n = tp.n, ih0 = tp.tr * TH, iw0 = tp.tc * TW;
         const int oh_lo = (ih0 + P - (K - 1)) >> 1, ow_lo = (iw0 + P - (K - 1)) >> 1;
         __syncthreads();
-        stage_dy<DWU_SU, RG>(dt, d, go, n, oh_lo, ow_lo, DH, DW, v0, ncv);
+        const int rb = carry_rows(dt, (walk & WALK_CARRY) && tp.above, DH - TH / 2, DH, DW, cv);
+        stage_dy<DWU_SU, RG>(dt, d, go, n, oh_lo, ow_lo, DH, DW, v0, ncv, rb);
         const int64_t tbase = (((int64_t)n * g.H + ih0) * g.W + iw0) * g.C + v0 * 8 + cofs;
         if constexpr (XK != 0) {
 #define CLS(PR_, PC_)                                                                                              \
@@ -277,7 +277,7 @@
     const XExp xe{xin, we, cin};
 #define LV1(KK, RR, EE, CC, XX, RGV)                                                                                \
     hipLaunchKernelGGL((dw_bwd_uni_s2_kernel<KK, RR, EE, CC, XX, RGV>), grid, dim3(BLOCK), p.lds, st, d, x1, w, g,   \
-                       p.TH, p.TW, e, dx, pdz, pdzx, dwp, p.red_taps, xe)
+                       p.TH, p.TW, e, dx, pdz, pdzx, dwp, p.red_taps, xe, walk_mode(p))
 #define LV(KK, RR, EE, CC, XX)                                                                                      \
     if (p.k == KK && p.R == RR && epi == (EE == EPI_BNBWD) && p.cpt == CC && p.xk == XX) {                          \
         if (p.ring) LV1(KK, RR, EE, CC, XX, true); else LV1(KK, RR, EE, CC, XX, false);                             \
diff --git a/pytorch_rt1_for_distributed_training_amd/csrc/kernels/dw_fwd.hip b/pytorch_rt1_for_distributed_training_amd/csrc/kernels/dw_fwd.hip
--- a/pytorch_rt1_for_distributed_training_amd/csrc/kernels/dw_fwd.hip
+++ b/pytorch_rt1_for_distributed_training_amd/csrc/kernels/dw_fwd.hip
@@ -10,8 +10,12 @@
 template <int SU, int PRO, bool RING>
 __device__ __forceinline__ void stage_tile_t(uint4* tile, const bf16_t* __restrict__ x, const DwGeo& g, int n, int ih0,
                                              int iw0, int IH, int IW, int Hs, int Ws, int v0, int ncv,
-                                             const float* __restrict__ scale, const float* __restrict__ shift) {
+                                             const float* __restrict__ scale, const float* __restrict__ shift,
+                                             int r_begin) {
     const int cv = g.cv;
+    tile += r_begin * IW * cv;
+    ih0 += r_begin;
+    IH -= r_begin;
     const int t = threadIdx.x;
     const int vv = t % cv, PLs = BLOCK / cv;
     int pb = t / cv;
@@ -80,13 +84,14 @@
 template <int SU = DW_SU, bool RING = false>
 __device__ __forceinline__ void stage_tile(uint4* tile, const bf16_t* __restrict__ x, const DwGeo& g, int n, int ih0,
                                            int iw0, int IH, int IW, int Hs, int Ws, int v0, int ncv,
-                                           const float* __restrict__ scale, const float* __restrict__ shift, int act) {
+                                           const float* __restrict__ scale, const float* __restrict__ shift, int act,
+                                           int r_begin = 0) {
     if (!scale)
-        stage_tile_t<SU, PRO_COPY, RING>(tile, x, g, n, ih0, iw0, IH, IW, Hs, Ws, v0, ncv, scale, shift);
+        stage_tile_t<SU, PRO_COPY, RING>(tile, x, g, n, ih0, iw0, IH, IW, Hs, Ws, v0, ncv, scale, shift, r_begin);
     else if (act == ACT_SILU)
-        stage_tile_t<SU, PRO_SILU, RING>(tile, x, g, n, ih0, iw0, IH, IW, Hs, Ws, v0, ncv, scale, shift);
+        stage_tile_t<SU, PRO_SILU, RING>(tile, x, g, n, ih0, iw0, IH, IW, Hs, Ws, v0, ncv, scale, shift, r_begin);
     else
-        stage_tile_t<SU, PRO_AFFINE, RING>(tile, x, g, n, ih0, iw0, IH, IW, Hs, Ws, v0, ncv, scale, shift);
+        stage_tile_t<SU, PRO_AFFINE, RING>(tile, x, g, n, ih0, iw0, IH, IW, Hs, Ws, v0, ncv, scale, shift, r_begin);
 }
 
 __device__ __forceinline__ void write_partials(float* red, const float (&s)[8], const float (&q)[8], int PL, int pl,
@@ -148,7 +153,7 @@
                                                        const float* __restrict__ scale,
                                                        const float* __restrict__ shift, int act, DwGeo g, int TH,
                                                        int TW, bf16_t* __restrict__ out, float* __restrict__ psum,
-                                                       float* __restrict__ psq, BnBwdEpi e, XExp xe) {
+                                                       float* __restrict__ psq, BnBwdEpi e, XExp xe, int walk) {
     extern __shared__ __attribute__((aligned(16))) char smem[];
     const int IH = (TH - 1) * S + K, IW = (TW - 1) * S + K;
     const int cv = g.cv;
@@ -169,7 +174,6 @@
         wl[i] = (cc < ncv * 8) ? w[(int64_t)(v0 * 8 + cc) * K * K + tap] : 0.f;
     }
     const int tiles_h = (g.Ho + TH - 1) / TH, tiles_w = (g.Wo + TW - 1) / TW;
-    const int64_t ntiles = (int64_t)g.N * tiles_h * tiles_w;
     float s_acc[8], q_acc[8];
     f2 s2[4], q2[4];
 #pragma unroll
@@ -185,18 +189,20 @@
 #pragma unroll
     for (int j = 0; j < 8; ++j) s_acc[j] = q_acc[j] = 0.f;
 
-    for (int64_t tile_id = blockIdx.x; tile_id < ntiles; tile_id += gridDim.x) {
-        const int n = (int)(tile_id / (tiles_h * tiles_w));
-        const int rem = (int)(tile_id - (int64_t)n * tiles_h * tiles_w);
-        const int oh0 = (rem / tiles_w) * TH, ow0 = (rem % tiles_w) * TW;
+    const TileWalk tiles(blockIdx.x, gridDim.x, g.N, tiles_h, tiles_w, walk & WALK_COLUMNS);
+    TileWalk::Pos tp = tiles.at(0);
+    for (int ti = 0; ti < tiles.count; tiles.advance(tp, ti), ++ti) {
+        const int n = tp.n, oh0 = tp.tr * TH, ow0 = tp.tc * TW;
         __syncthreads();
+        const int rb = carry_rows(tile, (walk & WALK_CARRY) && tp.above, K - S, IH, IW, cv);
         if constexpr (XK != 0)
-            stage_xmfma<xk_kc(XK), xk_ng(XK), true>(reinterpret_cast<bf16_t*>(tile), cv * 8, xe, g.H, g.W, n,
-                                                    oh0 * S - g.pad, ow0 * S - g.pad, IH, IW, v0 * 8, ncv * 8, ecl);
+            stage_xmfma<xk_kc(XK), xk_ng(XK), true>(reinterpret_cast<bf16_t*>(tile + rb * IW * cv), cv * 8, xe, g.H,
+                                                    g.W, n, oh0 * S - g.pad, ow0 * S - g.pad, IH, IW, v0 * 8, ncv * 8,
+                                                    ecl, nullptr, 1, rb * IW, (IH - rb) * IW);
         else
 #if !(RT1_DW_TIMING & 2)
             stage_tile<DW_SU, RG>(tile, x, g, n, oh0 * S - g.pad, ow0 * S - g.pad, IH, IW, g.H, g.W, v0, ncv, scale,
-                                      shift, act);
+                                      shift, act, rb);
 #else
             ;
 #endif
@@ -303,7 +309,7 @@
 __global__ __launch_bounds__(BLOCK, EPI == EPI_NONE ? 4 : 3) void dw_bwd_data_s2_kernel(const bf16_t* __restrict__ dy,
                                                                const float* __restrict__ w, DwGeo g, int TH, int TW,
                                                                bf16_t* __restrict__ dx, float* __restrict__ pdz,
-                                                               float* __restrict__ pdzx, BnBwdEpi e) {
+                                                               float* __restrict__ pdzx, BnBwdEpi e, int walk) {
     extern __shared__ __attribute__((aligned(16))) char smem[];
     constexpr int R = 4;
     const int DH = (TH + K) / 2 + 1, DW = (TW + K) / 2 + 1;
@@ -324,20 +330,20 @@
         wl[i] = (cc < ncv * 8) ? w[(int64_t)(v0 * 8 + cc) * K * K + tap] : 0.f;
     }
     const int tiles_h = (g.H + TH - 1) / TH, tiles_w = (g.W + TW - 1) / TW;
-    const int64_t ntiles = (int64_t)g.N * tiles_h * tiles_w;
     float s_acc[8], q_acc[8];
     stage_epi_consts<EPI>(ecl, e, v0, ncv, cv);
 #pragma unroll
     for (int j = 0; j < 8; ++j) s_acc[j] = q_acc[j] = 0.f;
 
-    for (int64_t tile_id = blockIdx.x; tile_id < ntiles; tile_id += gridDim.x) {
-        const int n = (int)(tile_id / (tiles_h * tiles_w));
-        const int rem = (int)(tile_id - (int64_t)n * tiles_h * tiles_w);
-        const int ih0 = (rem / tiles_w) * TH, iw0 = (rem % tiles_w) * TW;
+    const TileWalk tiles(blockIdx.x, gridDim.x, g.N, tiles_h, tiles_w, walk & WALK_COLUMNS);
+    TileWalk::Pos tp = tiles.at(0);
+    for (int ti = 0; ti < tiles.count; tiles.advance(tp, ti), ++ti) {
+        const int n = tp.n, ih0 = tp.tr * TH, iw0 = tp.tc * TW;
         const int oh_lo = (ih0 + g.pad - (K - 1)) >> 1;
         const int ow_lo = (iw0 + g.pad - (K - 1)) >> 1;
         __syncthreads();
-        stage_tile(tile, dy, g, n, oh_lo, ow_lo, DH, DW, g.Ho, g.Wo, v0, ncv, nullptr, nullptr, 0);
+        const int rb = carry_rows(tile, (walk & WALK_CARRY) && tp.above, DH - TH / 2, DH, DW, cv);
+        stage_tile(tile, dy, g, n, oh_lo, ow_lo, DH, DW, g.Ho, g.Wo, v0, ncv, nullptr, nullptr, 0, rb);
         __syncthreads();
         if (lane_cv >= ncv || pl >= PL) continue;
         for (int grp = pl; grp < ngroups; grp += PL) {
@@ -637,10 +643,11 @@
     if (p.k == KK && p.s == SS && p.R == RR) {                                                                      \
         if (p.ring)                                                                                                 \
             hipLaunchKernelGGL((dw_fwd_kernel<KK, SS, RR, EPI, 0, true>), grid, dim3(BLOCK), p.lds, st, x, w,       \
-                               scale, shift, act, g, p.TH, p.TW, out, ps, pq, e, XExp{nullptr, nullptr, 0});        \
+                               scale, shift, act, g, p.TH, p.TW, out, ps, pq, e, XExp{nullptr, nullptr, 0},         \
+                               walk_mode(p));                                                                       \
         else                                                                                                        \
             hipLaunchKernelGGL((dw_fwd_kernel<KK, SS, RR, EPI>), grid, dim3(BLOCK), p.lds, st, x, w, scale, shift,  \
-                               act, g, p.TH, p.TW, out, ps, pq, e, XExp{nullptr, nullptr, 0});                      \
+                               act, g, p.TH, p.TW, out, ps, pq, e, XExp{nullptr, nullptr, 0}, walk_mode(p));        \
         return (int)hipGetLastError();                                                                              \
     }
     L(3, 1, 5) L(3, 1, DW_R1) L(3, 2, 2) L(5, 1, 5) L(5, 1, DW_R1) L(5, 2, 2)
@@ -690,7 +697,7 @@
     dim3 grid(grid_x, p.chunks);
 #define L(KK, EE)                                                                                                   \
     hipLaunchKernelGGL((dw_bwd_data_s2_kernel<KK, EE>), grid, dim3(BLOCK), p.lds, st, dy, w, g, p.TH, p.TW, dx, pdz, \
-                       pdzx, e)
+                       pdzx, e, walk_mode(p))
     if (k == 3) { if (epi) L(3, EPI_BNBWD); else L(3, EPI_NONE); }
     else if (k == 5) { if (epi) L(5, EPI_BNBWD); else L(5, EPI_NONE); }
     else return (int)hipErrorInvalidValue;
@@ -710,7 +717,7 @@
 #define L(KK, SS, RR, XX)                                                                                           \
     if (p.k == KK && p.s == SS && p.xk == XX && p.R == RR) {                                                        \
         hipLaunchKernelGGL((dw_fwd_kernel<KK, SS, RR, EPI_STATS, XX>), grid, dim3(BLOCK), p.lds, st, nullptr, w,    \
-                           scale1, shift1, (int)ACT_SILU, g, p.TH, p.TW, out, psum, psq, e, xe);                    \
+                           scale1, shift1, (int)ACT_SILU, g, p.TH, p.TW, out, psum, psq, e, xe, walk_mode(p));      \
         return (int)hipGetLastError();                                                                              \
     }
 #define X1(KK, XX) L(KK, 1, DW_R1, XX)
diff --git a/pytorch_rt1_for_distributed_training_amd/csrc/kernels/dw_plan.hip b/pytorch_rt1_for_distributed_training_amd/csrc/kernels/dw_plan.hip
--- a/pytorch_rt1_for_distributed_training_amd/csrc/kernels/dw_plan.hip
+++ b/pytorch_rt1_for_distributed_training_amd/csrc/kernels/dw_plan.hip
@@ -1,5 +1,6 @@
 #include <algorithm>
 #include <array>
+#include <atomic>
 #include <unordered_map>
 
 #include "dw/dw_common.h"
@@ -199,6 +200,20 @@
     return best;
 }
 
+#ifndef DW_CARRY_MIN_SHARE
+#define DW_CARRY_MIN_SHARE 12
+#endif
+bool carry_pays(int kind, int K, int S, int TH, int tile_rows, int xk) {
+    if (tile_rows < 2) return false;
+    if (kind == TK_FWD && xk) return true;
+    int rows, o;
+    if (kind == TK_FWD) { rows = (TH - 1) * S + K; o = K - S; }
+    else if (is_uni(kind)) { rows = TH + K - 1; o = K - 1; }
+    else if (is_uni2(kind) || kind == TK_BWD_S2) { rows = (TH + K) / 2 + 1; o = rows - TH / 2; }
+    else return false;
+    return o > 0 && 2 * o <= rows && o * 100 >= DW_CARRY_MIN_SHARE * rows;
+}
+
 int clamp_grid(int64_t tiles, int max_blocks_x) {
     int64_t gx = tiles < max_blocks_x ? tiles : max_blocks_x;
     return (int)(gx < 1 ? 1 : gx);
@@ -283,6 +298,7 @@
         p.red_taps = (int)std::min<size_t>((size_t)k * k, (size_t)p.lds / per_tap);
     }
     tiles = cdiv(mh, tc.TH) * cdiv(mw, tc.TW);
+    p.carry = carry_pays(p.kind, k, S, tc.TH, cdiv(mh, tc.TH), p.xk) ? 1 : 0;
     p.err = ok ? 0 : (int)hipErrorInvalidValue;
     return p;
 }
@@ -317,10 +333,17 @@
     return p;
 }
 
+namespace {
+std::atomic<int> g_dw_carry{1};
+}
+int dw_carry() { return g_dw_carry.load(std::memory_order_relaxed); }
+
 }
 }
 
 extern "C" {
+
+int rt1_dw_set_carry(int on) { return rt1::dw::g_dw_carry.exchange(on ? 1 : 0); }
 
 int rt1_dw_grid(int N, int H, int W, int C, int k, int s, int max_blocks_x, int pro, int epi) {
     return dw_plan(OP_FWD, N, H, W, C, k, s, pro, epi, 0, 0, max_blocks_x).grid_x;
diff --git a/pytorch_rt1_for_distributed_training_amd/csrc/rt1_kernels.h b/pytorch_rt1_for_distributed_training_amd/csrc/rt1_kernels.h
--- a/pytorch_rt1_for_distributed_training_amd/csrc/rt1_kernels.h
+++ b/pytorch_rt1_for_distributed_training_amd/csrc/rt1_kernels.h
@@ -85,6 +85,7 @@
 int rt1_dw_x_supported(int cin, int C, int k, int s);
 int rt1_dw_grid_x(int N, int H, int W, int C, int k, int s, int cin, int max_blocks_x);
 int rt1_dw_tile_info(int which, int H, int W, int C, int k, int s, int cin, int* out);
+int rt1_dw_set_carry(int on);
 int rt1_dw_fwd_x(const rt1_bf16* x, int cin, const rt1_bf16* we, const float* w, const float* scale1,
                  const float* shift1, int N, int H, int W, int C, int k, int s, int grid_x, rt1_bf16* out, float* psum,
                  float* psq, hipStream_t st);
diff --git a/pytorch_rt1_for_distributed_training_amd/ops/_ext.py b/pytorch_rt1_for_distributed_training_amd/ops/_ext.py
--- a/pytorch_rt1_for_distributed_training_amd/ops/_ext.py
+++ b/pytorch_rt1_for_distributed_training_amd/ops/_ext.py
@@ -24,8 +24,10 @@
             _MOD = importlib.util.module_from_spec(spec)
             spec.loader.exec_module(_MOD)
             sys.modules[name] = _MOD
-            return _MOD
-        _MOD = importlib.import_module("pytorch_rt1_for_distributed_training_amd._rt1_hip")
+        else:
+            _MOD = importlib.import_module("pytorch_rt1_for_distributed_training_amd._rt1_hip")
+        from . import switches
+        _MOD.dw_set_carry(switches.on("dw_carry"))
     except ImportError as e:
         _ERR = e
         raise ImportError(
diff --git a/pytorch_rt1_for_distributed_training_amd/ops/switches.py b/pytorch_rt1_for_distributed_training_amd/ops/switches.py
--- a/pytorch_rt1_for_distributed_training_amd/ops/switches.py
+++ b/pytorch_rt1_for_distributed_training_amd/ops/switches.py
@@ -12,6 +12,7 @@
     "dw_s2_fused": "1",
     "dw_variant": "1",
     "dw_res": "1",
+    "dw_carry": "1",
     "pw_pro": "1",
     "proj_bwd": "1",
     "se_fused": "1",
```

Measured after the change: 1445 samples/s, median of 6. Within noise of the previous version (+0.5%).
